# ZPP-Robotics/OSQP-Solver

Measured on AMD Instinct MI355X. Metric: QPs/sec on a 1024-QP batch of box-QPs (n=512, m=1024), OSQP defaults; ADMM iters/sec alongside, higher is better.
Workload: dtype f64

## Files before the change

### include/mi_osqp.h

```cpp
#ifndef MI_OSQP_H
#define MI_OSQP_H

#include <stdint.h>

#ifdef __cplusplus
extern "C" {
#endif

typedef enum {
  MI_OSQP_OK = 0,
  MI_OSQP_ERR_INVALID_DATA = 1,
  MI_OSQP_ERR_INVALID_SETTINGS = 2,
  MI_OSQP_ERR_PATTERN_CHANGED = 3,
  MI_OSQP_ERR_NONCONVEX = 4,
  MI_OSQP_ERR_DEVICE = 5,
  MI_OSQP_ERR_NULL = 6,
  MI_OSQP_ERR_ALLOC = 7
} mi_osqp_error;

typedef enum {
  MI_OSQP_EXIT_OPTIMAL = 0,
  MI_OSQP_EXIT_PRIMAL_INFEASIBLE = 1,
  MI_OSQP_EXIT_DUAL_INFEASIBLE = 2,
  MI_OSQP_EXIT_OPTIMAL_INACCURATE = 3,
  MI_OSQP_EXIT_PRIMAL_INFEASIBLE_INACCURATE = 4,
  MI_OSQP_EXIT_DUAL_INFEASIBLE_INACCURATE = 5,
  MI_OSQP_EXIT_MAX_ITERATIONS = 6,
  MI_OSQP_EXIT_INTERRUPTED = 7,
  MI_OSQP_EXIT_TIME_LIMIT_REACHED = 8,
  MI_OSQP_EXIT_NON_CONVEX = 9,
  MI_OSQP_EXIT_UNKNOWN = 10
} mi_osqp_exit_code;

typedef struct {
  double  rho;
  double  sigma;
  int64_t scaling;
  int64_t adaptive_rho;
  int64_t adaptive_rho_interval;
  double  adaptive_rho_tolerance;
  int64_t max_iter;
  double  eps_abs;
  double  eps_rel;
  double  eps_prim_inf;
  double  eps_dual_inf;
  double  alpha;
  int64_t scaled_termination;
  int64_t check_termination;
  int64_t warm_start;
  int64_t verbose;
  int64_t polish;
  int64_t polish_refine_iter;
  double  delta;
} mi_osqp_settings;

typedef struct {
  int64_t iter;
  int64_t status_val;
  int64_t exit_code;
  double  obj_val;
  double  pri_res;
  double  dua_res;
  int64_t rho_updates;
  double  rho_estimate;
  double  rho;
  int64_t status_polish;
} mi_osqp_info;

typedef struct {
  int64_t n, m, N, batch, tile, n_tiles;
  int64_t nnz_P_triu, nnz_A, nnz_KKT, nnz_L;
  int64_t n_supernodes, n_blocks;
  int64_t fwd_levels, bwd_levels, fwd_slots, bwd_slots, chk_slots;
  int64_t lds_bytes, threads_per_block;
  int64_t dense_tail_rows, dense_tail_slots;
  double  setup_seconds_host, setup_seconds_factor, setup_seconds_upload;
  int64_t nnz_L_before_tail;
  int64_t solve_groups, solve_group_threads;
  int64_t resident_state, lds_bytes_iterate;
  int64_t pipelined_refactors;
  int64_t resident_factor_steps, lds_bytes_factor;
  int64_t dense_tail_tasks, dense_tail_waves_used, dense_tail_wave_tasks_max;
  int64_t refactor_lanes;
  int64_t iterate_launches_deep_ring, iterate_launches_long_head;
} mi_osqp_stats;

typedef struct mi_osqp_solver mi_osqp_solver;
typedef struct mi_osqp_batch  mi_osqp_batch;

void        mi_osqp_default_settings(mi_osqp_settings *s);
const char *mi_osqp_exit_code_name(int64_t exit_code);
const char *mi_osqp_error_name(int64_t err);
const char *mi_osqp_version(void);
const char *mi_osqp_last_error(void);

int mi_osqp_setup(mi_osqp_solver **out, int64_t n, int64_t m,
                  const int64_t *P_colptr, const int64_t *P_rowidx, const double *P_val,
                  const double *q,
                  const int64_t *A_colptr, const int64_t *A_rowidx, const double *A_val,
                  const double *l, const double *u, const mi_osqp_settings *settings);
int mi_osqp_update_A(mi_osqp_solver *h, const int64_t *A_colptr, const int64_t *A_rowidx,
                     const double *A_val);
int mi_osqp_update_bounds(mi_osqp_solver *h, const double *l, const double *u);
int mi_osqp_update_A_bounds(mi_osqp_solver *h, const int64_t *A_colptr, const int64_t *A_rowidx, const double *A_val,
                            const double *l, const double *u);
int mi_osqp_warm_start_x(mi_osqp_solver *h, const double *x);
int mi_osqp_update_q(mi_osqp_solver *h, const double *q);
int mi_osqp_update_P(mi_osqp_solver *h, const int64_t *P_colptr, const int64_t *P_rowidx, const double *P_val);
int mi_osqp_update_P_A(mi_osqp_solver *h, const int64_t *P_colptr, const int64_t *P_rowidx, const double *P_val,
                       const int64_t *A_colptr, const int64_t *A_rowidx, const double *A_val);
int mi_osqp_warm_start_y(mi_osqp_solver *h, const double *y);
int mi_osqp_solve(mi_osqp_solver *h, mi_osqp_info *info);
int mi_osqp_get_primal(mi_osqp_solver *h, double *x_out);
int mi_osqp_get_dual(mi_osqp_solver *h, double *y_out);
int mi_osqp_get_prim_inf_cert(mi_osqp_solver *h, double *dy_out );
int mi_osqp_get_dual_inf_cert(mi_osqp_solver *h, double *dx_out );
int mi_osqp_adjoint(mi_osqp_solver *h, const double *dx, const double *dy, double *dq, double *dP, double *dA, double *dl, double *du,
                    int32_t *status);
int mi_osqp_get_stats(mi_osqp_solver *h, mi_osqp_stats *st);
int mi_osqp_get_settings(mi_osqp_solver *h, mi_osqp_settings *out);
int mi_osqp_update_settings(mi_osqp_solver *h, const mi_osqp_settings *s);
void mi_osqp_free(mi_osqp_solver *h);

int mi_osqp_batch_setup(mi_osqp_batch **out, int64_t B, int64_t n, int64_t m,
                        const int64_t *P_colptr, const int64_t *P_rowidx, const double *P_val,
                        const double *q,
                        const int64_t *A_colptr, const int64_t *A_rowidx, const double *A_val,
                        const double *l, const double *u, const mi_osqp_settings *settings,
                        int64_t device);
int mi_osqp_batch_update_A(mi_osqp_batch *h, const int64_t *A_colptr, const int64_t *A_rowidx,
                           const double *A_val);
int mi_osqp_batch_update_bounds(mi_osqp_batch *h, const double *l, const double *u);
int mi_osqp_batch_update_A_bounds(mi_osqp_batch *h, const int64_t *A_colptr, const int64_t *A_rowidx, const double *A_val,
                                  const double *l, const double *u);
int mi_osqp_batch_warm_start_x(mi_osqp_batch *h, const double *x);
int mi_osqp_batch_update_q(mi_osqp_batch *h, const double *q);
int mi_osqp_batch_update_P(mi_osqp_batch *h, const int64_t *P_colptr, const int64_t *P_rowidx, const double *P_val);
int mi_osqp_batch_update_P_A(mi_osqp_batch *h, const int64_t *P_colptr, const int64_t *P_rowidx, const double *P_val,
                             const int64_t *A_colptr, const int64_t *A_rowidx, const double *A_val);
int mi_osqp_batch_warm_start_y(mi_osqp_batch *h, const double *y);
int mi_osqp_batch_get_P_upper_pattern(mi_osqp_batch *h, int64_t *colptr, int64_t *rowidx, int64_t *nnz_out);
int mi_osqp_batch_solve(mi_osqp_batch *h);
int mi_osqp_batch_get_primal(mi_osqp_batch *h, double *x_out );
int mi_osqp_batch_get_dual(mi_osqp_batch *h, double *y_out );
int mi_osqp_batch_get_info(mi_osqp_batch *h, mi_osqp_info *info );
int mi_osqp_batch_get_prim_inf_cert(mi_osqp_batch *h, double *dy_out );
int mi_osqp_batch_get_dual_inf_cert(mi_osqp_batch *h, double *dx_out );
int mi_osqp_batch_get_stats(mi_osqp_batch *h, mi_osqp_stats *st);
int mi_osqp_batch_get_ordering(mi_osqp_batch *h, int64_t *kkt_perm);
void mi_osqp_batch_free(mi_osqp_batch *h);
int mi_osqp_prefetch_analysis(int64_t B, int64_t n, int64_t m, const int64_t *Pp, const int64_t *Pi,
                              const int64_t *Ap, const int64_t *Ai, int64_t device);
void mi_osqp_release_device_cache(void);

int mi_osqp_batch_update_bounds_device(mi_osqp_batch *h, const double *d_l, const double *d_u, void *stream);
int mi_osqp_batch_update_A_bounds_device(mi_osqp_batch *h, const double *d_Av, const double *d_l, const double *d_u, void *stream);
int mi_osqp_batch_update_q_device(mi_osqp_batch *h, const double *d_q, void *stream);
int mi_osqp_batch_update_P_device(mi_osqp_batch *h, const double *d_Pv, void *stream);
int mi_osqp_batch_update_P_A_bounds_device(mi_osqp_batch *h, const double *d_Pv, const double *d_Av, const double *d_l, const double *d_u,
                                           void *stream);
int mi_osqp_batch_solve_device(mi_osqp_batch *h, double *d_x_out, int32_t *d_status, int32_t *d_iters, void *stream);
int mi_osqp_batch_reset(mi_osqp_batch *h);
int mi_osqp_batch_last_solve_stats(mi_osqp_batch *h, int64_t *total_iters, int64_t *kernel_launches,
                                   double *device_seconds, double *refactor_seconds, int64_t *refactor_count,
                                   double *compact_seconds);
int mi_osqp_batch_last_polish_stats(mi_osqp_batch *h, int64_t *polished, int64_t *accepted, double *seconds);
int mi_osqp_batch_get_polish_active(mi_osqp_batch *h, int8_t *act);
// ... 45 lines not shown
int mi_gomp_scene_create(mi_gomp_scene **out, mi_osqp_batch *h, int64_t dims, int64_t waypoints,
                         int64_t n_balls, const mi_gomp_ball *balls, int64_t n_lines, const mi_gomp_line *lines,
                         const double *con_lo, const double *con_hi);
typedef struct { int32_t n_joints; int32_t reserved; double a[8], d[8], alpha[8], theta0[8]; } mi_gomp_chain;
int mi_gomp_scene_create_chain(mi_gomp_scene **out, mi_osqp_batch *h, int64_t dims, int64_t waypoints,
                               const mi_gomp_chain *chain, int64_t n_balls, const mi_gomp_ball *balls,
                               int64_t n_lines, const mi_gomp_line *lines, const double *con_lo, const double *con_hi);
typedef struct { double a[3], b[3]; double radius; double margin; } mi_gomp_capsule;
int mi_gomp_scene_create_world(mi_gomp_scene **out, mi_osqp_batch *h, int64_t dims, int64_t waypoints,
                               const mi_gomp_chain *chain, int64_t n_balls, const mi_gomp_ball *balls,
                               int64_t n_lines, const mi_gomp_line *lines, int64_t n_capsules, const mi_gomp_capsule *capsules,
                               const double *con_lo, const double *con_hi);
void mi_gomp_scene_free(mi_gomp_scene *sc);
int mi_gomp_scene_set_rows(mi_gomp_scene *sc, int64_t n_ids, const int64_t *ids, const double *A_val, const double *l, const double *u);
int mi_gomp_scene_get_rows(mi_gomp_scene *sc, int64_t id, double *A_val, double *l, double *u);
int mi_gomp_assemble_some(mi_gomp_scene *sc, int64_t n_ids, const int64_t *ids, const double *x, int32_t *ok_out);
int mi_gomp_relinearise_some(mi_gomp_scene *sc, int64_t n_ids, const int64_t *ids, const double *x, int32_t *ok_out);

typedef struct mi_osqp_multi mi_osqp_multi;
int mi_osqp_multi_batch_setup(mi_osqp_multi **out, int64_t n_devices, const int64_t *devices,
                              int64_t B, int64_t n, int64_t m,
                              const int64_t *P_colptr, const int64_t *P_rowidx, const double *P_val,
                              const double *q,
                              const int64_t *A_colptr, const int64_t *A_rowidx, const double *A_val,
                              const double *l, const double *u, const mi_osqp_settings *settings);
int mi_osqp_multi_batch_update_A(mi_osqp_multi *h, const int64_t *A_colptr, const int64_t *A_rowidx, const double *A_val);
int mi_osqp_multi_batch_update_bounds(mi_osqp_multi *h, const double *l, const double *u);
int mi_osqp_multi_batch_update_A_bounds(mi_osqp_multi *h, const int64_t *A_colptr, const int64_t *A_rowidx, const double *A_val,
                                        const double *l, const double *u);
int mi_osqp_multi_batch_warm_start_x(mi_osqp_multi *h, const double *x);
int mi_osqp_multi_batch_update_q(mi_osqp_multi *h, const double *q);
int mi_osqp_multi_batch_update_P(mi_osqp_multi *h, const int64_t *P_colptr, const int64_t *P_rowidx, const double *P_val);
int mi_osqp_multi_batch_update_P_A(mi_osqp_multi *h, const int64_t *P_colptr, const int64_t *P_rowidx, const double *P_val,
                                   const int64_t *A_colptr, const int64_t *A_rowidx, const double *A_val);
int mi_osqp_multi_batch_warm_start_y(mi_osqp_multi *h, const double *y);
int mi_osqp_multi_batch_get_settings(mi_osqp_multi *h, mi_osqp_settings *out);
int mi_osqp_multi_batch_update_settings(mi_osqp_multi *h, const mi_osqp_settings *s);
int mi_osqp_multi_batch_update_rho_each(mi_osqp_multi *h, const double *rho );
int mi_osqp_multi_batch_solve(mi_osqp_multi *h);
int mi_osqp_multi_batch_solve_async(mi_osqp_multi *h);
int mi_osqp_multi_batch_wait(mi_osqp_multi *h);
int mi_osqp_multi_batch_get_primal(mi_osqp_multi *h, double *x_out );
int mi_osqp_multi_batch_get_dual(mi_osqp_multi *h, double *y_out );
int mi_osqp_multi_batch_get_info(mi_osqp_multi *h, mi_osqp_info *info );
int mi_osqp_multi_batch_get_prim_inf_cert(mi_osqp_multi *h, double *dy_out );
int mi_osqp_multi_batch_get_dual_inf_cert(mi_osqp_multi *h, double *dx_out );
int64_t mi_osqp_multi_batch_shards(mi_osqp_multi *h);
int mi_osqp_multi_batch_shard(mi_osqp_multi *h, int64_t k, int64_t *device, int64_t *begin, int64_t *end, mi_osqp_batch **handle);
void mi_osqp_multi_batch_free(mi_osqp_multi *h);

int mi_osqp_batch_spmv(mi_osqp_batch *h, const double *d_x, const double *d_y,
                       double *d_Px, double *d_Aty, double *d_Ax, void *stream);
int mi_osqp_batch_kkt_solve(mi_osqp_batch *h, const double *d_rhs, double *d_sol, void *stream);
int mi_osqp_batch_refactor_device(mi_osqp_batch *h);
int mi_osqp_batch_kernel_time(mi_osqp_batch *h, double *avg_ms, int64_t *launches);
int mi_osqp_batch_refactor_time(mi_osqp_batch *h, double *factor_ms, double *tail_ms, int64_t *launches, int64_t *qps);
int mi_osqp_batch_refactor_peak(mi_osqp_batch *h, int64_t *qps, double *factor_ms, double *tail_ms);

int mi_osqp_batch_get_scaling(mi_osqp_batch *h, double *D , double *E , double *c );

int mi_osqp_debug_host_kkt_solve(int64_t n, int64_t m,
                                 const int64_t *P_colptr, const int64_t *P_rowidx, const double *P_val,
                                 const int64_t *A_colptr, const int64_t *A_rowidx, const double *A_val,
                                 const double *l, const double *u, const mi_osqp_settings *settings,
                                 int64_t tile, const double *rhs ,
                                 double *sol_schedule , double *sol_direct ,
                                 mi_osqp_stats *st);

int mi_osqp_debug_host_block_factor(int64_t n, int64_t m,
                                    const int64_t *P_colptr, const int64_t *P_rowidx, const double *P_val,
                                    const int64_t *A_colptr, const int64_t *A_rowidx, const double *A_val,
                                    const double *l, const double *u, const mi_osqp_settings *settings,
                                    double *max_rel_diff_L, double *max_rel_diff_Dinv, int64_t *counts);

int mi_osqp_debug_refactor_chunks(int64_t n_flagged, const int64_t *flagged, int64_t n_active, const int64_t *active, int64_t tile,
                                  int64_t chunk_qps, int64_t max_chunks, int64_t *n_chunks, int64_t *work_begin, int64_t *tiles,
                                  int64_t *tile_begin);

int mi_osqp_debug_refactor_lanes(int64_t n_flagged, const int64_t *flagged, int64_t n_active, const int64_t *active, int64_t tile,
                                 int64_t chunk_qps, int64_t max_chunks, int64_t kbt, int64_t lanes, int64_t chunk0_first,
                                 int64_t scratch_slots, int64_t *n_lanes, int64_t *lane_of, int64_t *order, int64_t *order_begin,
                                 int64_t *scratch_begin, int64_t *n_waits, int64_t *wait_chunk, int64_t *wait_for);

int mi_osqp_debug_iterate_form(int64_t tiles, int64_t has_head, int64_t forced_form, int64_t long_min, int64_t *form);

int mi_osqp_debug_trace_kkt_solve(mi_osqp_batch *h, int32_t which, const double *d_rhs, double *d_sol,
                                  uint32_t *out, int64_t out_capacity_words, int64_t *dims);

#ifdef __cplusplus
}
#endif
#endif
```

### osqp-solver_amd/__init__.py

```python
import ctypes as C
import os

import numpy as np

try:
    import torch
except ImportError:
    torch = None

from . import build as _build

_HERE = os.path.dirname(os.path.abspath(__file__))
_LIB = None

EXIT_NAMES = ["kOptimal", "kPrimalInfeasible", "kDualInfeasible", "kOptimalInaccurate",
              "kPrimalInfeasibleInaccurate", "kDualInfeasibleInaccurate", "kMaxIterations",
              "kInterrupted", "kTimeLimitReached", "kNonConvex", "kUnknown"]
K_OPTIMAL = 0


class Settings(C.Structure):
    _fields_ = [("rho", C.c_double), ("sigma", C.c_double), ("scaling", C.c_int64),
                ("adaptive_rho", C.c_int64), ("adaptive_rho_interval", C.c_int64),
                ("adaptive_rho_tolerance", C.c_double), ("max_iter", C.c_int64),
                ("eps_abs", C.c_double), ("eps_rel", C.c_double), ("eps_prim_inf", C.c_double),
                ("eps_dual_inf", C.c_double), ("alpha", C.c_double), ("scaled_termination", C.c_int64),
                ("check_termination", C.c_int64), ("warm_start", C.c_int64), ("verbose", C.c_int64),
                ("polish", C.c_int64), ("polish_refine_iter", C.c_int64), ("delta", C.c_double)]


class Info(C.Structure):
    _fields_ = [("iter", C.c_int64), ("status_val", C.c_int64), ("exit_code", C.c_int64),
                ("obj_val", C.c_double), ("pri_res", C.c_double), ("dua_res", C.c_double),
                ("rho_updates", C.c_int64), ("rho_estimate", C.c_double), ("rho", C.c_double),
                ("status_polish", C.c_int64)]

    def as_dict(self):
        return {k: getattr(self, k) for k, _ in self._fields_}


class Stats(C.Structure):
    _fields_ = [(k, C.c_int64) for k in
                ("n", "m", "N", "batch", "tile", "n_tiles", "nnz_P_triu", "nnz_A", "nnz_KKT", "nnz_L",
                 "n_supernodes", "n_blocks", "fwd_levels", "bwd_levels", "fwd_slots", "bwd_slots",
                 "chk_slots", "lds_bytes", "threads_per_block", "dense_tail_rows", "dense_tail_slots")] + \
               [(k, C.c_double) for k in ("setup_seconds_host", "setup_seconds_factor", "setup_seconds_upload")] + \
               [("nnz_L_before_tail", C.c_int64), ("solve_groups", C.c_int64), ("solve_group_threads", C.c_int64),
                ("resident_state", C.c_int64), ("lds_bytes_iterate", C.c_int64), ("pipelined_refactors", C.c_int64),
                ("resident_factor_steps", C.c_int64), ("lds_bytes_factor", C.c_int64),
                ("dense_tail_tasks", C.c_int64), ("dense_tail_waves_used", C.c_int64), ("dense_tail_wave_tasks_max", C.c_int64),
                ("refactor_lanes", C.c_int64),
                ("iterate_launches_deep_ring", C.c_int64), ("iterate_launches_long_head", C.c_int64)]

    def as_dict(self):
        return {k: getattr(self, k) for k, _ in self._fields_}


class MiOsqpError(RuntimeError):
    def __init__(self, code, where):
        self.code = int(code)
        L = lib()
        msg = L.mi_osqp_error_name(int(code)).decode()
        extra = L.mi_osqp_last_error().decode()
        super().__init__(f"{where}: error {int(code)} ({msg}) {extra}")


def lib():
    global _LIB
    if _LIB is None:
        path = os.path.join(_HERE, "libmi_osqp.so")
        if os.environ.get("MI_OSQP_LIBRARY"):
            path = os.environ["MI_OSQP_LIBRARY"]
        else:
            try:
                path = _build.build()
            except Exception as e:
                if not os.path.exists(path):
                    raise ImportError(f"libmi_osqp.so missing and could not be built: {e}") from e
        L = C.CDLL(path)
        ip, dp, vp = C.POINTER(C.c_int64), C.POINTER(C.c_double), C.c_void_p
        L.mi_osqp_default_settings.argtypes = [C.POINTER(Settings)]
        for f in ("mi_osqp_exit_code_name", "mi_osqp_error_name"):
            getattr(L, f).restype = C.c_char_p; getattr(L, f).argtypes = [C.c_int64]
        L.mi_osqp_version.restype = C.c_char_p
        L.mi_osqp_last_error.restype = C.c_char_p
        L.mi_osqp_batch_setup.argtypes = [C.POINTER(vp), C.c_int64, C.c_int64, C.c_int64, ip, ip, dp, dp, ip, ip, dp,
                                          dp, dp, C.POINTER(Settings), C.c_int64]
        L.mi_osqp_batch_update_A.argtypes = [vp, ip, ip, dp]
        L.mi_osqp_batch_update_A_bounds.argtypes = [vp, ip, ip, dp, dp, dp]
        L.mi_osqp_batch_update_bounds.argtypes = [vp, dp, dp]
        L.mi_osqp_batch_warm_start_x.argtypes = [vp, dp]
        L.mi_osqp_batch_update_q.argtypes = [vp, dp]
        L.mi_osqp_batch_update_q_device.argtypes = [vp, vp, vp]
        L.mi_osqp_batch_update_P.argtypes = [vp, ip, ip, dp]
        L.mi_osqp_batch_update_P_A.argtypes = [vp, ip, ip, dp, ip, ip, dp]
        L.mi_osqp_batch_warm_start_y.argtypes = [vp, dp]
        L.mi_osqp_batch_get_P_upper_pattern.argtypes = [vp, ip, ip, ip]
        L.mi_osqp_batch_update_P_device.argtypes = [vp, vp, vp]
        L.mi_osqp_batch_update_P_A_bounds_device.argtypes = [vp, vp, vp, vp, vp, vp]
        L.mi_osqp_batch_update_P_some.argtypes = [vp, C.c_int64, ip, dp]
        L.mi_osqp_batch_update_P_A_bounds_some.argtypes = [vp, C.c_int64, ip, dp, dp, dp, dp]
        L.mi_osqp_batch_update_q_some.argtypes = [vp, C.c_int64, ip, dp]
        L.mi_osqp_batch_warm_start_y_some.argtypes = [vp, C.c_int64, ip, dp]
        L.mi_osqp_settings_update_check.argtypes = [C.POINTER(Settings), C.POINTER(Settings)]
        L.mi_osqp_batch_get_settings.argtypes = [vp, C.POINTER(Settings)]
        L.mi_osqp_batch_update_settings.argtypes = [vp, C.POINTER(Settings)]
        L.mi_osqp_batch_update_rho_each.argtypes = [vp, dp]
        L.mi_osqp_batch_update_rho_some.argtypes = [vp, C.c_int64, ip, dp]
        L.mi_osqp_get_settings.argtypes = [vp, C.POINTER(Settings)]
        L.mi_osqp_update_settings.argtypes = [vp, C.POINTER(Settings)]
        L.mi_osqp_multi_batch_get_settings.argtypes = [vp, C.POINTER(Settings)]
        L.mi_osqp_multi_batch_update_settings.argtypes = [vp, C.POINTER(Settings)]
        L.mi_osqp_multi_batch_update_rho_each.argtypes = [vp, dp]
        L.mi_osqp_batch_solve.argtypes = [vp]
        L.mi_osqp_batch_get_primal.argtypes = [vp, dp]
        L.mi_osqp_batch_get_dual.argtypes = [vp, dp]
        L.mi_osqp_batch_get_info.argtypes = [vp, C.POINTER(Info)]
        for f in ("mi_osqp_get_prim_inf_cert", "mi_osqp_get_dual_inf_cert", "mi_osqp_batch_get_prim_inf_cert",
                  "mi_osqp_batch_get_dual_inf_cert", "mi_osqp_multi_batch_get_prim_inf_cert", "mi_osqp_multi_batch_get_dual_inf_cert"):
            getattr(L, f).argtypes = [vp, dp]
        L.mi_osqp_batch_get_prim_inf_cert_some.argtypes = [vp, C.c_int64, ip, dp]
        L.mi_osqp_batch_get_dual_inf_cert_some.argtypes = [vp, C.c_int64, ip, dp]
        L.mi_osqp_batch_get_stats.argtypes = [vp, C.POINTER(Stats)]
        L.mi_osqp_batch_get_ordering.argtypes = [vp, ip]
        L.mi_osqp_batch_free.argtypes = [vp]; L.mi_osqp_batch_free.restype = None
        L.mi_osqp_batch_update_bounds_device.argtypes = [vp, vp, vp, vp]
        L.mi_osqp_batch_update_A_bounds_device.argtypes = [vp, vp, vp, vp, vp]
        L.mi_osqp_batch_solve_device.argtypes = [vp, vp, vp, vp, vp]
        L.mi_osqp_batch_reset.argtypes = [vp]
        L.mi_osqp_batch_refactor_device.argtypes = [vp]
        L.mi_osqp_batch_last_solve_stats.argtypes = [vp, ip, ip, dp, dp, ip, dp]
        L.mi_osqp_batch_last_polish_stats.argtypes = [vp, ip, ip, dp]
        L.mi_osqp_batch_get_polish_active.argtypes = [vp, C.POINTER(C.c_int8)]
        L.mi_osqp_batch_adjoint.argtypes = [vp, dp, dp, dp, dp, dp, dp, dp, C.POINTER(C.c_int32)]
        L.mi_osqp_adjoint.argtypes = [vp, dp, dp, dp, dp, dp, dp, dp, C.POINTER(C.c_int32)]
        L.mi_osqp_batch_adjoint_device.argtypes = [vp] * 10
        L.mi_osqp_batch_get_scaling.argtypes = [vp, dp, dp, dp]
        L.mi_osqp_batch_spmv.argtypes = [vp, vp, vp, vp, vp, vp, vp]
        L.mi_osqp_batch_kkt_solve.argtypes = [vp, vp, vp, vp]
        L.mi_osqp_batch_kernel_time.argtypes = [vp, dp, ip]
        L.mi_osqp_batch_refactor_time.argtypes = [vp, dp, dp, ip, ip]
        L.mi_osqp_batch_refactor_peak.argtypes = [vp, ip, dp, dp]
        L.mi_osqp_batch_reinit_some.argtypes = [vp, C.c_int64, ip, dp, dp, dp]
        L.mi_osqp_batch_update_A_bounds_some.argtypes = [vp, C.c_int64, ip, dp, dp, dp]
        L.mi_osqp_batch_warm_start_x_some.argtypes = [vp, C.c_int64, ip, dp]
        L.mi_osqp_batch_solve_begin_some.argtypes = [vp, C.c_int64, ip]
        L.mi_osqp_batch_polish_some.argtypes = [vp, C.c_int64, ip]
        L.mi_osqp_batch_advance.argtypes = [vp, C.c_int64]
        L.mi_osqp_batch_poll.argtypes = [vp, C.c_int64, ip, ip, C.c_int64]
        L.mi_osqp_batch_get_primal_some.argtypes = [vp, C.c_int64, ip, dp]
        L.mi_osqp_batch_get_dual_some.argtypes = [vp, C.c_int64, ip, dp]
        L.mi_osqp_batch_get_info_some.argtypes = [vp, C.c_int64, ip, C.POINTER(Info)]
        L.mi_osqp_batch_running.argtypes = [vp]; L.mi_osqp_batch_running.restype = C.c_int64
        L.mi_osqp_batch_ring_wraps.argtypes = [vp]; L.mi_osqp_batch_ring_wraps.restype = C.c_int64
        L.mi_osqp_release_device_cache.argtypes = []; L.mi_osqp_release_device_cache.restype = None
        L.mi_osqp_setup.argtypes = [C.POINTER(vp), C.c_int64, C.c_int64, ip, ip, dp, dp, ip, ip, dp, dp, dp, C.POINTER(Settings)]
        L.mi_osqp_update_A.argtypes = [vp, ip, ip, dp]
        L.mi_osqp_update_bounds.argtypes = [vp, dp, dp]
        L.mi_osqp_warm_start_x.argtypes = [vp, dp]
        L.mi_osqp_update_q.argtypes = [vp, dp]
        L.mi_osqp_update_P.argtypes = [vp, ip, ip, dp]
        L.mi_osqp_update_P_A.argtypes = [vp, ip, ip, dp, ip, ip, dp]
        L.mi_osqp_warm_start_y.argtypes = [vp, dp]
        L.mi_osqp_solve.argtypes = [vp, C.POINTER(Info)]
        L.mi_osqp_get_primal.argtypes = [vp, dp]
        L.mi_osqp_get_dual.argtypes = [vp, dp]
        L.mi_osqp_get_stats.argtypes = [vp, C.POINTER(Stats)]
        L.mi_osqp_free.argtypes = [vp]; L.mi_osqp_free.restype = None
        L.mi_osqp_multi_batch_setup.argtypes = [C.POINTER(vp), C.c_int64, ip, C.c_int64, C.c_int64, C.c_int64, ip, ip, dp, dp,
                                                ip, ip, dp, dp, dp, C.POINTER(Settings)]
        L.mi_osqp_multi_batch_update_A.argtypes = [vp, ip, ip, dp]
        L.mi_osqp_multi_batch_update_bounds.argtypes = [vp, dp, dp]
        L.mi_osqp_multi_batch_update_A_bounds.argtypes = [vp, ip, ip, dp, dp, dp]
        L.mi_osqp_multi_batch_warm_start_x.argtypes = [vp, dp]
        L.mi_osqp_multi_batch_update_q.argtypes = [vp, dp]
        L.mi_osqp_multi_batch_update_P.argtypes = [vp, ip, ip, dp]
        L.mi_osqp_multi_batch_update_P_A.argtypes = [vp, ip, ip, dp, ip, ip, dp]
        L.mi_osqp_multi_batch_warm_start_y.argtypes = [vp, dp]
        L.mi_osqp_multi_batch_solve.argtypes = [vp]
        L.mi_osqp_multi_batch_solve_async.argtypes = [vp]
        L.mi_osqp_multi_batch_wait.argtypes = [vp]
        L.mi_osqp_multi_batch_get_primal.argtypes = [vp, dp]
        L.mi_osqp_multi_batch_get_dual.argtypes = [vp, dp]
        L.mi_osqp_multi_batch_get_info.argtypes = [vp, C.POINTER(Info)]
        L.mi_osqp_multi_batch_shards.argtypes = [vp]; L.mi_osqp_multi_batch_shards.restype = C.c_int64
        L.mi_osqp_multi_batch_shard.argtypes = [vp, C.c_int64, ip, ip, ip, C.POINTER(vp)]
        L.mi_osqp_multi_batch_free.argtypes = [vp]; L.mi_osqp_multi_batch_free.restype = None
        L.mi_osqp_debug_host_kkt_solve.argtypes = [C.c_int64, C.c_int64, ip, ip, dp, ip, ip, dp, dp, dp,
                                                   C.POINTER(Settings), C.c_int64, dp, dp, dp, C.POINTER(Stats)]
        L.mi_osqp_debug_refactor_chunks.argtypes = [C.c_int64, ip, C.c_int64, ip, C.c_int64, C.c_int64, C.c_int64, ip, ip, ip, ip]
        L.mi_osqp_debug_refactor_lanes.argtypes = [C.c_int64, ip, C.c_int64, ip] + [C.c_int64] * 7 + [ip] * 8
        L.mi_osqp_debug_iterate_form.argtypes = [C.c_int64] * 4 + [ip]
        L.mi_osqp_prefetch_analysis.argtypes = [C.c_int64, C.c_int64, C.c_int64, ip, ip, ip, ip, C.c_int64]
        L.mi_osqp_debug_host_block_factor.argtypes = [C.c_int64, C.c_int64, ip, ip, dp, ip, ip, dp, dp, dp,
                                                      C.POINTER(Settings), dp, dp, ip]
        _LIB = L
    return _LIB


def host_cores():
    try:
        n = len(os.sched_getaffinity(0))
    except Exception:
        n = os.cpu_count() or 1
    for path in ("/sys/fs/cgroup/cpu.max",):
        try:
            quota, period = open(path).read().split()[:2]
            if quota != "max":
                n = min(n, max(1, int(round(int(quota) / int(period)))))
        except Exception:
            pass
    try:
        q = int(open("/sys/fs/cgroup/cpu/cpu.cfs_quota_us").read())
        p = int(open("/sys/fs/cgroup/cpu/cpu.cfs_period_us").read())
        if q > 0:
            n = min(n, max(1, int(round(q / p))))
    except Exception:
        pass
    return n


def default_settings(**kw):
    s = Settings()
    lib().mi_osqp_default_settings(C.byref(s))
    for k, v in kw.items():
        if not hasattr(s, k):
            raise KeyError(k)
        setattr(s, k, v)
    return s


class HandleSettings(Settings):

    def bind(self, getter):
        self._getter = getter
        return self

    def __call__(self):
        out = Settings()
        self._getter(out)
        C.memmove(C.byref(self), C.byref(out), C.sizeof(Settings))
        return out


def settings_update_check(in_force, wanted):
    return int(lib().mi_osqp_settings_update_check(C.byref(in_force), C.byref(wanted)))


def _handle_settings(kw, get_name, owner):
    import weakref
    hs = HandleSettings()
    C.memmove(C.byref(hs), C.byref(default_settings(**kw)), C.sizeof(Settings))
    ref = weakref.ref(owner)

    def getter(out):
        _chk(getattr(lib(), get_name)(ref()._h, C.byref(out)), get_name)
    return hs.bind(getter)


def _update_settings(self, fn_name, fields):
    s = self.settings()
    for k, v in fields.items():
        if not hasattr(s, k):
            raise KeyError(k)
        setattr(s, k, v)
    _chk(getattr(lib(), fn_name)(self._h, C.byref(s)), fn_name)
    return self.settings()


def _i64(a):
    return np.ascontiguousarray(a, dtype=np.int64)


def _f64(a):
# ... 498 lines not shown
        return self._b.update_settings(**fields)

    def solve(self):
        info = self._b.solve()[0]
        return int(info.exit_code), self._b.primal()[0]

    def info(self):
        return self._b.info()[0]

    def dual(self):
        return self._b.dual()[0]

    def prim_inf_cert(self):
        return self._b.prim_inf_cert()[0]

    def dual_inf_cert(self):
        return self._b.dual_inf_cert()[0]

    def adjoint(self, dx, dy=None):
        out = self._b.adjoint(dx, dy)
        return {k: (int(v[0]) if k == "status" else v[0]) for k, v in out.items()}

    def stats(self):
        return self._b.stats()


def debug_host_kkt_solve(P, A, l, u, rhs, tri_waves=0, **settings):
    L = lib()
    P, A = _csc(P), _csc(A)
    n, m = A.shape[1], A.shape[0]
    s = default_settings(**settings)
    rhs = _f64(rhs)
    sol_s, sol_d = np.empty(n + m), np.empty(n + m)
    st = Stats()
    Pp, Pi, Px = _i64(P.indptr), _i64(P.indices), _f64(P.data)
    Ap, Ai, Ax = _i64(A.indptr), _i64(A.indices), _f64(A.data)
    l, u = _f64(l), _f64(u)
    rc = L.mi_osqp_debug_host_kkt_solve(n, m, _ip(Pp), _ip(Pi), _dp(Px), _ip(Ap), _ip(Ai), _dp(Ax), _dp(l), _dp(u),
                                        C.byref(s), 1 + int(tri_waves), _dp(rhs), _dp(sol_s), _dp(sol_d), C.byref(st))
    _chk(rc, "debug_host_kkt_solve")
    return sol_s, sol_d, st.as_dict()


def prefetch_analysis(P, A, B=1, device=-1, check=True):
    L = lib()
    P, A = _csc(P), _csc(A)
    n, m = A.shape[1], A.shape[0]
    Pp, Pi, Ap, Ai = _i64(P.indptr), _i64(P.indices), _i64(A.indptr), _i64(A.indices)
    rc = L.mi_osqp_prefetch_analysis(B, n, m, _ip(Pp), _ip(Pi), _ip(Ap), _ip(Ai), device)
    if check:
        _chk(rc, "prefetch_analysis")
    return rc


def debug_refactor_chunks(flagged, active, tile, chunk_qps, max_chunks=8):
    f, a = _i64(flagged), _i64(active)
    nch = C.c_int64()
    wb = np.zeros(max_chunks + 2, dtype=np.int64); tb = np.zeros(max_chunks + 2, dtype=np.int64)
    tl = np.zeros(max(1, len(a)), dtype=np.int64)
    _chk(lib().mi_osqp_debug_refactor_chunks(len(f), _ip(f), len(a), _ip(a), tile, chunk_qps, max_chunks, C.byref(nch), _ip(wb), _ip(tl),
                                             _ip(tb)), "debug_refactor_chunks")
    k = int(nch.value)
    return ([f[wb[c]:wb[c + 1]].tolist() for c in range(k)], [tl[tb[c]:tb[c + 1]].tolist() for c in range(k)])


def debug_refactor_lanes(flagged, active, tile, chunk_qps, lanes, kbt=None, chunk0_first=False, scratch_slots=None, max_chunks=8):
    f, a = _i64(flagged), _i64(active)
    kbt = tile if kbt is None else kbt
    work, _ = debug_refactor_chunks(flagged, active, tile, chunk_qps, max_chunks)
    k = len(work)
    nl, nw = C.c_int64(), C.c_int64()
    lane_of = np.zeros(max_chunks + 2, dtype=np.int64); order = np.zeros(max_chunks + 2, dtype=np.int64)
    ob = np.zeros(4, dtype=np.int64); sb = np.zeros(max_chunks + 2, dtype=np.int64)
    wc = np.zeros((max_chunks + 1) ** 2, dtype=np.int64); wf = np.zeros((max_chunks + 1) ** 2, dtype=np.int64)
    _chk(lib().mi_osqp_debug_refactor_lanes(len(f), _ip(f), len(a), _ip(a), tile, chunk_qps, max_chunks, kbt, lanes, int(bool(chunk0_first)),
                                            2 ** 31 - 1 if scratch_slots is None else scratch_slots, C.byref(nl), _ip(lane_of), _ip(order),
                                            _ip(ob), _ip(sb), C.byref(nw), _ip(wc), _ip(wf)), "debug_refactor_lanes")
    L = int(nl.value)
    return dict(n_lanes=L, lane_of=lane_of[:k].tolist(), order=[order[ob[l]:ob[l + 1]].tolist() for l in range(L)],
                scratch=[(int(sb[c]), (len(work[c]) + kbt - 1) // kbt * kbt) for c in range(k)],
                waits=list(zip(wc[:nw.value].tolist(), wf[:nw.value].tolist())))


def debug_iterate_form(tiles, has_head=True, forced_form=0, long_min=-1):
    form = C.c_int64()
    _chk(lib().mi_osqp_debug_iterate_form(tiles, int(bool(has_head)), forced_form, long_min, C.byref(form)), "debug_iterate_form")
    return int(form.value)


def debug_host_block_factor(P, A, l, u, **settings):
    L = lib()
    P, A = _csc(P), _csc(A)
    n, m = A.shape[1], A.shape[0]
    s = default_settings(**settings)
    Pp, Pi, Px = _i64(P.indptr), _i64(P.indices), _f64(P.data)
    Ap, Ai, Ax = _i64(A.indptr), _i64(A.indices), _f64(A.data)
    l, u = _f64(l), _f64(u)
    dL, dD = C.c_double(), C.c_double()
    cnt = (C.c_int64 * 4)()
    rc = L.mi_osqp_debug_host_block_factor(n, m, _ip(Pp), _ip(Pi), _dp(Px), _ip(Ap), _ip(Ai), _dp(Ax), _dp(l), _dp(u),
                                           C.byref(s), C.byref(dL), C.byref(dD), cnt)
    _chk(rc, "debug_host_block_factor")
    return dL.value, dD.value, dict(blocks=cnt[0], triples=cnt[1], storage=cnt[2], levels=cnt[3])
```

### osqp-solver_amd/csrc/device_types.h

```cpp
#pragma once
#include <hip/hip_runtime.h>
#include <stdint.h>

namespace miosqp {

#define MI_CHUNK 16

struct SchedDev {
  const uint32_t *step, *idxw;
  const uint64_t *idxw64;
  const uint32_t *lvl_pos, *tail_bar;
  int n_phases, nw, n_levels;
  uint32_t n_steps, n_slots;
};

struct DenseTailDev {
  int s, k, n_phases;
  uint32_t n_steps;
  const uint32_t *task;
  const uint32_t *wave_task, *wave_step, *tail_bar;
};

enum { DS_C = 0, DS_CINV, DS_RHO, DS_RHO_EST, DS_PRI_RES, DS_DUA_RES, DS_OBJ, DS_COUNT };
enum { IS_STATUS = 0, IS_ITER, IS_RHO_UPDATES, IS_DONE, IS_NEED_REFACTOR, IS_CUR, IS_PENDING, IS_EPOCH, IS_COUNT };

enum { RF_FORM_NONE = 0, RF_FORM_DEEP_RING = 1, RF_FORM_LONG_HEAD = 2 };

struct KernelArgs {
  int n, m, N, B;
  SchedDev fwd, bwd, chk;
  const uint32_t *pinv;
  const uint32_t *xloc;
  const double *fwd_val, *bwd_val, *chk_val, *dinv;
  DenseTailDev dt;
  const double *dt_val;
  const double *fwd_val0, *bwd_val0, *dt_val0;
  const int *use_work;
  double *x, *z, *y;
  const double *q, *l, *u, *rho_vec, *rho_inv, *Dsc, *Dsc_inv, *Esc, *Esc_inv;
  double *dx, *dy, *out1, *out2, *dscal;
  int *iscal;
  double *x_out, *y_out;
  double *cert_out;
  int cert_stride;
  double *xs_global;
  int xs_len;
  int rs_off;
  int rf_off;
  int rf_form;
  int wide;
  double sigma, alpha, eps_abs, eps_rel, eps_prim_inf, eps_dual_inf, rho_tolerance;
  int check_termination, rho_interval, max_iter, scaled_termination, scaling, adaptive_rho;
  int iter_begin, iter_end;
  int op_out_lds;
  int info_at_end;
  int mw_groups;
  unsigned *mw_bar;
  double *mw_scratch;
  int df;
  unsigned df_shadow;
  const unsigned char *rflag;
  const int *sel;
  const int *tiles;
};

struct FactorArgs {
  int n, m, N, B, nnzP, nnzK, pa_len, n_levels, force_all;
  int debug_skip;
  uint32_t storage;
  SchedDev fwd, bwd;
  const uint32_t *blk, *lvl, *utask, *tri4, *dtask, *ttask, *asm_dst, *asm_src;
  const uint32_t *ubig;
  int *use_work;
  const int32_t *fwd_srcblk, *bwd_srcblk;
  const double *pa_val, *l, *u, *dscal;
  double *rho_vec, *rho_inv, *Lblk, *Dl, *dinv_scratch, *fwd_val, *bwd_val, *dinv;
  int *iscal, *npos;
  int home_bt;
  const int *work;
  int wg_base;
  double sigma;
  int dt_k;
  int mw_groups;
  unsigned *mw_bar;
  const signed char *pmask;
  const int32_t *arow;
  int *pstat;
  double pdelta;
};

struct TailArgs {
  int n, N, s, k, kbt, home_bt;
  uint32_t storage, n_slots;
  int n_lt, n_ltcol;
  uint32_t n_quads;
  int nh;
  uint32_t cs_doubles;
  const int *work;
  int wg_base;
  const uint32_t *lt_pos, *ltcol_col, *tile_tab, *wave_tiles, *diag_tile;
  const uint64_t *asm_q64;
  const int32_t *src_tile;
  const uint32_t *dt_task, *dt_task_step;
  uint32_t n_tasks;
  const double *Lblk, *Dl;
  double *Sd, *dt_val, *dinv;
  int *npos, *iscal;
  unsigned long long *trace;
  int *pstat;
};
hipError_t launch_tail(const TailArgs &a, int nwork, size_t lds_asm, size_t lds, hipStream_t st);

struct PolishArgs {
  int *stat;
  signed char *act;
  double *sol;
  int refine_iter;
  int inner;
  double delta;
};
hipError_t launch_polish_active(const KernelArgs &a, const PolishArgs &p, int BT, hipStream_t st);
hipError_t launch_polish_active_list(const KernelArgs &a, const PolishArgs &p, const int *slots, int nslots, int BT, hipStream_t st);
hipError_t launch_polish_publish(const KernelArgs &a, const PolishArgs &p, const int *slots, int nslots, int *host_stat, int BT, hipStream_t st);
hipError_t launch_polish(const KernelArgs &a, const PolishArgs &p, int BT, int tiles, int threads, size_t lds, int n_cus, hipStream_t st);
struct AdjointArgs {
  const double *gx, *gy;
  double *dq, *dP, *dA, *dl, *du;
  const int32_t *prow, *pcol, *arow, *acol;
  int nnzP, nnzA;
};
hipError_t launch_adjoint(const KernelArgs &a, const PolishArgs &p, const AdjointArgs &g, int BT, int tiles, int threads, size_t lds, int n_cus, hipStream_t st);
hipError_t launch_adjoint_finish(const int *stat, const AdjointArgs &g, int32_t *status, int B, int n, int m, hipStream_t st);
hipError_t launch_factor(const FactorArgs &a, int BT, int tiles, int threads, hipStream_t st);
size_t factor_lds_bytes(int BT, int threads);
bool factor_fits_lds(const FactorArgs &a, int threads);

int max_coresident_groups(int threads, size_t lds, int n_cus);
int max_coresident_factor_groups(int threads, int n_cus);
hipError_t launch_iterate(const KernelArgs &a, int BT, int tiles, int threads, size_t lds, hipStream_t st);
int rf_head_steps(int form);
int rf_lds_steps();
hipError_t launch_check(const KernelArgs &a, int BT, int tiles, int threads, size_t lds, hipStream_t st);
hipError_t launch_advance(const KernelArgs &a, int BT, int tiles, int threads, size_t lds, hipStream_t st, int max_segments, int seg_len,
                          int *host_is, double *host_ds, unsigned *stop, unsigned seq, unsigned *counter, unsigned *host_done);
hipError_t launch_spmv(const KernelArgs &a, int BT, int tiles, int threads, size_t lds, hipStream_t st,
                       const double *x, const double *y, double *Px, double *Aty, double *Ax);
struct SpmvFused {
  const uint32_t *ptr, *ent;
  const double *pa_val;
  int pa_len;
  const uint32_t *ell, *rowid;
  int n_pass;
  uint32_t ell_off[4], ell_k[4];
};
hipError_t launch_spmv_fused(const KernelArgs &a, const SpmvFused &t, int BT, int tiles, int n_cus, hipStream_t st,
                             const double *x, const double *y, double *Px, double *Aty, double *Ax);
size_t spmv_fused_lds_bytes(int n, int m, int pa_len, int BT);
hipError_t launch_kkt_solve(const KernelArgs &a, int BT, int tiles, int threads, size_t lds, hipStream_t st,
                            const double *rhs, double *sol);
hipError_t launch_kkt_trace(const KernelArgs &a, int BT, int tiles, int threads, size_t lds, hipStream_t st,
                            const double *rhs, double *sol, uint32_t *trace, uint32_t words);
hipError_t launch_warm_start(const KernelArgs &a, int BT, int tiles, int threads, size_t lds, hipStream_t st,
                             const double *x0);
hipError_t launch_interleave(const double *src, double *dst, const int *ids, int nq, int len, int BT, hipStream_t st);
hipError_t launch_scatter(const double *src, double *dst, const int *map, const int *ids, int nq, int srclen,
                          const SchedDev &sd, int BT, hipStream_t st);
hipError_t launch_deinterleave(const double *src, double *dst, int nq, int len, int BT, hipStream_t st);
struct RuizArgs {
  int n, m, nnzP, nnzA, B, BT, iters;
  const int *ids;
  int raw_by_qp;
  int fresh;
  const double *rawP, *rawq;
  const int32_t *Prow, *Pcol, *Arow, *Acol;
  const double *rawPnew;
  const double *rawA;
  const double *rawl, *rawu;
  double *pa_val, *q, *Dsc, *Dsc_inv, *Esc, *Esc_inv, *l, *u, *dscal;
  double *dn, *en;
  double *pa_out;
};
hipError_t launch_ruiz(const RuizArgs &a, hipStream_t st);
hipError_t launch_lin_cost(const double *gq, const int *ids, double *q, double *rawq, const double *Dsc, const double *dscal,
                           int nq, int n, int BT, int scaling, hipStream_t st);
hipError_t launch_warm_start_y(const KernelArgs &a, int nslots, int BT, hipStream_t st, const double *y0);
hipError_t launch_start_slots(const KernelArgs &a, const int *slots, const int *clear, int nslots, int BT, int cold, hipStream_t st);
hipError_t launch_fresh_slots(const KernelArgs &a, const int *slots, int nslots, int BT, double rho0, hipStream_t st);
hipError_t launch_set_rho_slots(const KernelArgs &a, const int *slots, const double *rho, double rho_all, int nslots, int BT, hipStream_t st);
hipError_t launch_worklist(const int *iscal, int *work, int nslots, int BT, hipStream_t st);
hipError_t launch_resume_flagged(const KernelArgs &a, int nslots, int BT, hipStream_t st);
hipError_t launch_copy_slot_streams(double *dst, const double *src, const int *slots, int nslots, size_t per, hipStream_t st);
hipError_t launch_keep_rows(double *dst, const double *src, const int *ids, int n_ids, int len, hipStream_t st);
hipError_t launch_copy_flagged_streams(double *dst, const double *src, const int *flags, int want, int nslots, size_t per, hipStream_t st);
hipError_t launch_copy_slot_rows(double *dst, const double *src, const int *slots, int nslots, int len, int BT, hipStream_t st);
enum { MI_GM_UR5E_FLANGE = 1, MI_GM_UR5E_WRIST3 = 2, MI_GM_UR5E_ELBOW = 3, MI_GM_YAW_2LINK = 4, MI_GM_TABLE = 5, MI_GM_DH_CHAIN = 6 };
#define MI_GOMP_MAXD 8
struct GompChainDev { int n_joints, pad; double a[MI_GOMP_MAXD], d[MI_GOMP_MAXD], ca[MI_GOMP_MAXD], sa[MI_GOMP_MAXD], theta0[MI_GOMP_MAXD]; };
struct GompBallDev { int model, is_gripper; double radius; double param[12]; };
struct GompLineDev { double D[3], A[3]; int below, pad; };
struct GompCapsuleDev { double a[3], e[3], ee, R, margin; };
struct GompArgs {
  int dims, W, n_balls, n_lines, n, m, nnzA, n_ids, row0, write_rows;
  int n_caps, pad;
  const int *ids;
  const GompBallDev *balls;
  const GompLineDev *lines;
  const GompCapsuleDev *caps;
  double con_lo[3], con_hi[3];
  const int *aidx;
  const double *traj;
  double *A, *l, *u;
  int *ok;
  GompChainDev chain;
};
hipError_t launch_gomp_relinearise(const GompArgs &g, hipStream_t st);
hipError_t launch_gather_status(const int *iscal, int32_t *status, int32_t *iters, int B, int BT, hipStream_t st);
hipError_t launch_fail_slots(const KernelArgs &a, const int *slots, int nfail, int BT, int iter, hipStream_t st);
hipError_t launch_fail_flagged(const KernelArgs &a, const int *slots, int nslots, int BT, int iter, hipStream_t st);
hipError_t launch_bounds(const double *gl, const double *gu, double *l, double *u, const double *Esc,
                         const double *rho_vec, const double *dscal, int *changed, int B, int m, int BT,
                         int scaling, hipStream_t st);

}
```

### osqp-solver_amd/csrc/host_core.cpp

```cpp
#include "host_core.hpp"
#include "sched_format.h"

#include <algorithm>
#include <cmath>
#include <cstdio>
#include <cstdlib>
#include <cstring>
#include <numeric>
#include <set>
#include <chrono>
#include <thread>

#include "../../include/mi_osqp.h"

namespace miosqp {

int validate_settings(const Settings &s) {
  if (s.scaling < 0 || s.max_iter <= 0 || s.check_termination < 0) return 1;
  if (s.adaptive_rho != 0 && s.adaptive_rho != 1) return 1;
  if (s.adaptive_rho_interval < 0 || s.adaptive_rho_tolerance < 1.0) return 1;
  if (!(s.rho > 0.0) || !(s.sigma > 0.0)) return 1;
  if (s.eps_abs < 0.0 || s.eps_rel < 0.0 || (s.eps_abs == 0.0 && s.eps_rel == 0.0)) return 1;
  if (!(s.eps_prim_inf > 0.0) || !(s.eps_dual_inf > 0.0)) return 1;
  if (!(s.alpha > 0.0) || !(s.alpha < 2.0)) return 1;
  if ((s.scaled_termination | 1) != 1 || (s.warm_start | 1) != 1) return 1;
  if ((s.polish | 1) != 1 || s.polish_refine_iter < 0 || !(s.delta > 0.0)) return 1;
  return 0;
}


static void min_degree(int N, const std::vector<int> &Kp, const std::vector<int> &Ki,
                       std::vector<int> &perm) {
  std::vector<std::vector<int>> adj(N);
  for (int j = 0; j < N; j++)
    for (int k = Kp[j]; k < Kp[j + 1]; k++) {
      int i = Ki[k];
      if (i != j) { adj[i].push_back(j); adj[j].push_back(i); }
    }
  for (auto &a : adj) { std::sort(a.begin(), a.end()); a.erase(std::unique(a.begin(), a.end()), a.end()); }
  std::vector<char> dead(N, 0);
  std::set<std::pair<int, int>> pq;
  std::vector<int> deg(N);
  for (int v = 0; v < N; v++) { deg[v] = (int)adj[v].size(); pq.insert({deg[v], v}); }
  perm.assign(N, 0);
  std::vector<int> tmp;
  int alive = N;
  for (int step = 0; step < N && !pq.empty();) {
    const int v = pq.begin()->second;
    pq.erase(pq.begin());
    if ((int)adj[v].size() == alive - 1) {
      perm[step++] = v; dead[v] = 1;
      for (int u = 0; u < N; u++) if (!dead[u]) { perm[step++] = u; dead[u] = 1; }
      break;
    }
    perm[step++] = v; dead[v] = 1; alive--;
    const std::vector<int> S = adj[v];
    for (int u : S) {
      tmp.clear();
      std::set_union(adj[u].begin(), adj[u].end(), S.begin(), S.end(), std::back_inserter(tmp));
      tmp.erase(std::remove_if(tmp.begin(), tmp.end(), [&](int x) { return x == u || x == v; }), tmp.end());
      adj[u].swap(tmp);
      pq.erase({deg[u], u});
      deg[u] = (int)adj[u].size();
      pq.insert({deg[u], u});
    }
    std::vector<int>().swap(adj[v]);
  }
}

namespace {
struct NDCtx {
  const std::vector<std::vector<int>> &adj;
  std::vector<int> stamp, level;
  int cur = 0;
  std::vector<int> out;
  int leaf;
};

void nd_leaf(NDCtx &c, const std::vector<int> &nodes) {
  int k = (int)nodes.size();
  if (k <= 2) { for (int v : nodes) c.out.push_back(v); return; }
  int st = ++c.cur;
  std::vector<int> loc(k);
  for (int i = 0; i < k; i++) { c.stamp[nodes[i]] = st; c.level[nodes[i]] = i; }
  std::vector<int> Kp(k + 1, 0), Ki;
  for (int j = 0; j < k; j++) {
    for (int u : c.adj[nodes[j]]) if (c.stamp[u] == st && c.level[u] < j) Ki.push_back(c.level[u]);
    Ki.push_back(j);
    Kp[j + 1] = (int)Ki.size();
  }
// ... 777 lines not shown
    }
    dt.n_lt = (int)dt.lt_pos.size(); dt.n_ltcol = (int)dt.ltcol_col.size();
    const uint16_t zero_slot = (uint16_t)dt.n_lt;
    for (auto &fr : frag) for (auto &f : fr) for (uint16_t &v : f.second) if (v == 0xFFFFu) v = zero_slot;
    struct TileRec { int I, J; std::vector<std::pair<int, int>> src; };
    std::vector<TileRec> tiles;
    for (int I = 0; I < nt; I++)
      for (int J = 0; J <= I; J++) {
        TileRec t{I, J, {}};
        size_t a = 0, b = 0;
        while (a < frag[I].size() && b < frag[J].size()) {
          if (frag[I][a].first < frag[J][b].first) a++;
          else if (frag[I][a].first > frag[J][b].first) b++;
          else { t.src.push_back({(int)a, (int)b}); a++; b++; }
        }
        tiles.push_back(std::move(t));
      }
    const int nw = 16;
    std::vector<int> order(tiles.size());
    std::iota(order.begin(), order.end(), 0);
    std::stable_sort(order.begin(), order.end(), [&](int x, int y) { return tiles[x].src.size() > tiles[y].src.size(); });
    std::vector<std::vector<int>> mine(nw);
    for (size_t d = 0; d < order.size(); d++) { const size_t round = d / nw, pos = d % nw; mine[(round & 1) ? nw - 1 - pos : pos].push_back(order[d]); }
    dt.tile_tab.clear(); dt.wave_tiles.assign(nw + 1, 0u); dt.asm_q.clear(); dt.asm_qcol.clear();
    for (int w = 0; w < nw; w++) {
      dt.wave_tiles[w] = (uint32_t)(dt.tile_tab.size() / 4);
      for (int ti : mine[w]) {
        const TileRec &t = tiles[ti];
        const uint32_t q0 = (uint32_t)(dt.asm_q.size() / 64);
        const size_t padded = (t.src.size() + 31) / 32 * 32;
        for (size_t s0 = 0; s0 < padded; s0 += 4) {
          for (int g = 0; g < 4; g++) {
            const bool real = s0 + g < t.src.size();
            const auto *fa = real ? &frag[t.I][t.src[s0 + g].first] : nullptr;
            const auto *fb = real ? &frag[t.J][t.src[s0 + g].second] : nullptr;
            dt.asm_qcol.push_back(real ? (uint16_t)fa->first : (uint16_t)0);
            for (int e = 0; e < 16; e++) dt.asm_q.push_back(real ? ((uint32_t)fa->second[e] | ((uint32_t)fb->second[e] << 16)) : ((uint32_t)zero_slot | ((uint32_t)zero_slot << 16)));
          }
        }
        const uint32_t blk_id = find_blk(ct0 + t.I, ct0 + t.J);
        dt.tile_tab.insert(dt.tile_tab.end(), {((uint32_t)t.I << 16) | (uint32_t)t.J, bf.blk[4 * blk_id], q0, (uint32_t)(dt.asm_q.size() / 64)});
      }
    }
    dt.wave_tiles[nw] = (uint32_t)(dt.tile_tab.size() / 4);
    dt.asm_q64.resize(dt.asm_q.size());
    for (size_t e = 0; e < dt.asm_q.size(); e++) {
      const uint64_t w = dt.asm_q[e], ci = dt.asm_qcol[e / 16];
      dt.asm_q64[e] = ((w & 0xFFFFu) * 8u) | ((((w >> 16) * 8u) | ((ci * 8u) << 17)) << 32);
    }
    dt.src_tile.resize(dt.src.size());
    for (size_t e = 0; e < dt.src.size(); e++) {
      const int32_t sc = dt.src[e];
      dt.src_tile[e] = sc < 0 ? sc : (int32_t)dt_tile_offset(sc % k, sc / k);
    }
    dt.diag_tile.resize(k);
    for (int i = 0; i < k; i++) dt.diag_tile[i] = dt_tile_offset(i, i);
    dt.task_step.clear();
    { uint32_t pos = 0; for (size_t t = 0; t < dt.task.size() / 4; t++) { dt.task_step.push_back(pos); pos += dt.task[4 * t + 3]; } }
  }
}


Tuning tuning_from_env() {
  Tuning t;
  if (const char *e = getenv("MI_OSQP_TILE")) { const int v = atoi(e); if (v == 1 || v == 2 || v == 4) t.tile = v; }
  if (const char *e = getenv("MI_OSQP_THREADS")) t.threads = std::max(64, std::min(1024, atoi(e) / 64 * 64));
  t.global_xs = getenv("MI_OSQP_GLOBAL_XS") != nullptr;
  if (const char *e = getenv("MI_OSQP_GROUPS")) t.groups = std::max(0, std::min(256, atoi(e)));
  if (const char *e = getenv("MI_OSQP_GROUP_THREADS")) t.group_threads = std::max(64, std::min(512, atoi(e) / 64 * 64));
  if (const char *e = getenv("MI_OSQP_ASSUME_CUS")) t.assume_cus = std::max(0, atoi(e));
  if (const char *e = getenv("MI_OSQP_FACTOR_THREADS")) t.factor_threads = std::max(64, std::min(1024, atoi(e) / 64 * 64));
  if (const char *e = getenv("MI_OSQP_FACTOR_GROUPS")) t.factor_groups = std::max(1, std::min(256, atoi(e)));
  t.ruiz = getenv("MI_OSQP_HOST_RUIZ") ? 1 : getenv("MI_OSQP_DEVICE_RUIZ") ? -1 : 0;
  if (const char *e = getenv("MI_OSQP_CONT_RING_KB")) t.cont_ring_kb = std::max(0L, atol(e));
  if (const char *e = getenv("MI_OSQP_ANALYSIS_CACHE")) t.analysis_cache = atoi(e) != 0;
  t.stream_state = getenv("MI_OSQP_STREAM_STATE") != nullptr;
  t.stream_factor = getenv("MI_OSQP_STREAM_FACTOR") != nullptr;
  if (const char *e = getenv("MI_OSQP_REFACTOR_PIPELINE")) t.refactor_pipeline = atoi(e) != 0;
  if (const char *e = getenv("MI_OSQP_REFACTOR_PIPELINE_MIN")) t.pipeline_min = std::max(0, atoi(e));
  if (const char *e = getenv("MI_OSQP_REFACTOR_CHUNKS")) t.pipeline_chunks = std::max(0, std::min(8, atoi(e)));
  if (const char *e = getenv("MI_OSQP_REFACTOR_CHUNK_QPS")) t.pipeline_chunk_qps = std::max(0, atoi(e));
  if (const char *e = getenv("MI_OSQP_REFACTOR_LANES")) t.refactor_lanes = std::max(1, std::min(3, atoi(e)));
  if (const char *e = getenv("MI_OSQP_REFACTOR_CHUNK0")) t.lanes_chunk0 = atoi(e) != 0;
  if (const char *e = getenv("MI_OSQP_RF_FORM")) { const int v = atoi(e); if (v == kIterDeepRing || v == kIterLongHead) t.rf_form = v; }
  if (const char *e = getenv("MI_OSQP_RF_LONG_MIN")) t.rf_long_min = std::max(0, atoi(e));
  AnalysisTuning &a = t.analysis;
  if (const char *e = getenv("MI_OSQP_DENSE_TAIL")) a.dense_tail = atoi(e);
  if (const char *e = getenv("MI_OSQP_ORDERING")) a.ordering = e[0];
  if (const char *e = getenv("MI_OSQP_ND_LEAF")) a.nd_leaf = atoi(e);
  if (const char *e = getenv("MI_OSQP_RELAX")) a.relax = atoi(e);
  a.serial = getenv("MI_OSQP_SERIAL_ANALYSIS") != nullptr;
  return t;
}

RefactorChunks refactor_chunks(const std::vector<int> &flagged, const std::vector<int> &active, int bt, int chunk_qps, int max_chunks) {
  RefactorChunks rc;
  const int nq = (int)flagged.size();
  max_chunks = std::max(1, max_chunks);
  chunk_qps = std::max(1, chunk_qps);
  if ((nq + chunk_qps - 1) / chunk_qps > max_chunks) chunk_qps = (nq + max_chunks - 1) / max_chunks;
  const int n_ref = (nq + chunk_qps - 1) / chunk_qps;
  rc.n_chunks = 1 + n_ref;
  rc.work_begin.assign(1, 0);
  for (int c = 0; c <= n_ref; c++) rc.work_begin.push_back(std::min(nq, c * chunk_qps));
  std::vector<std::pair<int, int>> tc;
  size_t f = 0;
  for (size_t i = 0; i < active.size(); i++) {
    const int tile = active[i] / bt;
    if (i && active[i - 1] / bt == tile) continue;
    int chunk = 0;
    while (f < flagged.size() && flagged[f] / bt < tile) f++;
    for (size_t g = f; g < flagged.size() && flagged[g] / bt == tile; g++) chunk = 1 + (int)g / chunk_qps;
    tc.emplace_back(chunk, tile);
  }
  std::stable_sort(tc.begin(), tc.end(), [](const std::pair<int, int> &x, const std::pair<int, int> &y) { return x.first < y.first; });
  rc.tile_begin.assign((size_t)rc.n_chunks + 1, 0);
  for (const auto &p : tc) { rc.tiles.push_back(p.second); rc.tile_begin[(size_t)p.first + 1]++; }
  for (int c = 0; c < rc.n_chunks; c++) rc.tile_begin[(size_t)c + 1] += rc.tile_begin[c];
  return rc;
}

RefactorLanes refactor_lanes(const RefactorChunks &ch, const std::vector<int> &flagged, int bt, int kbt, int lanes, bool chunk0_first, int scratch_slots) {
  RefactorLanes rl;
  const int nc = ch.n_chunks, n_ref = nc - 1;
  bt = std::max(1, bt); kbt = std::max(1, kbt);
  int L = std::max(1, std::min(std::min(3, lanes), std::max(1, n_ref)));
  std::vector<int> padded((size_t)nc + 1, 0);
  for (int c = 1; c < nc; c++) padded[(size_t)c + 1] = padded[c] + (ch.work_begin[(size_t)c + 1] - ch.work_begin[c] + kbt - 1) / kbt * kbt;
  if (padded[nc] > scratch_slots) L = 1;
  rl.n_lanes = L;
  rl.lane_of.assign(nc, 0);
  rl.order.assign(L, std::vector<int>());
  rl.scratch_begin.assign((size_t)nc + 1, 0);
  if (L == 1) {
    for (int c = 0; c < nc; c++) rl.order[0].push_back(c);
    return rl;
  }
  rl.scratch_begin = padded;
  for (int c = 1; c < nc; c++) { rl.lane_of[c] = (c - 1) % L; rl.order[(c - 1) % L].push_back(c); }
  if (chunk0_first) { rl.lane_of[0] = L - 1; rl.order[L - 1].insert(rl.order[L - 1].begin(), 0); }
  else {
    int at = L - 1;
    for (int a = L - 1; a >= 0; a--) if (rl.order[a].size() < rl.order[at].size()) at = a;
    rl.lane_of[0] = at; rl.order[at].push_back(0);
  }
  for (int c = 1; c < nc; c++) {
    std::vector<char> need(nc, 0);
    for (int t = ch.tile_begin[c]; t < ch.tile_begin[(size_t)c + 1]; t++) {
      const int tile = ch.tiles[t];
      size_t g = std::lower_bound(flagged.begin(), flagged.end(), tile * bt) - flagged.begin();
      for (; g < flagged.size() && flagged[g] / bt == tile; g++) {
        const int d = (int)(std::upper_bound(ch.work_begin.begin() + 1, ch.work_begin.end(), (int)g) - ch.work_begin.begin()) - 1;
        if (d >= 1 && d < c && rl.lane_of[d] != rl.lane_of[c]) need[d] = 1;
      }
    }
    for (int d = 1; d < c; d++) if (need[d]) { rl.wait_chunk.push_back(c); rl.wait_for.push_back(d); }
  }
  return rl;
}

int iterate_form(int tiles, bool has_head, const Tuning &t) {
  if (!has_head) return kIterStreamed;
  if (t.rf_form == kIterDeepRing || t.rf_form == kIterLongHead) return t.rf_form;
  const int long_min = t.rf_long_min >= 0 ? t.rf_long_min : kRfLongMinDefault;
  return tiles > 0 && tiles >= long_min ? kIterLongHead : kIterDeepRing;
}


int analyze(int64_t n64, int64_t m64, const int64_t *Pp, const int64_t *Pi, const int64_t *Ap,
            const int64_t *Ai, const AnalysisTuning &tune, Analysis &an, int nwaves, int bt, int max_extra_rows, int dense_tail_max, int tri_waves, int n_tiles) {
  if (nwaves < 1 || nwaves > 16 || (bt != 1 && bt != 2 && bt != 4) || tri_waves < 0 || tri_waves > 2048) return MI_OSQP_ERR_INVALID_SETTINGS;
  if (n64 <= 0 || m64 < 0 || !Pp || !Ap || n64 + m64 > (int64_t)1 << 30) return MI_OSQP_ERR_INVALID_DATA;
  int n = (int)n64, m = (int)m64, N = n + m;
  an = Analysis();
  an.n = n; an.m = m; an.N = N;
  if (Pp[0] != 0 || Ap[0] != 0) return MI_OSQP_ERR_INVALID_DATA;
  for (int j = 0; j < n; j++) {
    if (Pp[j + 1] < Pp[j] || Ap[j + 1] < Ap[j]) return MI_OSQP_ERR_INVALID_DATA;
    for (int64_t k = Pp[j]; k < Pp[j + 1]; k++) if (Pi[k] < 0 || Pi[k] >= n) return MI_OSQP_ERR_INVALID_DATA;
    for (int64_t k = Ap[j]; k < Ap[j + 1]; k++) if (Ai[k] < 0 || Ai[k] >= m) return MI_OSQP_ERR_INVALID_DATA;
  }
  if (Pp[n] > (int64_t)1 << 30 || Ap[n] > (int64_t)1 << 30) return MI_OSQP_ERR_INVALID_DATA;
  an.Pp.assign(n + 1, 0);
  for (int j = 0; j < n; j++) {
    an.Pp[j] = (int)an.Pi.size();
    for (int64_t k = Pp[j]; k < Pp[j + 1]; k++)
      if (Pi[k] <= j) { an.Pi.push_back((int)Pi[k]); an.Psrc.push_back((int)k); }
  }
  an.Pp[n] = (int)an.Pi.size();
  an.Ap.assign(Ap, Ap + n + 1);
  an.Ai.assign(Ai, Ai + Ap[n]);
  int nnzP = an.Pp[n], nnzA = an.Ap[n];
  std::vector<int> cnt(N, 0);
  an.PisDiag.assign(nnzP, 0);
  std::vector<char> hasDiag(n, 0);
  for (int j = 0; j < n; j++)
    for (int k = an.Pp[j]; k < an.Pp[j + 1]; k++) { cnt[j]++; if (an.Pi[k] == j) { hasDiag[j] = 1; an.PisDiag[k] = 1; } }
  for (int j = 0; j < n; j++) if (!hasDiag[j]) cnt[j]++;
  for (int k = 0; k < nnzA; k++) cnt[n + an.Ai[k]]++;
  for (int r = 0; r < m; r++) cnt[n + r]++;
  an.Kp.assign(N + 1, 0);
  for (int j = 0; j < N; j++) an.Kp[j + 1] = an.Kp[j] + cnt[j];
  an.Ki.assign(an.Kp[N], 0);
  an.PtoK.assign(nnzP, 0); an.AtoK.assign(nnzA, 0); an.rhotoK.assign(m, 0);
  std::vector<int> nxt(an.Kp.begin(), an.Kp.end() - 1);
  for (int j = 0; j < n; j++) {
    for (int k = an.Pp[j]; k < an.Pp[j + 1]; k++) { int pos = nxt[j]++; an.Ki[pos] = an.Pi[k]; an.PtoK[k] = pos; }
    if (!hasDiag[j]) { int pos = nxt[j]++; an.Ki[pos] = j; an.sigmaOnlyK.push_back(pos); }
  }
  for (int j = 0; j < n; j++)
    for (int k = an.Ap[j]; k < an.Ap[j + 1]; k++) { int pos = nxt[n + an.Ai[k]]++; an.Ki[pos] = j; an.AtoK[k] = pos; }
  for (int r = 0; r < m; r++) { int pos = nxt[n + r]++; an.Ki[pos] = n + r; an.rhotoK[r] = pos; }
  an.tri_waves = tri_waves;
  an.wide = N >= 65535 || 2 * n + m >= 65535 || tri_waves > 0;
  if (max_extra_rows < 0) max_extra_rows = 1 << 30;
  if (!an.wide && max_extra_rows > 65534 - N) max_extra_rows = 65534 - N;
  auto finalize = [&](Analysis &an, const std::vector<int> &perm0, double &cost, int relax_zeros = 0, int *phases_out = nullptr, double *stream_out = nullptr) {
    an.perm = perm0;
    an.pinv.assign(N, 0);
    for (int k = 0; k < N; k++) an.pinv[an.perm[k]] = k;
    build_permuted_lower(an);
    std::vector<std::vector<int>> cols;
    std::vector<int> parent, post;
    symbolic(an, cols, parent);
    postorder(parent, post);
    {
      std::vector<int> p2(N);
      for (int k = 0; k < N; k++) p2[k] = an.perm[post[k]];
      an.perm.swap(p2);
      for (int k = 0; k < N; k++) an.pinv[an.perm[k]] = k;
    }
    build_permuted_lower(an);
    symbolic(an, cols, parent);
    an.etree = parent;
    if (relax_zeros > 0) {
      auto close = [&](int s0, int e) {
        for (int c = s0; c < e; c++) {
          std::vector<int> ns;
          ns.reserve((size_t)(e - c) + cols[e].size());
          for (int r = c + 1; r <= e; r++) ns.push_back(r);
          ns.insert(ns.end(), cols[e].begin(), cols[e].end());
// ... 719 lines not shown
```

### osqp-solver_amd/csrc/host_core.hpp

```cpp
#pragma once

#include <cstdint>
#include <string>
#include <vector>

namespace miosqp {

constexpr double kInfty = 1e30;
constexpr double kRhoMin = 1e-6, kRhoMax = 1e6, kRhoEqOverIneq = 1e3, kRhoTol = 1e-4;
constexpr double kMinScaling = 1e-4, kMaxScaling = 1e4;
constexpr double kDivisionTol = 1.0 / kInfty;
constexpr int kChunk = 16;
constexpr uint32_t kNoRow = 0xFFFFFFFFu;

struct Settings {
  double rho = 0.1, sigma = 1e-6;
  int64_t scaling = 10, adaptive_rho = 1, adaptive_rho_interval = 0;
  double adaptive_rho_tolerance = 5.0;
  int64_t max_iter = 4000;
  double eps_abs = 1e-3, eps_rel = 1e-3, eps_prim_inf = 1e-4, eps_dual_inf = 1e-4, alpha = 1.6;
  int64_t scaled_termination = 0, check_termination = 25, warm_start = 1, verbose = 0;
  int64_t polish = 0, polish_refine_iter = 3;
  double delta = 1e-6;
};
int validate_settings(const Settings &s);

struct AnalysisTuning {
  int dense_tail = -1;
  char ordering = 0;
  int nd_leaf = 0;
  int relax = -1;
  bool serial = false;
  bool operator==(const AnalysisTuning &o) const {
    return dense_tail == o.dense_tail && ordering == o.ordering && nd_leaf == o.nd_leaf && relax == o.relax && serial == o.serial;
  }
};
struct Tuning {
  int tile = 0;
  int threads = 0;
  bool global_xs = false;
  int groups = -1;
  int group_threads = 0;
  int assume_cus = 0;
  int factor_threads = 1024;
  int factor_groups = 0;
  int ruiz = 0;
  long cont_ring_kb = -1;
  bool analysis_cache = true;
  bool stream_state = false;
  bool stream_factor = false;
  bool refactor_pipeline = true;
  int pipeline_min = 0;
  int pipeline_chunks = 0;
  int pipeline_chunk_qps = 0;
  int refactor_lanes = 0;
  int lanes_chunk0 = -1;
  int rf_form = 0;
  int rf_long_min = -1;
  AnalysisTuning analysis;
};
Tuning tuning_from_env();

enum IterateForm { kIterStreamed = 0, kIterDeepRing = 1, kIterLongHead = 2 };
constexpr int kRfLongMinDefault = 0;
int iterate_form(int tiles, bool has_head, const Tuning &t);

struct RefactorChunks {
  int n_chunks = 1;
  std::vector<int> work_begin;
  std::vector<int> tiles;
  std::vector<int> tile_begin;
};
RefactorChunks refactor_chunks(const std::vector<int> &flagged, const std::vector<int> &active, int bt, int chunk_qps, int max_chunks);

struct RefactorLanes {
  int n_lanes = 1;
  std::vector<int> lane_of;
  std::vector<std::vector<int>> order;
  std::vector<int> scratch_begin;
  std::vector<int> wait_chunk, wait_for;
};
RefactorLanes refactor_lanes(const RefactorChunks &ch, const std::vector<int> &flagged, int bt, int kbt, int lanes, bool chunk0_first, int scratch_slots);

struct Schedule {
  int n_phases = 0, nw = 0, bt = 1;
  bool barriers = true;
  std::vector<uint32_t> phase;
  std::vector<int> level_first_phase;
  std::vector<uint32_t> step;
  std::vector<uint32_t> step_ob;
  std::vector<uint32_t> outA;
  std::vector<uint32_t> idx;
  std::vector<uint32_t> idxw;
  std::vector<uint64_t> idxw64;
  std::vector<int32_t> src;
  uint32_t n_slots = 0;
  uint32_t n_steps = 0;
  std::vector<uint32_t> wave_range;
  std::vector<uint32_t> lvl_pos;
  std::vector<uint32_t> tail_bar;
  bool dataflow = false;
  uint32_t shadow = 0, pad = 0;
  uint32_t phys_steps() const { return n_steps; }
  size_t phase_stride() const { return 4 * (size_t)nw + 1; }
  int n_levels = 0;
};

struct BlockFactor {
  uint32_t storage = 0;
  std::vector<uint32_t> blk;
  std::vector<uint32_t> lvl;
  std::vector<uint32_t> utask;
  std::vector<uint32_t> tri;
  std::vector<uint32_t> tri4;
  std::vector<uint32_t> utask4;
  bool overflow = false;
  std::vector<uint32_t> ubig;
  std::vector<uint32_t> dtask4;
  std::vector<uint32_t> ttask4;
  std::vector<uint32_t> dtask;
  std::vector<uint32_t> ttask;
  std::vector<uint32_t> asm_dst;
  std::vector<uint32_t> asm_src;
  std::vector<int32_t> lpos;
  int n_levels = 0;
  size_t n_blocks() const { return blk.size() / 4; }
};
enum { ASM_P = 0, ASM_P_SIGMA = 1, ASM_SIGMA = 2, ASM_A = 3, ASM_NEG_RHOINV = 4 };

struct DenseTail {
  int s = 0, k = 0, nb = 0;
  int nw = 0, n_phases = 0;
  uint32_t n_steps = 0;
  std::vector<uint32_t> task;
  std::vector<uint32_t> wave_task;
  std::vector<uint32_t> wave_step;
  std::vector<uint32_t> tail_bar;
  std::vector<int32_t> src;
  std::vector<uint32_t> sblk;
  int n_lt = 0, n_ltcol = 0;
  std::vector<uint32_t> lt_pos;
  std::vector<uint32_t> ltcol_col;
  std::vector<uint32_t> tile_tab;
  std::vector<uint32_t> wave_tiles;
  std::vector<uint32_t> asm_q;
  std::vector<uint16_t> asm_qcol;
  std::vector<uint64_t> asm_q64;
  std::vector<int32_t> src_tile;
  std::vector<uint32_t> diag_tile;
  std::vector<uint32_t> task_step;
  size_t asm_lds_bytes() const { return ((size_t)n_lt + 1 + (size_t)n_ltcol) * sizeof(double); }
};
inline uint32_t dt_tile_offset(int i, int j) {
  const int I = i / 16, J = j / 16, r = i % 16, c = j % 16;
  return (uint32_t)((I * (I + 1) / 2 + J) * 256 + ((r % 4) * 16 + c) * 4 + r / 4);
}
enum { DT_DIAG = 1, DT_SWAP = 2 };

struct Analysis {
  int n = 0, m = 0, N = 0;
  bool wide = false;
  std::vector<int> Pp, Pi, Psrc;
  std::vector<int> Ap, Ai;
  std::vector<int> Kp, Ki, PtoK, AtoK, rhotoK, sigmaOnlyK;
  std::vector<char> PisDiag;
// ... 65 lines not shown
```

### osqp-solver_amd/csrc/kernels.hip

```cpp
#include <hip/hip_runtime.h>
#include <stdint.h>
#include <stdlib.h>
#include <string.h>

#include <algorithm>
#include <map>
#include <mutex>

#include "device_types.h"
#include "sched_format.h"

namespace miosqp {

static hipError_t ensure_dynamic_lds(const void *kern, size_t lds);

#define MI_INFTY 1e30
#define MI_MIN_SCALING 1e-4
#define MI_DIV_TOL 1e-30
#define MI_RHO_EST_DIV 1e-10
#define MI_RHO_MIN 1e-6
#define MI_RHO_MAX 1e6
#define MI_NOROW 0xFFFFFFFFu
#ifdef MI_OSQP_DEBUG_BUILD
#define MI_DBG_SKIP(a) ((a).debug_skip)
// ... 881 lines not shown
      run_tri<BT, MI_PFV_NT(NT, GX), GX, 0, WIDE>(a.bwd, p.vbwd, xs, wave, lane);
    } else {
      kkt_solve_lds<BT, MI_PFV_NT(NT, GX), GX, WIDE>(a, p, xs, tid, nthr, wave, nw, lane, mw);
    }
    constexpr int U = GX ? 4 : 1;
    int tid_i = tid;
    if constexpr (RF != 0) asm volatile("" : "+v"(tid_i));
    uint32_t fl[U], xl[U];
    for (int e0 = tid_i; e0 < n * BT; e0 += nthr * U) {
      size_t pos[U]; double xt[U], xp[U], qv[U];
#pragma unroll
      for (int u = 0; u < U; u++) { const int e = e0 + u * nthr < n * BT ? e0 + u * nthr : e0; pos[u] = (size_t)a.pinv[e / BT] * BT + b; }
      if (df) {
#pragma unroll
        for (int u = 0; u < U; u++) { fl[u] = a.rflag[pos[u]]; xl[u] = a.xloc[pos[u]]; }
      }
#pragma unroll
      for (int u = 0; u < U; u++) {
        const int e = e0 + u * nthr < n * BT ? e0 + u * nthr : e0;
        xt[u] = df ? ld_sc1(xs + df_bloc((uint32_t)pos[u], fl[u], sh)) : xs[pos[u]]; xp[u] = X[e]; qv[u] = Q[e];
      }
#pragma unroll
      for (int u = 0; u < U; u++) {
        const int e = e0 + u * nthr;
        if (e < n * BT) {
          double xn = alpha * xt[u] + (1.0 - alpha) * xp[u];
          if (!done) {
            X[e] = xn;
            if constexpr (RS) { if (last) p.x[e] = xn; }
            if (do_info) p.dx[e] = xn - xp[u];
          } else xn = xp[u];
          if (df) { st_sc1(xs + pos[u], sigma * xn - qv[u]); df_arm_fwd(xs, (uint32_t)pos[u], fl[u], xl[u], sh); }
          else xs[pos[u]] = sigma * xn - qv[u];
        }
      }
    }
    for (int e0 = tid_i; e0 < m * BT; e0 += nthr * U) {
      size_t pos[U]; double nu[U], zp[U], yv[U], ri[U], rv[U], lo[U], up[U];
#pragma unroll
      for (int u = 0; u < U; u++) { const int e = e0 + u * nthr < m * BT ? e0 + u * nthr : e0; pos[u] = (size_t)a.pinv[n + e / BT] * BT + b; }
      if (df) {
#pragma unroll
        for (int u = 0; u < U; u++) { fl[u] = a.rflag[pos[u]]; xl[u] = a.xloc[pos[u]]; }
      }
#pragma unroll
      for (int u = 0; u < U; u++) {
        const int e = e0 + u * nthr < m * BT ? e0 + u * nthr : e0;
        nu[u] = df ? ld_sc1(xs + df_bloc((uint32_t)pos[u], fl[u], sh)) : xs[pos[u]]; zp[u] = Z[e]; yv[u] = Y[e]; ri[u] = RI[e]; rv[u] = RV[e]; lo[u] = LO[e]; up[u] = UP[e];
      }
#pragma unroll
      for (int u = 0; u < U; u++) {
        const int e = e0 + u * nthr;
        if (e < m * BT) {
          double zt = zp[u] - ri[u] * yv[u];
          zt += ri[u] * nu[u];
          const double zr = alpha * zt + (1.0 - alpha) * zp[u];
          double zn = fmin(fmax(zr + ri[u] * yv[u], lo[u]), up[u]);
          const double dyv = rv[u] * (zr - zn);
          double yn = yv[u] + dyv;
          if (!done) {
            Z[e] = zn; Y[e] = yn;
            if constexpr (RS) { if (last) { p.z[e] = zn; p.y[e] = yn; } }
            if (do_info) p.dy[e] = dyv;
          } else { zn = zp[u]; yn = yv[u]; }
          if (df) { st_sc1(xs + pos[u], zn - ri[u] * yn); df_arm_fwd(xs, (uint32_t)pos[u], fl[u], xl[u], sh); }
          else xs[pos[u]] = zn - ri[u] * yn;
        }
      }
    }
    if constexpr (GX) wg_or_grid_barrier(mw); else __syncthreads();
  }
}
template <int BT, int NT, bool GX, bool WIDE = false, bool RS = false, int RF = 0>
__global__ __launch_bounds__(NT) void iterate_kernel(KernelArgs a) {
  extern __shared__ double smem[];
  iterate_body<BT, NT, GX, WIDE, RS, RF>(a, smem, a.iter_end - a.iter_begin);
}

template <int BT, int NT, bool GX, bool WIDE = false>
__device__ __forceinline__ int check_body(const KernelArgs &a, double *smem, int n_iter) {
  bool dfm = false;
  if constexpr (GX && BT == 1 && WIDE) dfm = a.df != 0 && a.mw_groups > 1;
  const Mw mw{a.mw_bar, dfm ? (unsigned)a.mw_groups : 1u};
  const int tile = dfm ? 0 : blockIdx.x;
  const int ltid = threadIdx.x, lwave = __builtin_amdgcn_readfirstlane(ltid >> 6), lnw = blockDim.x >> 6;
  const int tid = dfm ? blockIdx.x * blockDim.x + threadIdx.x : threadIdx.x, nthr = dfm ? blockDim.x * mw.G : blockDim.x;
  const int lane = tid & 63, wave = __builtin_amdgcn_readfirstlane(tid >> 6), nw = nthr >> 6;
  const int b = tid % BT;
  auto sync = [&]() { if constexpr (GX && BT == 1 && WIDE) wg_or_grid_barrier(mw); else __syncthreads(); };
  auto gscratch = [&](int slot) { return a.mw_scratch + (size_t)slot * 256 * 16; };
  const int n = a.n, m = a.m;
  double *red;
  double *xs = solve_vector<BT, GX>(a, smem, tile, red);
  const TilePtrs<BT> p = tile_ptrs<BT>(a, tile, true);
  int done = p.iscal[IS_DONE * BT + b];
  if (__syncthreads_and(done)) return 0;
  const int iter = p.iscal[IS_CUR * BT + b] + n_iter;
  int status = p.iscal[IS_STATUS * BT + b];
  int rho_updates = p.iscal[IS_RHO_UPDATES * BT + b];
  double rho = p.dscal[DS_RHO * BT + b];
  const double c = p.dscal[DS_C * BT + b], cinv = p.dscal[DS_CINV * BT + b];
  const bool unscale = a.scaling && !a.scaled_termination;
  const bool is_last = iter >= a.max_iter;
  const bool is_check = a.check_termination && (iter % a.check_termination == 0);
  const bool is_rho = a.adaptive_rho && a.rho_interval && (iter % a.rho_interval == 0);
  bool any_check = is_check || is_last, any_last = is_last;
  if constexpr (BT > 1) { any_check = __syncthreads_or(any_check); any_last = __syncthreads_or(any_last); }
  int need_refactor = 0;
  for (int e = tid; e < n * BT; e += nthr) xs[e] = p.x[e];
  for (int e = tid; e < m * BT; e += nthr) xs[(size_t)n * BT + e] = p.y[e];
  sync();
  run_spmv<BT, MI_PFV, WIDE>(a.chk, p.vchk, xs, p.out1, wave, lane, 0, 3, nw);
  sync();
  double mx[14];
#pragma unroll
  for (int k = 0; k < 14; k++) mx[k] = 0.0;
  double sm[1] = {0.0};
  for (int e = tid; e < n * BT; e += nthr) {
    const double px = p.out1[e], aty = p.out1[(size_t)n * BT + e], qv = p.q[e], xv = p.x[e];
    const double di = p.Dsc_inv[e];
    double dres = qv + px;
    dres += aty;
    mx[0] = fmax(mx[0], fabs(dres));      mx[1] = fmax(mx[1], fabs(di * dres));
    mx[2] = fmax(mx[2], fabs(qv));        mx[3] = fmax(mx[3], fabs(aty));   mx[4] = fmax(mx[4], fabs(px));
    mx[5] = fmax(mx[5], fabs(di * qv));   mx[6] = fmax(mx[6], fabs(di * aty)); mx[7] = fmax(mx[7], fabs(di * px));
    sm[0] += 0.5 * xv * px + qv * xv;
  }
  for (int e = tid; e < m * BT; e += nthr) {
    const double ax = p.out1[(size_t)2 * n * BT + e], zv = p.z[e], ei = p.Esc_inv[e];
    const double pres = ax - zv;
    mx[8] = fmax(mx[8], fabs(pres));      mx[9] = fmax(mx[9], fabs(ei * pres));
    mx[10] = fmax(mx[10], fabs(zv));      mx[11] = fmax(mx[11], fabs(ax));
    mx[12] = fmax(mx[12], fabs(ei * zv)); mx[13] = fmax(mx[13], fabs(ei * ax));
  }
  block_reduce<BT, 14, true>(mx, red, ltid, lwave, lnw, lane);
  block_reduce<BT, 1, false>(sm, red, ltid, lwave, lnw, lane);
  if constexpr (GX && BT == 1 && WIDE) {
    grid_reduce<14, true>(mx, red, mw, gscratch(0), ltid, lwave, lnw, lane);
    grid_reduce<1, false>(sm, red, mw, gscratch(1), ltid, lwave, lnw, lane);
  }
  const double pri_res = (m == 0) ? 0.0 : (unscale ? mx[9] : mx[8]);
  const double dua_res = unscale ? cinv * mx[1] : mx[0];
  double obj = sm[0];
  if (a.scaling) obj *= cinv;
  const double pri_nrm = unscale ? fmax(mx[12], mx[13]) : fmax(mx[10], mx[11]);
  const double dua_nrm = unscale ? cinv * fmax(fmax(mx[5], mx[6]), mx[7]) : fmax(fmax(mx[2], mx[3]), mx[4]);

  double mi[4] = {0.0, 0.0, 0.0, 0.0};
  double si[2] = {0.0, 0.0};
  for (int e = tid; e < n * BT; e += nthr) {
    const double d = p.dx[e];
    xs[e] = d;
    mi[1] = fmax(mi[1], unscale ? fabs(p.Dsc[e] * d) : fabs(d));
    si[1] += p.q[e] * d;
  }
  for (int e = tid; e < m * BT; e += nthr) {
    double d = p.dy[e];
    const double lo = p.l[e], up = p.u[e];
    if (up > MI_INFTY * MI_MIN_SCALING) {
      if (lo < -MI_INFTY * MI_MIN_SCALING) d = 0.0; else d = fmin(d, 0.0);
    } else if (lo < -MI_INFTY * MI_MIN_SCALING) d = fmax(d, 0.0);
    xs[(size_t)n * BT + e] = d;
    mi[0] = fmax(mi[0], unscale ? fabs(p.Esc[e] * d) : fabs(d));
    si[0] += up * fmax(d, 0.0) + lo * fmin(d, 0.0);
  }
  sync();
  run_spmv<BT, MI_PFV, WIDE>(a.chk, p.vchk, xs, p.out2, wave, lane, 0, 3, nw);
// ... 41 lines not shown
             mi[3] < cost_scaling * eps_dinf * norm_dx) dual_inf = viol[0] == 0.0;
    if (prim_ok && dual_ok) return approx ? 2 : 1;
    if (prim_inf) return approx ? 3 : -3;
    if (dual_inf) return approx ? 4 : -4;
    return 0;
  };

  int new_status = 0;
  if (any_check) { const int s0 = decide(false); if (is_check || is_last) new_status = s0; }
  double rho_est = p.dscal[DS_RHO_EST * BT + b];
  auto rho_estimate = [&]() -> double {
    const double pr = mx[8] / (fmax(mx[10], mx[11]) + MI_RHO_EST_DIV);
    const double du = mx[0] / (fmax(fmax(mx[2], mx[3]), mx[4]) + MI_RHO_EST_DIV);
    double e = rho * sqrt(pr / du);
    return fmin(fmax(e, MI_RHO_MIN), MI_RHO_MAX);
  };
  if (!done && is_rho && (new_status == 0 || (is_last && !is_check))) {
    const double rn = rho_estimate();
    rho_est = rn;
    if (rn > rho * a.rho_tolerance || rn < rho / a.rho_tolerance) {
      need_refactor = 1;
      rho = fmin(fmax(rn, MI_RHO_MIN), MI_RHO_MAX);
      rho_updates++;
    }
  }
  if (any_last) {
    const int s1 = decide(true);
    if (!done && new_status == 0 && is_last) new_status = s1 ? s1 : -2;
  }
  if (!done && new_status != 0) {
    done = 1; status = new_status;
    rho_est = rho_estimate();

    if (tid < BT) {
      p.dscal[DS_PRI_RES * BT + b] = pri_res; p.dscal[DS_DUA_RES * BT + b] = dua_res;
      p.dscal[DS_OBJ * BT + b] = (status == -3 || status == 3) ? MI_INFTY
                                 : (status == -4 || status == 4) ? -MI_INFTY
                                 : (status == -7) ? __builtin_nan("") : obj;
      p.iscal[IS_ITER * BT + b] = iter;
    }
  }
  if (tid < BT) p.dscal[DS_RHO_EST * BT + b] = rho_est;
  const int just_done = done && (p.iscal[IS_DONE * BT + b] == 0);
  sync();
  const int slot = tile * BT + b, qp = slot < a.B ? slot : -1;
  if (just_done && qp >= 0) {
    const bool has_sol = !(status == -3 || status == 3 || status == -4 || status == 4 || status == -7);
    const double nanv = __builtin_nan("");
    for (int e = tid; e < n * BT; e += nthr) {
      const int i = e / BT;
      a.x_out[(size_t)qp * n + i] = has_sol ? (a.scaling ? p.Dsc[e] * p.x[e] : p.x[e]) : nanv;
      if (!has_sol) p.x[e] = 0.0;
    }
    for (int e = tid; e < m * BT; e += nthr) {
      const int j = e / BT;
      a.y_out[(size_t)qp * m + j] = has_sol ? (a.scaling ? p.Esc[e] * p.y[e] * cinv : p.y[e]) : nanv;
      if (!has_sol) { p.y[e] = 0.0; p.z[e] = 0.0; }
    }
    if (status == -3 || status == 3) {
      double *cert = a.cert_out + (size_t)qp * a.cert_stride;
      for (int e = tid; e < m * BT; e += nthr) {
        double d = p.dy[e];
        const double lo = p.l[e], up = p.u[e];
        if (up > MI_INFTY * MI_MIN_SCALING) {
          if (lo < -MI_INFTY * MI_MIN_SCALING) d = 0.0; else d = fmin(d, 0.0);
        } else if (lo < -MI_INFTY * MI_MIN_SCALING) d = fmax(d, 0.0);
        cert[e / BT] = (unscale ? p.Esc[e] * d : d) / norm_dy;
      }
    } else if (status == -4 || status == 4) {
      double *cert = a.cert_out + (size_t)qp * a.cert_stride;
      for (int e = tid; e < n * BT; e += nthr) {
        const double d = p.dx[e];
        cert[e / BT] = (unscale ? p.Dsc[e] * d : d) / norm_dx;
      }
    }
  }
  sync();
  const bool was_done = done && !just_done;
  if (tid < BT) {
    p.iscal[IS_DONE * BT + b] = done; p.iscal[IS_STATUS * BT + b] = status;
    p.iscal[IS_RHO_UPDATES * BT + b] = rho_updates;
    if (!was_done) { p.iscal[IS_NEED_REFACTOR * BT + b] = need_refactor; p.iscal[IS_CUR * BT + b] = iter; }
    p.dscal[DS_RHO * BT + b] = rho;
  }
  int ev = (just_done ? 1 : 0) | (need_refactor ? 2 : 0);
  if constexpr (BT > 1) ev = (__syncthreads_or(ev & 1) ? 1 : 0) | (__syncthreads_or(ev & 2) ? 2 : 0);
  return ev;
}
template <int BT, int NT, bool GX, bool WIDE = false>
__global__ __launch_bounds__(NT) void check_kernel(KernelArgs a) {
  extern __shared__ double smem[];
  (void)check_body<BT, NT, GX, WIDE>(a, smem, a.iter_end - a.iter_begin);
}

struct AdvanceArgs {
  int max_segments, seg_len;
  int *host_is;
  double *host_ds;
  unsigned *stop;
  unsigned seq;
  unsigned *counter;
  unsigned *host_done;
};
template <int BT, int NT, bool RS = false>
__global__ __launch_bounds__(NT) void advance_kernel(KernelArgs a, AdvanceArgs v) {
  extern __shared__ double smem[];
  const int tile = blockIdx.x, tid = threadIdx.x;
  int *is = a.iscal + (size_t)tile * IS_COUNT * BT;
  if (tid < BT && __hip_atomic_load(&is[IS_PENDING * BT + tid], __ATOMIC_ACQUIRE, __HIP_MEMORY_SCOPE_AGENT) == 1) {
    is[IS_PENDING * BT + tid] = 0; is[IS_DONE * BT + tid] = 0;
  }
  __syncthreads();
  bool iterated = false;
  for (int sgm = 0; sgm < v.max_segments; sgm++) {
    const int done = tid < BT ? is[IS_DONE * BT + tid] : 1;
    if (__syncthreads_and(done)) break;
    iterated = true;
    iterate_body<BT, NT, false, false, RS>(a, smem, v.seg_len);
    const int ev = check_body<BT, NT, false>(a, smem, v.seg_len);
    if ((ev & 1) && v.stop && tid == 0) __hip_atomic_store(v.stop, v.seq, __ATOMIC_RELAXED, __HIP_MEMORY_SCOPE_AGENT);
    if (ev & 2) {
      __syncthreads();
      if (tid < BT && is[IS_NEED_REFACTOR * BT + tid] == 1 && !is[IS_DONE * BT + tid]) { is[IS_DONE * BT + tid] = 1; is[IS_PENDING * BT + tid] = 2; }
    }
    if (v.stop && sgm + 1 < v.max_segments) {
      const unsigned sw = __hip_atomic_load(v.stop, __ATOMIC_RELAXED, __HIP_MEMORY_SCOPE_AGENT);
      if (__syncthreads_or(sw == v.seq)) break;
    }
    __syncthreads();
  }
  if (!v.host_is) return;
  __syncthreads();
  if (tid < IS_COUNT * BT) v.host_is[(size_t)tile * IS_COUNT * BT + tid] = is[tid];
  if (v.host_ds && tid < DS_COUNT * BT) v.host_ds[(size_t)tile * DS_COUNT * BT + tid] = a.dscal[(size_t)tile * DS_COUNT * BT + tid];
  __threadfence_system();
  __syncthreads();
  if (tid == 0 && v.counter) {
    if (iterated) __hip_atomic_fetch_add(v.counter + 1, 1u, __ATOMIC_RELAXED, __HIP_MEMORY_SCOPE_AGENT);
    const unsigned left = __hip_atomic_fetch_add(v.counter, 1u, __ATOMIC_ACQ_REL, __HIP_MEMORY_SCOPE_AGENT) + 1u;
    if (left == gridDim.x) {
      const unsigned active = __hip_atomic_load(v.counter + 1, __ATOMIC_RELAXED, __HIP_MEMORY_SCOPE_AGENT);
      __hip_atomic_store(v.counter, 0u, __ATOMIC_RELAXED, __HIP_MEMORY_SCOPE_AGENT);
      __hip_atomic_store(v.counter + 1, 0u, __ATOMIC_RELAXED, __HIP_MEMORY_SCOPE_AGENT);
      v.host_done[1] = active;
      __threadfence_system();
      __hip_atomic_store(v.host_done, v.seq, __ATOMIC_RELEASE, __HIP_MEMORY_SCOPE_SYSTEM);
    }
  }
}


template <int BT, int NT, bool GX, bool WIDE = false>
__global__ __launch_bounds__(NT) void spmv_kernel(KernelArgs a, const double *__restrict__ gx,
                                                    const double *__restrict__ gy, double *gPx,
                                                    double *gAty, double *gAx) {
  extern __shared__ double smem[];
  const int tile = blockIdx.x, tid = threadIdx.x, nthr = blockDim.x;
  const int lane = tid & 63, wave = __builtin_amdgcn_readfirstlane(tid >> 6);
  const int n = a.n, m = a.m;
  double *lds_rest;
  double *xs = solve_vector<BT, GX>(a, smem, tile, lds_rest);
  const TilePtrs<BT> p = tile_ptrs<BT>(a, tile);
  double *res = a.op_out_lds ? smem + (size_t)(n + m) * BT : p.out1;
  for (int bb = 0; bb < BT; bb++) {
    const int q = tile * BT + bb;
    const bool ok = q < a.B;
// ... 1437 lines not shown
    return hipGetLastError();
  };
  const int slots = (a.k / 16 - 4 + MI_TAIL_NW - 1) / MI_TAIL_NW;
  if (slots <= 1) return go(&tail_kernel<1, 4>);
  if (slots == 2) return go(&tail_kernel<2, 4>);
  if (slots == 3) return go(&tail_kernel<3, 4>);
  return go(&tail_kernel<4, 4>);
}


__global__ void interleave_kernel(const double *__restrict__ src, double *dst, const int *ids, int nq,
                                  int len, int BT) {
  const size_t g = (size_t)blockIdx.x * blockDim.x + threadIdx.x;
  if (g >= (size_t)nq * len) return;
  const int j = (int)(g / len), i = (int)(g % len);
  const int q = ids ? ids[j] : j;
  dst[((size_t)(q / BT) * len + i) * BT + (q % BT)] = src[g];
}
__global__ void scatter_kernel(const double *__restrict__ src, double *dst, const int *__restrict__ map,
                               const int *ids, int nq, int srclen, SchedDev sd, int BT) {
  const size_t g = (size_t)blockIdx.x * blockDim.x + threadIdx.x;
  const uint32_t slots = sd.n_slots;
  if (g >= (size_t)nq * slots) return;
  const int j = (int)(g / slots);
  const uint32_t s = (uint32_t)(g % slots);
  const int q = ids ? ids[j] : j;
  dst[(size_t)q * slots + s] = slot_value(map[s], src + (size_t)j * srclen, 1, 0);
  (void)BT;
}
__global__ void deinterleave_kernel(const double *__restrict__ src, double *dst, int nq, int len, int BT) {
  const size_t g = (size_t)blockIdx.x * blockDim.x + threadIdx.x;
  if (g >= (size_t)nq * len) return;
  const int q = (int)(g / len), i = (int)(g % len);
  dst[g] = src[((size_t)(q / BT) * len + i) * BT + (q % BT)];
}
__global__ void gather_status_kernel(const int *__restrict__ iscal, int32_t *status, int32_t *iters, int B, int BT) {
  const int q = blockIdx.x * blockDim.x + threadIdx.x;
  if (q >= B) return;
  const int *t = iscal + (size_t)(q / BT) * IS_COUNT * BT;
  if (status) status[q] = t[IS_STATUS * BT + q % BT];
  if (iters) iters[q] = t[IS_ITER * BT + q % BT];
}
__global__ void fail_slots_kernel(KernelArgs a, const int *__restrict__ slots, int BT, int iter) {
  const int slot = slots[blockIdx.x], tid = threadIdx.x, nthr = blockDim.x;
  if (slot < 0) return;
  const size_t tile = (size_t)slot / BT, b = (size_t)slot % BT;
  const int qp = slot < a.B ? slot : -1;
  const double nanv = __builtin_nan("");
  for (int i = tid; i < a.n; i += nthr) {
    a.x[(tile * a.n + i) * BT + b] = 0.0;
    if (qp >= 0) a.x_out[(size_t)qp * a.n + i] = nanv;
  }
  for (int j = tid; j < a.m; j += nthr) {
    a.z[(tile * a.m + j) * BT + b] = 0.0; a.y[(tile * a.m + j) * BT + b] = 0.0;
    if (qp >= 0) a.y_out[(size_t)qp * a.m + j] = nanv;
  }
  if (tid == 0) {
    int *is = a.iscal + tile * IS_COUNT * BT;
    is[IS_DONE * BT + b] = 1; is[IS_STATUS * BT + b] = -7; is[IS_NEED_REFACTOR * BT + b] = 0; is[IS_ITER * BT + b] = iter;
    double *ds = a.dscal + tile * DS_COUNT * BT;
    ds[DS_OBJ * BT + b] = nanv; ds[DS_PRI_RES * BT + b] = nanv; ds[DS_DUA_RES * BT + b] = nanv;
  }
}
hipError_t launch_fail_slots(const KernelArgs &a, const int *slots, int nfail, int BT, int iter, hipStream_t st) {
  if (!nfail) return hipSuccess;
  hipLaunchKernelGGL(fail_slots_kernel, dim3(nfail), dim3(256), 0, st, a, slots, BT, iter);
  return hipGetLastError();
}
__device__ __forceinline__ void fail_one_slot(const KernelArgs &a, int slot, int BT, int iter, int tid, int nthr) {
  const size_t tile = (size_t)slot / BT, b = (size_t)slot % BT;
  const double nanv = __builtin_nan("");
  for (int i = tid; i < a.n; i += nthr) { a.x[(tile * a.n + i) * BT + b] = 0.0; if (slot < a.B) a.x_out[(size_t)slot * a.n + i] = nanv; }
  for (int j = tid; j < a.m; j += nthr) {
    a.z[(tile * a.m + j) * BT + b] = 0.0; a.y[(tile * a.m + j) * BT + b] = 0.0;
    if (slot < a.B) a.y_out[(size_t)slot * a.m + j] = nanv;
  }
  if (tid == 0) {
    int *is = a.iscal + tile * IS_COUNT * BT;
    is[IS_DONE * BT + b] = 1; is[IS_STATUS * BT + b] = -7; is[IS_ITER * BT + b] = iter;
    double *ds = a.dscal + tile * DS_COUNT * BT;
    ds[DS_OBJ * BT + b] = nanv; ds[DS_PRI_RES * BT + b] = nanv; ds[DS_DUA_RES * BT + b] = nanv;
  }
}
__global__ void fail_flagged_kernel(KernelArgs a, const int *__restrict__ slots, int BT, int iter) {
  const int slot = slots[blockIdx.x];
  if (slot < 0) return;
  int *flag = a.iscal + ((size_t)slot / BT) * IS_COUNT * BT + IS_NEED_REFACTOR * BT + (size_t)slot % BT;
  if (*flag >= 0) return;
  fail_one_slot(a, slot, BT, iter, threadIdx.x, blockDim.x);
  __syncthreads();
  if (threadIdx.x == 0) *flag = 0;
}
hipError_t launch_fail_flagged(const KernelArgs &a, const int *slots, int nslots, int BT, int iter, hipStream_t st) {
  if (nslots <= 0) return hipSuccess;
  hipLaunchKernelGGL(fail_flagged_kernel, dim3(nslots), dim3(256), 0, st, a, slots, BT, iter);
  return hipGetLastError();
}
__global__ void start_slots_kernel(KernelArgs a, const int *__restrict__ slots, const int *__restrict__ clear, int BT, int cold) {
  const int slot = slots[blockIdx.x], tid = threadIdx.x, nthr = blockDim.x;
  if (slot < 0) return;
  const size_t tile = (size_t)slot / BT, b = (size_t)slot % BT;
  int *is = a.iscal + tile * IS_COUNT * BT;
  if (is[IS_NEED_REFACTOR * BT + b] < 0) {
    fail_one_slot(a, slot, BT, 0, tid, nthr);
    __syncthreads();
    if (tid == 0) { is[IS_PENDING * BT + b] = 0; __threadfence_system(); is[IS_EPOCH * BT + b] += 1; }
    return;
  }
  if (cold) {
    for (int i = tid; i < a.n; i += nthr) a.x[(tile * a.n + i) * BT + b] = 0.0;
    for (int j = tid; j < a.m; j += nthr) { a.z[(tile * a.m + j) * BT + b] = 0.0; a.y[(tile * a.m + j) * BT + b] = 0.0; }
  }
  __syncthreads();
  if (tid == 0) {
    is[IS_STATUS * BT + b] = -10; is[IS_ITER * BT + b] = 0; is[IS_NEED_REFACTOR * BT + b] = 0;
    is[IS_CUR * BT + b] = 0;
    if (clear[blockIdx.x]) is[IS_RHO_UPDATES * BT + b] = 0;
    __threadfence();
    __hip_atomic_store(&is[IS_PENDING * BT + b], 1, __ATOMIC_RELEASE, __HIP_MEMORY_SCOPE_AGENT);
    __threadfence();
    is[IS_EPOCH * BT + b] += 1;
  }
}
hipError_t launch_start_slots(const KernelArgs &a, const int *slots, const int *clear, int nslots, int BT, int cold, hipStream_t st) {
  if (!nslots) return hipSuccess;
  hipLaunchKernelGGL(start_slots_kernel, dim3(nslots), dim3(256), 0, st, a, slots, clear, BT, cold);
  return hipGetLastError();
}
__global__ void fresh_slots_kernel(KernelArgs a, const int *__restrict__ slots, int BT, double rho0) {
  const int slot = slots[blockIdx.x], tid = threadIdx.x, nthr = blockDim.x;
  if (slot < 0) return;
  const size_t tile = (size_t)slot / BT, b = (size_t)slot % BT;
  for (int i = tid; i < a.n; i += nthr) { a.x[(tile * a.n + i) * BT + b] = 0.0; a.dx[(tile * a.n + i) * BT + b] = 0.0; }
  for (int j = tid; j < a.m; j += nthr) { a.z[(tile * a.m + j) * BT + b] = 0.0; a.y[(tile * a.m + j) * BT + b] = 0.0; a.dy[(tile * a.m + j) * BT + b] = 0.0; }
  if (tid == 0) {
    int *is = a.iscal + tile * IS_COUNT * BT;
    is[IS_STATUS * BT + b] = -10; is[IS_ITER * BT + b] = 0; is[IS_RHO_UPDATES * BT + b] = 0; is[IS_DONE * BT + b] = 1;
    is[IS_NEED_REFACTOR * BT + b] = 0; is[IS_CUR * BT + b] = 0; is[IS_PENDING * BT + b] = 0;
    double *ds = a.dscal + tile * DS_COUNT * BT;
    ds[DS_RHO * BT + b] = rho0; ds[DS_RHO_EST * BT + b] = rho0; ds[DS_PRI_RES * BT + b] = 0.0; ds[DS_DUA_RES * BT + b] = 0.0; ds[DS_OBJ * BT + b] = 0.0;
  }
}
hipError_t launch_fresh_slots(const KernelArgs &a, const int *slots, int nslots, int BT, double rho0, hipStream_t st) {
  if (!nslots) return hipSuccess;
  hipLaunchKernelGGL(fresh_slots_kernel, dim3(nslots), dim3(256), 0, st, a, slots, BT, rho0);
  return hipGetLastError();
}
__global__ void set_rho_slots_kernel(KernelArgs a, const int *__restrict__ slots, const double *__restrict__ rho, double rho_all, int nslots, int BT) {
  const int j = (int)(blockIdx.x * blockDim.x + threadIdx.x);
  if (j >= nslots) return;
  const int slot = slots ? slots[j] : j;
  if (slot < 0) return;
  const size_t tile = (size_t)slot / BT, b = (size_t)slot % BT;
  a.dscal[(tile * DS_COUNT + DS_RHO) * BT + b] = rho ? rho[j] : rho_all;
}
hipError_t launch_set_rho_slots(const KernelArgs &a, const int *slots, const double *rho, double rho_all, int nslots, int BT, hipStream_t st) {
  if (nslots <= 0) return hipSuccess;
  hipLaunchKernelGGL(set_rho_slots_kernel, dim3((nslots + 255) / 256), dim3(256), 0, st, a, slots, rho, rho_all, nslots, BT);
  return hipGetLastError();
}
__global__ __launch_bounds__(1024) void worklist_kernel(const int *__restrict__ iscal, int *work, int nslots, int BT) {
  __shared__ int s_cnt;
  if (threadIdx.x == 0) s_cnt = 0;
  for (int s = threadIdx.x; s < nslots; s += blockDim.x) work[s] = -1;
  __syncthreads();
  for (int s = threadIdx.x; s < nslots; s += blockDim.x)
    if (iscal[(size_t)(s / BT) * IS_COUNT * BT + IS_NEED_REFACTOR * BT + s % BT] == 1) work[atomicAdd(&s_cnt, 1)] = s;
}
hipError_t launch_worklist(const int *iscal, int *work, int nslots, int BT, hipStream_t st) {
  hipLaunchKernelGGL(worklist_kernel, dim3(1), dim3(1024), 0, st, iscal, work, nslots, BT);
  return hipGetLastError();
}
__global__ void resume_flagged_kernel(KernelArgs a, int BT) {
  const int slot = blockIdx.x, tid = threadIdx.x, nthr = blockDim.x;
  const size_t tile = (size_t)slot / BT, b = (size_t)slot % BT;
  int *is = a.iscal + tile * IS_COUNT * BT;
  if (is[IS_PENDING * BT + b] != 2) return;
  const int flag = is[IS_NEED_REFACTOR * BT + b];
  if (flag == 1) return;
  if (flag < 0) fail_one_slot(a, slot, BT, is[IS_CUR * BT + b], tid, nthr);
  __syncthreads();
  __threadfence();
  if (tid == 0) __hip_atomic_store(&is[IS_PENDING * BT + b], flag < 0 ? 0 : 1, __ATOMIC_RELEASE, __HIP_MEMORY_SCOPE_AGENT);
}
hipError_t launch_resume_flagged(const KernelArgs &a, int nslots, int BT, hipStream_t st) {
  if (!nslots) return hipSuccess;
  hipLaunchKernelGGL(resume_flagged_kernel, dim3(nslots), dim3(64), 0, st, a, BT);
  return hipGetLastError();
}
__global__ void copy_slot_streams_kernel(double *dst, const double *__restrict__ src, const int *__restrict__ slots, size_t per) {
  const int slot = slots[blockIdx.y];
  if (slot < 0) return;
  const size_t off = (size_t)slot * per;
  for (size_t e = (size_t)blockIdx.x * blockDim.x + threadIdx.x; e < per; e += (size_t)gridDim.x * blockDim.x) dst[off + e] = src[off + e];
}
__global__ void copy_flagged_streams_kernel(double *dst, const double *__restrict__ src, const int *__restrict__ flags, int want, size_t per) {
  const int slot = blockIdx.y;
  if (flags && (flags[slot] != 0) != (want != 0)) return;
  const size_t off = (size_t)slot * per;
  for (size_t e = (size_t)blockIdx.x * blockDim.x + threadIdx.x; e < per; e += (size_t)gridDim.x * blockDim.x) dst[off + e] = src[off + e];
}
hipError_t launch_copy_flagged_streams(double *dst, const double *src, const int *flags, int want, int nslots, size_t per, hipStream_t st) {
  if (!nslots || !per) return hipSuccess;
  const unsigned gx = (unsigned)std::min<size_t>(64, (per + 1023) / 1024);
  hipLaunchKernelGGL(copy_flagged_streams_kernel, dim3(gx, nslots), dim3(256), 0, st, dst, src, flags, want, per);
  return hipGetLastError();
}
hipError_t launch_copy_slot_streams(double *dst, const double *src, const int *slots, int nslots, size_t per, hipStream_t st) {
  if (!nslots || !per) return hipSuccess;
  const unsigned gx = (unsigned)std::min<size_t>(64, (per + 255) / 256);
  hipLaunchKernelGGL(copy_slot_streams_kernel, dim3(gx, nslots), dim3(256), 0, st, dst, src, slots, per);
  return hipGetLastError();
}
__global__ void copy_slot_rows_kernel(double *dst, const double *__restrict__ src, const int *__restrict__ slots, int len, int BT) {
  const int slot = slots[blockIdx.y];
  if (slot < 0) return;
  const size_t base = (size_t)(slot / BT) * len * BT + slot % BT;
  for (int i = blockIdx.x * blockDim.x + threadIdx.x; i < len; i += gridDim.x * blockDim.x) dst[base + (size_t)i * BT] = src[base + (size_t)i * BT];
}
hipError_t launch_copy_slot_rows(double *dst, const double *src, const int *slots, int nslots, int len, int BT, hipStream_t st) {
  if (!nslots || !len) return hipSuccess;
  const unsigned gx = (unsigned)std::min(16, (len + 255) / 256);
  hipLaunchKernelGGL(copy_slot_rows_kernel, dim3(gx, nslots), dim3(256), 0, st, dst, src, slots, len, BT);
  return hipGetLastError();
}
__global__ void keep_rows_kernel(double *__restrict__ dst, const double *__restrict__ src, const int *__restrict__ ids, int len) {
  const int j = blockIdx.y;
  const size_t to = (size_t)ids[j] * len, from = (size_t)j * len;
  for (int i = blockIdx.x * blockDim.x + threadIdx.x; i < len; i += gridDim.x * blockDim.x) dst[to + i] = src[from + i];
}
hipError_t launch_keep_rows(double *dst, const double *src, const int *ids, int n_ids, int len, hipStream_t st) {
  if (!n_ids || !len) return hipSuccess;
  const unsigned gx = (unsigned)std::min(16, (len + 255) / 256);
  hipLaunchKernelGGL(keep_rows_kernel, dim3(gx, n_ids), dim3(256), 0, st, dst, src, ids, len);
  return hipGetLastError();
}
__global__ void bounds_kernel(const double *__restrict__ gl, const double *__restrict__ gu, double *l, double *u,
                              const double *__restrict__ Esc, const double *__restrict__ rho_vec,
                              const double *__restrict__ dscal, int *changed, int B, int m, int BT, int scaling) {
  const size_t g = (size_t)blockIdx.x * blockDim.x + threadIdx.x;
  if (g >= (size_t)B * m) return;
  const int q = (int)(g / m), i = (int)(g % m);
  const size_t e = ((size_t)(q / BT) * m + i) * BT + (q % BT);
  double lo = fmax(gl[g], -MI_INFTY), up = fmin(gu[g], MI_INFTY);
  if (lo > up) { atomicOr(changed, 2); return; }
  if (scaling) { lo *= Esc[e]; up *= Esc[e]; }
  l[e] = lo; u[e] = up;
  const double rho = dscal[((size_t)(q / BT) * DS_COUNT + DS_RHO) * BT + (q % BT)];
  double want;
  if (lo < -MI_INFTY * MI_MIN_SCALING && up > MI_INFTY * MI_MIN_SCALING) want = MI_RHO_MIN;
  else if (up - lo < 1e-4) want = 1e3 * rho;
  else want = rho;
  if (want != rho_vec[e]) atomicOr(changed, 1);
// ... 718 lines not shown
```

### osqp-solver_amd/csrc/solver.hip

```cpp
#include <hip/hip_runtime.h>
#include <time.h>

#include <algorithm>
#include <atomic>
#include <chrono>
#include <cmath>
#include <condition_variable>
#include <functional>
#include <limits>
#include <cstdio>
#include <cstdlib>
#include <cstring>
#include <string>
#include <thread>
#include <map>
#include <memory>
#include <mutex>
#include <vector>

#include "../../include/mi_osqp.h"
#include "device_types.h"
#include "host_core.hpp"

using namespace miosqp;
// ... 202 lines not shown
    return 0;
  }
  void free() { if (p && !devpool::give(dev, p, cap)) (void)hipFree(p); p = nullptr; n = 0; cap = 0; }
  ~DevBuf() { free(); }
};

struct SchedBufs {
  DevBuf<uint32_t> step, idxw, lvl_pos, tail_bar;
  DevBuf<uint64_t> idxw64;
  DevBuf<int32_t> src;
  int upload(const Schedule &s) {
    int rc;
    if ((rc = step.upload(s.step)) || (rc = idxw.upload(s.idxw)) || (rc = idxw64.upload(s.idxw64)) || (rc = src.upload(s.src)) ||
        (rc = lvl_pos.upload(s.lvl_pos)) || (rc = tail_bar.upload(s.tail_bar))) return rc;
    return 0;
  }
  SchedDev view(const Schedule &s) const {
    SchedDev d; d.step = step.p; d.idxw = idxw.p; d.idxw64 = idxw64.p; d.lvl_pos = lvl_pos.p; d.tail_bar = tail_bar.p;
    d.n_phases = s.n_phases; d.nw = s.nw; d.n_levels = s.n_levels;
    d.n_steps = s.n_steps; d.n_slots = s.n_slots;
    return d;
  }
};

struct mi_osqp_batch {
  Settings st;
  bool rho_interval_auto = false;
  Tuning tune;
  std::shared_ptr<const Analysis> anp;
  int B = 0, BT = 1, ntiles = 0, threads = 512, device = 0, n_cus = 256;
  size_t lds = 0;
  size_t lds_iter = 0;
  int rs_off = 0;
  size_t lds_factor = 0;
  int rf_off = 0, rf_steps = 0;
  int64_t rf_launches[3] = {0, 0, 0};
  std::vector<QPNumeric> qp;
  bool host_bounds_stale = false;
  hipStream_t stream = nullptr;
  SchedBufs fwd, bwd, chk;
  DevBuf<uint32_t> pinv, xloc;
  DevBuf<double> fwd_val, bwd_val, chk_val, dinv, x, z, y, q, l, u, rho_vec, rho_inv, Dsc, Dsc_inv, Esc, Esc_inv;
  DevBuf<double> dx, dy, out1, out2, dscal, x_out, y_out, xs_global;
  DevBuf<double> cert_out;
  bool global_xs = false;
  int mw_groups = 0, mw_threads = 0;
  DevBuf<uint32_t> mw_bar;
  DevBuf<unsigned char> rflag;
  DevBuf<double> mw_scratch;
  DevBuf<double> fwd_val0, bwd_val0, dinv0, rho_vec0, rho_inv0, dscal0;
  DevBuf<int> use_work;
  DevBuf<int> iscal, flag, npos;
  DevBuf<uint32_t> bf_blk, bf_lvl, bf_utask, bf_tri, bf_dtask, bf_ttask, bf_asm_dst, bf_asm_src, bf_ubig;
  DevBuf<int32_t> fwd_srcblk, bwd_srcblk;
  DevBuf<double> pa_val, Lblk, Dl, dinv_scratch;
  DevBuf<uint32_t> dt_task, dt_wave_task, dt_wave_step, dt_tail_bar;
  DevBuf<uint32_t> dt_lt_pos, dt_ltcol_col, dt_tile_tab, dt_wave_tiles, dt_diag_tile, dt_task_step;
  DevBuf<uint64_t> dt_asm_q64;
  DevBuf<int32_t> dt_src_tile;
  int dt_nh = 0; uint32_t dt_cs_doubles = 0; size_t dt_lds = 0, dt_lds_asm = 0;
  DevBuf<int32_t> dt_src;
  DevBuf<double> dt_val, dt_val0, dt_Sd;
  DevBuf<uint32_t> sp_ptr, sp_ent;
  DevBuf<uint32_t> sp_ell, sp_rowid;
  int sp_npass = 0;
  uint32_t sp_ell_off[4] = {0, 0, 0, 0}, sp_ell_k[4] = {0, 0, 0, 0};
  bool host_rho_stale = false;
  bool host_scaling_stale = false;
  DevBuf<int32_t> rz_prow, rz_pcol, rz_arow, rz_acol;
  bool clear_rho_updates = true;
  int *h_npos = nullptr;
  DevBuf<double> stage; DevBuf<int> ids, work;
  int *h_iscal = nullptr;
  double *h_dscal = nullptr;
  size_t h_iscal_cap = 0, h_dscal_cap = 0, h_npos_cap = 0, pin_cap = 0;
  double *pin = nullptr;
  size_t pin_n = 0;
  hipEvent_t ev0 = nullptr, ev1 = nullptr, evf0 = nullptr, evf1 = nullptr, evf2 = nullptr;
  hipStream_t pipe_r = nullptr, pipe_i = nullptr, pipe_x = nullptr;
  hipEvent_t pipe_ev[streampool::kPipeEvents] = {};
  DevBuf<int> tile_list;
  int64_t pipelined_refactors = 0;
  int64_t refactor_lanes = 0;
  double factor_ms_sum = 0.0, dense_ms_sum = 0.0;
  int64_t refactor_launches = 0, refactor_qps = 0, peak_qps = 0;
  double peak_factor_ms = 0.0, peak_tail_ms = 0.0;
  mi_osqp_stats stats{};
  int64_t last_total_iters = 0, last_launches = 0, last_refactors = 0;
  double last_device_s = 0.0, last_refactor_s = 0.0, kernel_ms_sum = 0.0;
  int64_t kernel_launches = 0, kernel_qp_iters = 0;
  bool solved_once = false;
  std::vector<char> failed;
  DevBuf<int> fail_list;
  DevBuf<double> rawP, rawq;
  DevBuf<double> pol_fwd, pol_bwd, pol_dinv, pol_dt, pol_sol;
  DevBuf<signed char> pol_act;
  DevBuf<int> pol_stat;
  std::vector<int> pol_status;
  int64_t pol_count = 0, pol_accepted = 0;
  double pol_seconds = 0.0;
  hipEvent_t evp0 = nullptr, evp1 = nullptr;
  DevBuf<int> adj_stat;
  struct Cont {
    bool on = false;
    int L = 25;
    unsigned launch_seq = 0;
    DevBuf<unsigned> stop;
    int64_t adv_seq = 0, polled_seq = 0;
    std::vector<char> running, clear_rho;
    std::vector<mi_osqp_info> info;
    int n_running = 0;
    int *h_is[2] = {nullptr, nullptr}; double *h_ds[2] = {nullptr, nullptr}; size_t h_is_cap[2] = {0, 0}, h_ds_cap[2] = {0, 0};
    hipEvent_t ev[2] = {nullptr, nullptr}; int64_t seq_of[2] = {0, 0};
    double *xh = nullptr, *yh = nullptr; size_t xh_cap = 0, yh_cap = 0;
    double *ch = nullptr; size_t ch_cap = 0;
    std::vector<int> cert_status;
    char *ring_h = nullptr; size_t ring_cap = 0, ring_h_cap = 0, ring_head = 0;
    int64_t ring_wraps = 0;
    DevBuf<char> ring_d;
    DevBuf<int> work;
    hipEvent_t ev_adv = nullptr;
    std::vector<int> epoch;
    DevBuf<double> rz_scratch;
    double *keepA = nullptr, *keepl = nullptr, *keepu = nullptr;
    DevBuf<unsigned> counter;
    unsigned *h_done = nullptr; size_t h_done_cap = 0;
    std::vector<char> polishable, polishing;
    std::vector<int> pol_status;
    int *h_pstat = nullptr; size_t h_pstat_cap = 0;
  } cont;
  ~mi_osqp_batch() {
    DevGuard guard(device);
    if (stream) (void)hipStreamSynchronize(stream);
    for (int k = 0; k < 2; k++) { hostpool::give(cont.h_is[k], cont.h_is_cap[k]); hostpool::give(cont.h_ds[k], cont.h_ds_cap[k]); if (cont.ev[k]) (void)hipEventDestroy(cont.ev[k]); }
    hostpool::give(cont.xh, cont.xh_cap); hostpool::give(cont.yh, cont.yh_cap); hostpool::give(cont.ch, cont.ch_cap); hostpool::give(cont.ring_h, cont.ring_h_cap);
    if (cont.ev_adv) (void)hipEventDestroy(cont.ev_adv);
    if (evp0) (void)hipEventDestroy(evp0);
    if (evp1) (void)hipEventDestroy(evp1);
    hostpool::give(cont.h_done, cont.h_done_cap); hostpool::give(cont.h_pstat, cont.h_pstat_cap);
    hostpool::give(h_iscal, h_iscal_cap); hostpool::give(h_dscal, h_dscal_cap); hostpool::give(pin, pin_cap); hostpool::give(h_npos, h_npos_cap);
    if (pipe_r) (void)hipStreamSynchronize(pipe_r);
    if (pipe_i) (void)hipStreamSynchronize(pipe_i);
    if (pipe_x) (void)hipStreamSynchronize(pipe_x);
    streampool::Bundle sb{device, stream, {ev0, ev1, evf0, evf1, evf2}, pipe_r, pipe_i, pipe_x, {}};
    for (int k = 0; k < streampool::kPipeEvents; k++) sb.pipe_ev[k] = pipe_ev[k];
    if (stream && ev0 && ev1 && evf0 && evf1 && evf2) streampool::give(sb);
    else streampool::destroy(sb);
  }
};

struct mi_osqp_solver { mi_osqp_batch *b = nullptr; };


static Settings to_settings(const mi_osqp_settings *s) {
  Settings t;
  if (!s) return t;
  t.rho = s->rho; t.sigma = s->sigma; t.scaling = s->scaling; t.adaptive_rho = s->adaptive_rho;
  t.adaptive_rho_interval = s->adaptive_rho_interval; t.adaptive_rho_tolerance = s->adaptive_rho_tolerance;
  t.max_iter = s->max_iter; t.eps_abs = s->eps_abs; t.eps_rel = s->eps_rel; t.eps_prim_inf = s->eps_prim_inf;
  t.eps_dual_inf = s->eps_dual_inf; t.alpha = s->alpha; t.scaled_termination = s->scaled_termination;
  t.check_termination = s->check_termination; t.warm_start = s->warm_start; t.verbose = s->verbose;
  t.polish = s->polish; t.polish_refine_iter = s->polish_refine_iter; t.delta = s->delta;
  return t;
}

static void dense_tail_deal_stats(const DenseTail &dt, mi_osqp_stats &s) {
  s.dense_tail_tasks = s.dense_tail_waves_used = s.dense_tail_wave_tasks_max = 0;
  if (!dt.k) return;
  s.dense_tail_tasks = (int64_t)dt.task.size() / 4;
  for (int w = 0; w < dt.nw; w++) {
    const int64_t c = (int64_t)dt.wave_task[w + 1] - (int64_t)dt.wave_task[w];
    s.dense_tail_waves_used += c > 0; s.dense_tail_wave_tasks_max = std::max(s.dense_tail_wave_tasks_max, c);
  }
}

static size_t lds_bytes(int N, int BT, int threads) {
  int nw = threads / 64;
  return ((size_t)N * BT + (size_t)nw * 14 * BT + 14 * BT) * sizeof(double);
}

static KernelArgs make_args(mi_osqp_batch *h) {
  KernelArgs a{};
  a.n = (*h->anp).n; a.m = (*h->anp).m; a.N = (*h->anp).N; a.B = h->B;
  a.fwd = h->fwd.view((*h->anp).fwd); a.bwd = h->bwd.view((*h->anp).bwd); a.chk = h->chk.view((*h->anp).chk);
  a.pinv = h->pinv.p; a.xloc = h->xloc.p;
  a.fwd_val = h->fwd_val.p; a.bwd_val = h->bwd_val.p; a.chk_val = h->chk_val.p; a.dinv = h->dinv.p;
  a.fwd_val0 = h->fwd_val0.p; a.bwd_val0 = h->bwd_val0.p; a.dt_val0 = h->dt_val0.p;
  a.use_work = (h->fwd_val0.p && h->bwd_val0.p && (!(*h->anp).dt.k || h->dt_val0.p)) ? h->use_work.p : nullptr;
  a.x = h->x.p; a.z = h->z.p; a.y = h->y.p; a.q = h->q.p; a.l = h->l.p; a.u = h->u.p;
  a.rho_vec = h->rho_vec.p; a.rho_inv = h->rho_inv.p; a.Dsc = h->Dsc.p; a.Dsc_inv = h->Dsc_inv.p;
  a.Esc = h->Esc.p; a.Esc_inv = h->Esc_inv.p; a.dx = h->dx.p; a.dy = h->dy.p; a.out1 = h->out1.p; a.out2 = h->out2.p;
  a.dscal = h->dscal.p; a.iscal = h->iscal.p;
  a.x_out = h->x_out.p; a.y_out = h->y_out.p;
  a.cert_out = h->cert_out.p; a.cert_stride = (int)std::max<int64_t>(std::max<int64_t>(a.n, a.m), 1);
  a.xs_global = h->global_xs ? h->xs_global.p : nullptr; a.xs_len = (*h->anp).xs_total; a.wide = (*h->anp).wide ? 1 : 0;
  a.rs_off = h->rs_off; a.rf_off = h->rf_off;
  a.rf_form = iterate_form(h->ntiles, h->rf_off != 0, h->tune);
  a.mw_groups = h->mw_groups; a.mw_bar = h->mw_bar.p; a.mw_scratch = h->mw_scratch.p;
  a.df = (*h->anp).df ? 1 : 0; a.df_shadow = (unsigned)(*h->anp).Next; a.rflag = h->rflag.p;
  {
    const DenseTail &dt = (*h->anp).dt;
    a.dt.s = dt.s; a.dt.k = dt.k; a.dt.n_phases = dt.n_phases; a.dt.n_steps = dt.n_steps;
    a.dt.task = h->dt_task.p; a.dt.wave_task = h->dt_wave_task.p; a.dt.wave_step = h->dt_wave_step.p; a.dt.tail_bar = h->dt_tail_bar.p;
    a.dt_val = h->dt_val.p;
  }
  const Settings &s = h->st;
  a.sigma = s.sigma; a.alpha = s.alpha; a.eps_abs = s.eps_abs; a.eps_rel = s.eps_rel;
  a.eps_prim_inf = s.eps_prim_inf; a.eps_dual_inf = s.eps_dual_inf; a.rho_tolerance = s.adaptive_rho_tolerance;
  a.check_termination = (int)s.check_termination; a.rho_interval = (int)s.adaptive_rho_interval;
  a.max_iter = (int)s.max_iter; a.scaled_termination = (int)s.scaled_termination; a.scaling = s.scaling ? 1 : 0;
  a.adaptive_rho = (int)s.adaptive_rho; a.iter_begin = 0; a.iter_end = 0; a.info_at_end = 1;
  return a;
}

static FactorArgs make_factor_args(mi_osqp_batch *h, int force_all) {
  FactorArgs a{};
  const Analysis &an = (*h->anp);
  a.n = an.n; a.m = an.m; a.N = an.N; a.B = h->B; a.nnzP = an.Pp[an.n]; a.nnzK = an.nnzK();
  a.pa_len = an.Pp[an.n] + an.Ap[an.n]; a.n_levels = an.bf.n_levels; a.force_all = force_all;
  a.storage = an.bf.storage; a.fwd = h->fwd.view(an.fwd); a.bwd = h->bwd.view(an.bwd);
  a.blk = h->bf_blk.p; a.lvl = h->bf_lvl.p; a.utask = h->bf_utask.p; a.tri4 = h->bf_tri.p; a.dtask = h->bf_dtask.p; a.ubig = h->bf_ubig.p;
  a.ttask = h->bf_ttask.p; a.asm_dst = h->bf_asm_dst.p; a.asm_src = h->bf_asm_src.p;
  a.fwd_srcblk = h->fwd_srcblk.p; a.bwd_srcblk = h->bwd_srcblk.p;
// ... 746 lines not shown
  if (!h->evp1) HIPCHK(hipEventCreate(&h->evp1));
  return MI_OSQP_OK;
}

static constexpr int kPolishInner = 4;

static int polish_impl(mi_osqp_batch *h, const KernelArgs &a) {
  const int BT = h->BT, ntl = h->ntiles;
  int rc;
  h->pol_count = h->pol_accepted = 0; h->pol_seconds = 0.0;
  h->pol_status.assign((size_t)h->B, 0);
  if ((rc = ensure_polish_buffers(h))) return rc;
  std::vector<int> work = koptimal_slots(h);
  PolishArgs pa{h->pol_stat.p, h->pol_act.p, h->pol_sol.p, (int)h->st.polish_refine_iter, kPolishInner, h->st.delta};
  HIPCHK(hipEventRecord(h->evp0, h->stream));
  HIPCHK(launch_polish_active(a, pa, BT, h->stream));
  const int n_pol = (int)work.size();
  if (n_pol) {
    if ((rc = device_refactor_slots(h, std::move(work), nullptr, &pa))) return rc;
    if ((rc = run_spinning(h, h->stream, [&]() -> int {
          HIPCHK(launch_polish(polish_stream_args(h, a), pa, BT, ntl, h->mw_groups > 0 ? h->mw_threads : h->threads, h->lds, h->n_cus, h->stream));
          HIPCHK(hipEventRecord(h->evp1, h->stream));
          return MI_OSQP_OK;
        }))) return rc;
  } else {
    HIPCHK(hipEventRecord(h->evp1, h->stream));
  }
  HIPCHK(hipMemcpyAsync(h->pol_status.data(), h->pol_stat.p, (size_t)h->B * sizeof(int), hipMemcpyDeviceToHost, h->stream));
  HIPCHK(hipStreamSynchronize(h->stream));
  float ms = 0.f;
  HIPCHK(hipEventElapsedTime(&ms, h->evp0, h->evp1));
  h->pol_seconds = ms * 1e-3;
  h->pol_count = n_pol;
  for (int v : h->pol_status) h->pol_accepted += v == 1;
  return MI_OSQP_OK;
}

static int adjoint_impl(mi_osqp_batch *h, const AdjointArgs &ga, int32_t *d_status, hipStream_t user_stream) {
  hipStream_t keep = h->stream;
  struct Restore { mi_osqp_batch *h; hipStream_t s; ~Restore() { h->stream = s; } } restore{h, keep};
  if (user_stream) h->stream = user_stream;
  const Analysis &an = (*h->anp);
  const int BT = h->BT, ntl = h->ntiles;
  int rc;
  if ((rc = ensure_polish_buffers(h))) return rc;
  if (!h->adj_stat.p && ((rc = h->adj_stat.alloc((size_t)ntl * BT)))) return rc;
  if ((rc = h->adj_stat.zero(h->stream))) return rc;
  std::vector<int> work;
  if (h->solved_once) {
    HIPCHK(hipMemcpyAsync(h->h_iscal, h->iscal.p, (size_t)ntl * IS_COUNT * BT * sizeof(int), hipMemcpyDeviceToHost, h->stream));
    HIPCHK(hipStreamSynchronize(h->stream));
    work = koptimal_slots(h);
  }
  if (!work.empty()) {
    const KernelArgs a = make_args(h);
    PolishArgs pa{h->adj_stat.p, h->pol_act.p, h->pol_sol.p, (int)h->st.polish_refine_iter};
    HIPCHK(launch_polish_active(a, pa, BT, h->stream));
    if ((rc = device_refactor_slots(h, std::move(work), nullptr, &pa))) return rc;
    if ((rc = run_spinning(h, h->stream, [&]() -> int {
          HIPCHK(launch_adjoint(polish_stream_args(h, a), pa, ga, BT, ntl, h->mw_groups > 0 ? h->mw_threads : h->threads, h->lds, h->n_cus, h->stream));
          return MI_OSQP_OK;
        }))) return rc;
  }
  HIPCHK(launch_adjoint_finish(h->adj_stat.p, ga, d_status, h->B, an.n, an.m, h->stream));
  HIPCHK(hipStreamSynchronize(h->stream));
  return MI_OSQP_OK;
}

struct PipeRegion {
  bool open = false;
  int iter = 0, n_chunks = 0, n_lanes = 1;
  bool tail = false;
  double host_s = 0.0;
  std::vector<int> work, wl, tiles;
  std::vector<int> lane_last;
};
constexpr int kDefaultLanes = 2;
constexpr bool kDefaultChunk0First = false;
static bool pipeline_applies(const mi_osqp_batch *h, int n_ref) {
  const int longer_than = h->tune.pipeline_min > 0 ? h->tune.pipeline_min : h->n_cus;
  return h->tune.refactor_pipeline && n_ref > longer_than && h->mw_groups <= 0 && !h->global_xs && !(*h->anp).wide && !(*h->anp).df;
}

static int pipelined_refactor_iterate(mi_osqp_batch *h, const KernelArgs &a, const std::vector<int> &work, const std::vector<int> &active, PipeRegion *pr) {
  using streampool::kPipeChunks; using streampool::kPipeEvents; using streampool::kPipeLanes;
  const double t_begin = now_s();
  const int BT = h->BT, nq = (int)work.size();
  int rc;
  if (!h->pipe_r) HIPCHK(hipStreamCreateWithFlags(&h->pipe_r, hipStreamNonBlocking));
  if (!h->pipe_i) HIPCHK(hipStreamCreateWithFlags(&h->pipe_i, hipStreamNonBlocking));
  for (int k = 0; k < kPipeEvents; k++) if (!h->pipe_ev[k]) HIPCHK(hipEventCreate(&h->pipe_ev[k]));
  hipEvent_t ev_fork = h->pipe_ev[0], ev_i0 = h->pipe_ev[1], ev_join = h->pipe_ev[2];
  auto ev_chunk = [&](int c, int k) { return h->pipe_ev[3 + 3 * (c - 1) + k]; };
  auto ev_lane = [&](int l) { return h->pipe_ev[3 + 3 * kPipeChunks + l]; };
  int n_even = h->tune.pipeline_chunks > 0 ? h->tune.pipeline_chunks : (nq + h->n_cus - 1) / h->n_cus;
  int chunk_qps = (nq + n_even - 1) / n_even;
  if (h->tune.pipeline_chunks <= 0 && h->tune.pipeline_chunk_qps > 0) chunk_qps = h->tune.pipeline_chunk_qps;
  const RefactorChunks ch = refactor_chunks(work, active, BT, chunk_qps, kPipeChunks);
  const int kbt = nq <= h->n_cus ? 1 : BT;
  const int lanes_asked = h->tune.refactor_lanes > 0 ? h->tune.refactor_lanes : kDefaultLanes;
  const RefactorLanes rl = refactor_lanes(ch, work, BT, kbt, std::min(lanes_asked, kPipeLanes), h->tune.lanes_chunk0 < 0 ? kDefaultChunk0First : h->tune.lanes_chunk0 != 0,
                                          h->ntiles * BT + 4);
  const int L = rl.n_lanes;
  if (L > 2 && !h->pipe_x) HIPCHK(hipStreamCreateWithFlags(&h->pipe_x, hipStreamNonBlocking));
  std::vector<int> &wl = pr->wl;
  std::vector<int> wl_begin(1, 0);
  wl.clear();
  for (int c = 1; c < ch.n_chunks; c++) {
    wl.insert(wl.end(), work.begin() + ch.work_begin[c], work.begin() + ch.work_begin[c + 1]);
    wl.resize((wl.size() + kbt - 1) / kbt * kbt, -1);
    wl_begin.push_back((int)wl.size());
  }
  pr->tiles = ch.tiles; pr->work = work;
  if (h->work.n < wl.size() && (rc = h->work.alloc((size_t)h->ntiles * BT + 4 + (size_t)BT * kPipeChunks))) return rc;
  if (h->tile_list.n < ch.tiles.size() && (rc = h->tile_list.alloc((size_t)h->ntiles))) return rc;
  HIPCHK(hipMemcpyAsync(h->work.p, wl.data(), wl.size() * sizeof(int), hipMemcpyHostToDevice, h->stream));
  HIPCHK(hipMemcpyAsync(h->tile_list.p, pr->tiles.data(), pr->tiles.size() * sizeof(int), hipMemcpyHostToDevice, h->stream));
  pr->host_s = now_s() - t_begin;
  HIPCHK(hipEventRecord(ev_fork, h->stream));
  FactorArgs fa = make_factor_args(h, 0);
  const bool tail = (*h->anp).dt.k != 0;
  auto enqueue_refactor = [&](int c, int base, hipStream_t st) -> int {
    const int *wc = h->work.p + wl_begin[c - 1];
    const int slots = wl_begin[c] - wl_begin[c - 1];
    fa.work = wc; fa.wg_base = base / kbt;
    HIPCHK(hipEventRecord(ev_chunk(c, 0), st));
    HIPCHK(launch_factor(fa, kbt, slots / kbt, h->tune.factor_threads, st));
    HIPCHK(hipEventRecord(ev_chunk(c, 1), st));
    if (tail) {
      TailArgs da = make_tail_args(h, kbt, wc);
      da.wg_base = base;
      HIPCHK(launch_tail(da, slots, h->dt_lds_asm, h->dt_lds, st));
    }
    HIPCHK(hipEventRecord(ev_chunk(c, 2), st));
    return 0;
  };
  KernelArgs ai = a;
  auto enqueue_iterate = [&](int c, hipStream_t st) -> int {
    const int nt = ch.tile_begin[c + 1] - ch.tile_begin[c];
    if (!nt) return 0;
    ai.tiles = h->tile_list.p + ch.tile_begin[c];
    ai.rf_form = iterate_form(nt, h->rf_off != 0, h->tune);
    h->rf_launches[ai.rf_form]++;
    HIPCHK(launch_iterate(ai, BT, nt, h->threads, h->lds_iter + h->lds_factor, st));
    return 0;
  };
  pr->lane_last.assign(L, 0);
  if (L == 1) {
    HIPCHK(hipStreamWaitEvent(h->pipe_r, ev_fork, 0));
    HIPCHK(hipStreamWaitEvent(h->pipe_i, ev_fork, 0));
    for (int c = 1; c < ch.n_chunks; c++) if ((rc = enqueue_refactor(c, 0, h->pipe_r))) return rc;
    pr->lane_last[0] = ch.n_chunks - 1;
    HIPCHK(hipEventRecord(ev_i0, h->pipe_i));
    for (int c = 0; c < ch.n_chunks; c++) {
      if (c) HIPCHK(hipStreamWaitEvent(h->pipe_i, ev_chunk(c, 2), 0));
      if ((rc = enqueue_iterate(c, h->pipe_i))) return rc;
    }
    HIPCHK(hipEventRecord(ev_lane(0), h->pipe_i));
    HIPCHK(hipStreamWaitEvent(h->stream, ev_lane(0), 0));
  } else {
    hipStream_t lane[kPipeLanes] = {h->pipe_r, h->pipe_i, h->pipe_x};
    for (int l = 0; l < L; l++) HIPCHK(hipStreamWaitEvent(lane[l], ev_fork, 0));
    const bool chunk0_first = rl.order[rl.lane_of[0]].front() == 0;
    if (chunk0_first && (rc = enqueue_iterate(0, lane[rl.lane_of[0]]))) return rc;
    size_t w = 0;
    for (int c = 1; c < ch.n_chunks; c++) {
      const int l = rl.lane_of[c];
      if ((rc = enqueue_refactor(c, rl.scratch_begin[c], lane[l]))) return rc;
      pr->lane_last[l] = c;
      for (; w < rl.wait_chunk.size() && rl.wait_chunk[w] == c; w++) HIPCHK(hipStreamWaitEvent(lane[l], ev_chunk(rl.wait_for[w], 2), 0));
      if ((rc = enqueue_iterate(c, lane[l]))) return rc;
    }
    if (!chunk0_first && (rc = enqueue_iterate(0, lane[rl.lane_of[0]]))) return rc;
    for (int l = 0; l < L; l++) { HIPCHK(hipEventRecord(ev_lane(l), lane[l])); HIPCHK(hipStreamWaitEvent(h->stream, ev_lane(l), 0)); }
  }
  HIPCHK(hipEventRecord(ev_join, h->stream));
  HIPCHK(launch_fail_flagged(a, h->work.p, (int)wl.size(), BT, a.iter_begin, h->stream));
  pr->open = true; pr->iter = a.iter_begin; pr->n_chunks = ch.n_chunks; pr->n_lanes = L; pr->tail = tail;
  h->refactor_lanes = std::max<int64_t>(h->refactor_lanes, L);
  return 0;
}

static int pipelined_region_finish(mi_osqp_batch *h, PipeRegion *pr) {
  using streampool::kPipeChunks;
  if (!pr->open) return 0;
  pr->open = false;
  const int BT = h->BT, nq = (int)pr->work.size();
  hipEvent_t ev_fork = h->pipe_ev[0], ev_i0 = h->pipe_ev[1], ev_join = h->pipe_ev[2];
  auto ev_chunk = [&](int c, int k) { return h->pipe_ev[3 + 3 * (c - 1) + k]; };
  float f_ms = 0.f, d_ms = 0.f, r_ms = 0.f, i_ms = 0.f, w_ms = 0.f;
  for (int c = 1; c < pr->n_chunks; c++) {
    float f = 0.f, d = 0.f;
    HIPCHK(hipEventElapsedTime(&f, ev_chunk(c, 0), ev_chunk(c, 1))); HIPCHK(hipEventElapsedTime(&d, ev_chunk(c, 1), ev_chunk(c, 2)));
    f_ms += f; d_ms += pr->tail ? d : 0.f;
  }
  for (int c : pr->lane_last) {
    float r = 0.f;
    if (c) HIPCHK(hipEventElapsedTime(&r, ev_fork, ev_chunk(c, 2)));
    r_ms = std::max(r_ms, r);
  }
  HIPCHK(hipEventElapsedTime(&w_ms, ev_fork, ev_join));
  if (pr->n_lanes == 1) HIPCHK(hipEventElapsedTime(&i_ms, ev_i0, h->pipe_ev[3 + 3 * kPipeChunks])); else i_ms = w_ms;
  const double wall = pr->host_s + 1e-3 * std::max(w_ms, r_ms), ref_s = pr->host_s + 1e-3 * r_ms;
  h->last_refactor_s += ref_s; h->last_device_s += wall - ref_s;
  h->kernel_ms_sum += i_ms; h->kernel_launches++; h->last_launches++;
  h->factor_ms_sum += f_ms; h->dense_ms_sum += d_ms; h->refactor_launches++; h->refactor_qps += nq;
  if (nq >= h->peak_qps) { h->peak_qps = nq; h->peak_factor_ms = f_ms; h->peak_tail_ms = d_ms; }
  h->pipelined_refactors++;
  for (int s : pr->work)
    if (s >= 0 && s < h->B && h->h_iscal[(size_t)(s / BT) * IS_COUNT * BT + IS_STATUS * BT + s % BT] == -7) h->failed[s] = 1;
  return 0;
}

static int solve_impl(mi_osqp_batch *h, double *d_x_out, hipStream_t user_stream) {
  hipStream_t keep = h->stream;
  struct Restore { mi_osqp_batch *h; hipStream_t s; ~Restore() { h->stream = s; } } restore{h, keep};
  if (user_stream) h->stream = user_stream;
  int rc;
  if ((rc = reset_solve_state(h, !h->st.warm_start))) return rc;
  KernelArgs a = make_args(h);
  if (d_x_out) a.x_out = d_x_out;
  h->last_total_iters = h->last_launches = h->last_refactors = 0;
  h->last_device_s = h->last_refactor_s = 0.0;
  const int BT = h->BT, ntl = h->ntiles, nslots = ntl * BT;
  const Settings &S = h->st;
  int iterating = ntl;
  {
    std::vector<int> bad;
    for (int q = 0; q < h->B; q++) if (h->failed[q]) bad.push_back(q);
    if ((rc = fail_slots(h, a, bad, 0))) return rc;
  }
  auto segment_end = [&](int iter) {
    int seg_end = (int)S.max_iter;
    if (S.check_termination > 0) seg_end = std::min<int64_t>(seg_end, (iter / S.check_termination + 1) * S.check_termination);
    if (S.adaptive_rho && S.adaptive_rho_interval > 0)
      seg_end = std::min<int64_t>(seg_end, (iter / S.adaptive_rho_interval + 1) * S.adaptive_rho_interval);
    return seg_end;
  };
  auto loop = [&]() -> int {
    int iter = 0;
    bool iterated = false;
    PipeRegion region;
    while (true) {
      const int seg_end = segment_end(iter);
      a.iter_begin = iter; a.iter_end = seg_end; a.info_at_end = 1;
      {
        std::unique_lock<std::mutex> spin_lock(spin_mutex(h->device), std::defer_lock);
        if (h->mw_groups > 0) spin_lock.lock();
        if (!iterated) {
          HIPCHK(hipEventRecord(h->ev0, h->stream));
          if (h->mw_groups > 0) HIPCHK(hipMemsetAsync(h->mw_bar.p, 0, 4 * sizeof(uint32_t), h->stream));
          a.rf_form = iterate_form(iterating, h->rf_off != 0, h->tune);
          h->rf_launches[a.rf_form]++;
          HIPCHK(launch_iterate(a, BT, ntl, h->mw_groups > 0 ? h->mw_threads : h->threads, h->lds_iter + h->lds_factor, h->stream));
          HIPCHK(hipEventRecord(h->ev1, h->stream));
        }
        {
          int chk_threads = h->mw_groups > 0 ? h->mw_threads : h->threads;
          if (h->mw_groups <= 0 && h->threads == 1024 && ntl > 2 * h->n_cus) chk_threads = 512;
          HIPCHK(launch_check(a, BT, ntl, chk_threads, h->lds, h->stream));
        }
        HIPCHK(hipMemcpyAsync(h->h_iscal, h->iscal.p, (size_t)ntl * IS_COUNT * BT * sizeof(int), hipMemcpyDeviceToHost, h->stream));
        HIPCHK(hipStreamSynchronize(h->stream));
      }
      if ((rc = mw_barrier_ok(h))) {
        const std::string why = g_last_error;
        (void)restore_snapshot(h);
        g_last_error = why + " (the handle is back in the state of its last setup / update, cold-started)";
        return rc;
      }
      if (!iterated) {
        float ms = 0.f;
        HIPCHK(hipEventElapsedTime(&ms, h->ev0, h->ev1));
        h->last_device_s += ms * 1e-3; h->kernel_ms_sum += ms; h->kernel_launches++; h->last_launches++;
      } else if ((rc = pipelined_region_finish(h, &region))) return rc;
      iterated = false;
      iter = seg_end;
      std::vector<int> active, work;
      for (int s = 0; s < h->B; s++) {
        const int *t = h->h_iscal + (size_t)(s / BT) * IS_COUNT * BT;
        if (!t[IS_DONE * BT + s % BT]) active.push_back(s);
        if (t[IS_NEED_REFACTOR * BT + s % BT]) work.push_back(s);
      }
      const int n_ref = (int)work.size();
      if (active.empty() && !n_ref) break;
      if (n_ref) {
        double tr = now_s();
        std::vector<int> bad;
        int rc2;
        if (!active.empty() && pipeline_applies(h, n_ref)) {
          KernelArgs nx = a;
          nx.iter_begin = iter; nx.iter_end = segment_end(iter); nx.info_at_end = 1;
          if ((rc2 = pipelined_refactor_iterate(h, nx, work, active, &region))) return rc2;
          iterated = true;
          tr = now_s();
        } else if ((rc2 = device_refactor_slots(h, std::move(work), &bad))) return rc2;
        if ((rc2 = fail_slots(h, a, bad, iter))) return rc2;
        h->host_rho_stale = true;
        h->last_refactors += n_ref;
        h->last_refactor_s += now_s() - tr;
        if (!bad.empty()) {
          std::vector<char> isbad(nslots, 0);
          for (int q : bad) isbad[q] = 1;
          active.erase(std::remove_if(active.begin(), active.end(), [&](int q) { return isbad[q] != 0; }), active.end());
        }
      }
      if (active.empty()) break;
      iterating = 0;
      for (size_t i = 0; i < active.size(); i++) iterating += !i || active[i] / BT != active[i - 1] / BT;
    }
    return MI_OSQP_OK;
  };
  rc = loop();
  if (rc) {
    if (h->pipe_r) (void)hipStreamSynchronize(h->pipe_r);
    if (h->pipe_i) (void)hipStreamSynchronize(h->pipe_i);
    if (h->pipe_x) (void)hipStreamSynchronize(h->pipe_x);
    (void)hipStreamSynchronize(h->stream);
    return rc;
  }
  HIPCHK(hipMemcpyAsync(h->h_iscal, h->iscal.p, (size_t)nslots * IS_COUNT * sizeof(int), hipMemcpyDeviceToHost, h->stream));
  HIPCHK(hipStreamSynchronize(h->stream));
  for (int qi = 0; qi < h->B; qi++)
    h->last_total_iters += h->h_iscal[(size_t)(qi / BT) * IS_COUNT * BT + IS_ITER * BT + qi % BT];
  h->solved_once = true;
  if (h->st.polish && (rc = polish_impl(h, a))) return rc;
  if (!h->st.polish) { h->pol_status.clear(); h->pol_count = h->pol_accepted = 0; }
  return MI_OSQP_OK;
}


extern "C" {

void mi_osqp_default_settings(mi_osqp_settings *s) {
  if (!s) return;
  s->rho = 0.1; s->sigma = 1e-6; s->scaling = 10; s->adaptive_rho = 1; s->adaptive_rho_interval = 0;
  s->adaptive_rho_tolerance = 5.0; s->max_iter = 4000; s->eps_abs = 1e-3; s->eps_rel = 1e-3;
  s->eps_prim_inf = 1e-4; s->eps_dual_inf = 1e-4; s->alpha = 1.6; s->scaled_termination = 0;
  s->check_termination = 25; s->warm_start = 1; s->verbose = 0;
  s->polish = 0; s->polish_refine_iter = 3; s->delta = 1e-6;
}

const char *mi_osqp_exit_code_name(int64_t c) {
  static const char *names[] = {"kOptimal", "kPrimalInfeasible", "kDualInfeasible", "kOptimalInaccurate",
                                "kPrimalInfeasibleInaccurate", "kDualInfeasibleInaccurate", "kMaxIterations",
                                "kInterrupted", "kTimeLimitReached", "kNonConvex", "kUnknown"};
  return (c >= 0 && c <= 10) ? names[c] : "kUnknown";
}
const char *mi_osqp_error_name(int64_t e) {
  static const char *names[] = {"ok", "invalid data", "invalid settings", "sparsity pattern changed",
                                "non-convex problem / KKT inertia", "device error", "null argument", "allocation / size"};
  return (e >= 0 && e <= 7) ? names[e] : "unknown";
}
const char *mi_osqp_version(void) { return "mi-osqp 0.2 (gfx950)"; }
const char *mi_osqp_last_error(void) { return g_last_error.c_str(); }

static int64_t exit_code_of(int status) {
  switch (status) {
    case 1: return MI_OSQP_EXIT_OPTIMAL;
    case 2: return MI_OSQP_EXIT_OPTIMAL_INACCURATE;
    case -3: return MI_OSQP_EXIT_PRIMAL_INFEASIBLE;
    case 3: return MI_OSQP_EXIT_PRIMAL_INFEASIBLE_INACCURATE;
    case -4: return MI_OSQP_EXIT_DUAL_INFEASIBLE;
    case 4: return MI_OSQP_EXIT_DUAL_INFEASIBLE_INACCURATE;
    case -2: return MI_OSQP_EXIT_MAX_ITERATIONS;
    case -5: return MI_OSQP_EXIT_INTERRUPTED;
    case -6: return MI_OSQP_EXIT_TIME_LIMIT_REACHED;
    case -7: return MI_OSQP_EXIT_NON_CONVEX;
    default: return MI_OSQP_EXIT_UNKNOWN;
  }
}

int mi_osqp_batch_setup(mi_osqp_batch **out, int64_t B, int64_t n, int64_t m, const int64_t *Pp, const int64_t *Pi,
                        const double *Pv, const double *q, const int64_t *Ap, const int64_t *Ai, const double *Av,
                        const double *l, const double *u, const mi_osqp_settings *settings, int64_t device) {
  CallTimer timer_("batch_setup");
  if (!out) return MI_OSQP_ERR_NULL;
  *out = nullptr;
  if (n <= 0 || m < 0) return MI_OSQP_ERR_INVALID_DATA;
  mi_osqp_batch *h = new (std::nothrow) mi_osqp_batch();
  if (!h) return MI_OSQP_ERR_ALLOC;
  h->st = to_settings(settings);
  int rc = batch_setup_impl(h, B, n, m, Pp, Pi, Pv, q, Ap, Ai, Av, l, u, device);
  if (rc) { delete h; return rc; }
  *out = h;
  return MI_OSQP_OK;
}

int mi_osqp_prefetch_analysis(int64_t B, int64_t n, int64_t m, const int64_t *Pp, const int64_t *Pi, const int64_t *Ap, const int64_t *Ai, int64_t device) {
  CallTimer timer_("prefetch_analysis");
  if (B <= 0 || n <= 0 || m < 0 || !Pp || !Ap || (Pp[n] > 0 && !Pi) || (Ap[n] > 0 && !Ai)) return MI_OSQP_ERR_INVALID_DATA;
  mi_osqp_batch tmp;
  tmp.tune = tuning_from_env();
  int BT = 1, max_extra = -1;
  std::shared_ptr<const Analysis> an;
  return shape_and_analysis(&tmp, B, n, m, Pp, Pi, Ap, Ai, device, BT, max_extra, an);
// ... 110 lines not shown
  if (!h || !act) return MI_OSQP_ERR_NULL;
  const size_t cnt = (size_t)h->B * (*h->anp).m;
  if (!h->pol_act.p) { memset(act, 0, cnt); return MI_OSQP_OK; }
  DevGuard guard(h->device);
  if (h->cont.on) HIPCHK(hipStreamSynchronize(h->stream));
  if (cnt) HIPCHK(hipMemcpy(act, h->pol_act.p, cnt, hipMemcpyDeviceToHost));
  return MI_OSQP_OK;
}

static AdjointArgs adjoint_args(mi_osqp_batch *h, const double *d_dx, const double *d_dy, double *d_dq, double *d_dP, double *d_dA,
                                double *d_dl, double *d_du) {
  const Analysis &an = (*h->anp);
  AdjointArgs ga{};
  ga.gx = d_dx; ga.gy = d_dy; ga.dq = d_dq; ga.dP = d_dP; ga.dA = d_dA; ga.dl = d_dl; ga.du = d_du;
  ga.prow = h->rz_prow.p; ga.pcol = h->rz_pcol.p; ga.arow = h->rz_arow.p; ga.acol = h->rz_acol.p;
  ga.nnzP = (int)an.Pp[an.n]; ga.nnzA = (int)an.Ap[an.n];
  return ga;
}
int mi_osqp_batch_adjoint_device(mi_osqp_batch *h, const double *d_dx, const double *d_dy, double *d_dq, double *d_dP, double *d_dA,
                                 double *d_dl, double *d_du, int32_t *d_status, void *stream) {
  CallTimer timer_("batch_adjoint_device");
  if (!h) return MI_OSQP_ERR_NULL;
  if (!d_dx) { g_last_error = "adjoint: dx is null (dL/dx is required; only dy may be null)"; return MI_OSQP_ERR_NULL; }
  for (const double *o : {(const double *)d_dq, (const double *)d_dP, (const double *)d_dA, (const double *)d_dl, (const double *)d_du})
    if (o && (o == d_dx || o == d_dy)) { g_last_error = "adjoint: an output aliases dx or dy"; return MI_OSQP_ERR_INVALID_DATA; }
  DevGuard guard(h->device);
  { const int rc_ = cont_leave(h); if (rc_) return rc_; }
  return adjoint_impl(h, adjoint_args(h, d_dx, d_dy, d_dq, d_dP, d_dA, d_dl, d_du), d_status, (hipStream_t)stream);
}
int mi_osqp_batch_adjoint(mi_osqp_batch *h, const double *dx, const double *dy, double *dq, double *dP, double *dA, double *dl,
                          double *du, int32_t *status) {
  CallTimer timer_("batch_adjoint");
  if (!h) return MI_OSQP_ERR_NULL;
  if (!dx) { g_last_error = "adjoint: dx is null (dL/dx is required; only dy may be null)"; return MI_OSQP_ERR_NULL; }
  DevGuard guard(h->device);
  { const int rc_ = cont_leave(h); if (rc_) return rc_; }
  const Analysis &an = (*h->anp);
  const size_t B = (size_t)h->B, n = (size_t)an.n, m = (size_t)an.m, nnzP = (size_t)an.Pp[an.n], nnzA = (size_t)an.Ap[an.n];
  const size_t len[7] = {B * n, dy ? B * m : 0, dq ? B * n : 0, dP ? B * nnzP : 0, dA ? B * nnzA : 0, dl ? B * m : 0, du ? B * m : 0};
  size_t off[8] = {0};
  for (int k = 0; k < 7; k++) off[k + 1] = off[k] + len[k];
  DevBuf<double> buf;
  DevBuf<int> stat;
  int rc;
  if ((rc = buf.alloc(off[7])) || (rc = stat.alloc(B))) return rc;
  auto at = [&](int k) -> double * { return len[k] ? buf.p + off[k] : nullptr; };
  HIPCHK(hipMemcpy(at(0), dx, len[0] * sizeof(double), hipMemcpyHostToDevice));
  if (len[1]) HIPCHK(hipMemcpy(at(1), dy, len[1] * sizeof(double), hipMemcpyHostToDevice));
  if ((rc = adjoint_impl(h, adjoint_args(h, at(0), at(1), at(2), at(3), at(4), at(5), at(6)), stat.p, nullptr))) return rc;
  double *out[7] = {nullptr, nullptr, dq, dP, dA, dl, du};
  for (int k = 2; k < 7; k++) if (len[k]) HIPCHK(hipMemcpy(out[k], at(k), len[k] * sizeof(double), hipMemcpyDeviceToHost));
  if (status) HIPCHK(hipMemcpy(status, stat.p, B * sizeof(int32_t), hipMemcpyDeviceToHost));
  return MI_OSQP_OK;
}

int mi_osqp_batch_get_scaling(mi_osqp_batch *h, double *D, double *E, double *c) {
  if (!h || !D || !E || !c) return MI_OSQP_ERR_NULL;
  DevGuard guard(h->device);
  { const int rc_ = cont_leave(h); if (rc_) return rc_; }
  const int n = (*h->anp).n, m = (*h->anp).m, B = h->B, BT = h->BT;
  int rc;
  if ((rc = ensure_stage(h, (size_t)B * std::max({n, m, 1}) + 1, 0))) return rc;
  auto down = [&](const double *src, int len, double *dst) -> int {
    if (!len) return 0;
    HIPCHK(launch_deinterleave(src, h->stage.p, B, len, BT, h->stream));
    HIPCHK(hipMemcpyAsync(dst, h->stage.p, (size_t)B * len * sizeof(double), hipMemcpyDeviceToHost, h->stream));
    HIPCHK(hipStreamSynchronize(h->stream));
    return 0;
  };
  if ((rc = down(h->Dsc.p, n, D)) || (rc = down(h->Esc.p, m, E))) return rc;
  const size_t dcnt = (size_t)h->ntiles * DS_COUNT * BT;
  HIPCHK(hipMemcpy(h->h_dscal, h->dscal.p, dcnt * sizeof(double), hipMemcpyDeviceToHost));
  for (int q = 0; q < B; q++) c[q] = h->h_dscal[(size_t)(q / BT) * DS_COUNT * BT + DS_C * BT + q % BT];
  return MI_OSQP_OK;
}

int mi_osqp_batch_get_stats(mi_osqp_batch *h, mi_osqp_stats *st) {
  if (!h || !st) return MI_OSQP_ERR_NULL;
  *st = h->stats;
  st->pipelined_refactors = h->pipelined_refactors;
  st->refactor_lanes = h->refactor_lanes;
  st->iterate_launches_deep_ring = h->rf_launches[RF_FORM_DEEP_RING];
  st->iterate_launches_long_head = h->rf_launches[RF_FORM_LONG_HEAD];
  return MI_OSQP_OK;
}

int mi_osqp_batch_get_ordering(mi_osqp_batch *h, int64_t *kkt_perm) {
  if (!h || !kkt_perm) return MI_OSQP_ERR_NULL;
  const Analysis &an = (*h->anp);
  for (int k = 0; k < an.N; k++) kkt_perm[k] = an.perm[(size_t)k];
  return MI_OSQP_OK;
}

int mi_osqp_batch_last_solve_stats(mi_osqp_batch *h, int64_t *total_iters, int64_t *kernel_launches, double *device_seconds,
                                   double *refactor_seconds, int64_t *refactor_count, double *compact_seconds) {
  if (!h) return MI_OSQP_ERR_NULL;
  if (compact_seconds) *compact_seconds = 0.0;
  if (total_iters) *total_iters = h->last_total_iters;
  if (kernel_launches) *kernel_launches = h->last_launches;
  if (device_seconds) *device_seconds = h->last_device_s;
  if (refactor_seconds) *refactor_seconds = h->last_refactor_s;
  if (refactor_count) *refactor_count = h->last_refactors;
  return MI_OSQP_OK;
}

int mi_osqp_batch_kernel_time(mi_osqp_batch *h, double *avg_ms, int64_t *launches) {
  if (!h) return MI_OSQP_ERR_NULL;
  if (avg_ms) *avg_ms = h->kernel_launches ? h->kernel_ms_sum / (double)h->kernel_launches : 0.0;
  if (launches) *launches = h->kernel_launches;
  h->kernel_ms_sum = 0.0; h->kernel_launches = 0;
  return MI_OSQP_OK;
}

int mi_osqp_batch_refactor_time(mi_osqp_batch *h, double *factor_ms, double *dense_ms, int64_t *launches, int64_t *qps) {
  if (!h) return MI_OSQP_ERR_NULL;
  if (factor_ms) *factor_ms = h->factor_ms_sum;
  if (dense_ms) *dense_ms = h->dense_ms_sum;
  if (launches) *launches = h->refactor_launches;
  if (qps) *qps = h->refactor_qps;
  h->factor_ms_sum = h->dense_ms_sum = 0.0; h->refactor_launches = h->refactor_qps = 0;
  h->peak_qps = 0; h->peak_factor_ms = h->peak_tail_ms = 0.0;
  return MI_OSQP_OK;
}

int mi_osqp_batch_refactor_peak(mi_osqp_batch *h, int64_t *qps, double *factor_ms, double *tail_ms) {
  if (!h) return MI_OSQP_ERR_NULL;
  if (qps) *qps = h->peak_qps;
  if (factor_ms) *factor_ms = h->peak_factor_ms;
  if (tail_ms) *tail_ms = h->peak_tail_ms;
  return MI_OSQP_OK;
}

int mi_osqp_batch_reset(mi_osqp_batch *h) {
  CallTimer timer_("batch_reset");
  if (!h) return MI_OSQP_ERR_NULL;
  DevGuard guard(h->device);
  { const int rc_ = cont_leave(h); if (rc_) return rc_; }
  return restore_snapshot(h);
}
}
static int restore_snapshot(mi_osqp_batch *h) {
  h->clear_rho_updates = true;
  auto cp = [&](DevBuf<double> &dst, DevBuf<double> &src) -> int {
    if (src.n) HIPCHK(hipMemcpyAsync(dst.p, src.p, src.n * sizeof(double), hipMemcpyDeviceToDevice, h->stream));
    return 0;
  };
  int rc;
  const size_t nflags = (size_t)h->ntiles * h->BT;
  HIPCHK(hipMemsetD32Async((hipDeviceptr_t)h->use_work.p, 0, nflags, h->stream));
  if ((rc = cp(h->dinv, h->dinv0)) || (rc = cp(h->rho_vec, h->rho_vec0)) || (rc = cp(h->rho_inv, h->rho_inv0)) || (rc = cp(h->dscal, h->dscal0))) return rc;
  if ((rc = reset_solve_state(h, true))) return rc;
  HIPCHK(hipStreamSynchronize(h->stream));
  h->host_rho_stale = true;
  return MI_OSQP_OK;
}
extern "C" {

int mi_osqp_batch_warm_start_x(mi_osqp_batch *h, const double *x) {
  CallTimer timer_("batch_warm_start_x");
  if (!h || !x) return MI_OSQP_ERR_NULL;
  DevGuard guard(h->device);
  { const int rc_ = cont_leave(h); if (rc_) return rc_; }
  h->st.warm_start = 1;
  size_t cnt = (size_t)h->B * (*h->anp).n;
  int rc;
  if ((rc = ensure_stage(h, cnt, 0)) || (rc = ensure_pin(h, cnt))) return rc;
// ... 1539 lines not shown
                  const double *u, const mi_osqp_settings *settings) {
  if (!out) return MI_OSQP_ERR_NULL;
  *out = nullptr;
  mi_osqp_batch *b = nullptr;
  int rc = mi_osqp_batch_setup(&b, 1, n, m, Pp, Pi, Pv, q, Ap, Ai, Av, l, u, settings, -1);
  if (rc) return rc;
  mi_osqp_solver *s = new (std::nothrow) mi_osqp_solver();
  if (!s) { delete b; return MI_OSQP_ERR_ALLOC; }
  s->b = b; *out = s;
  return MI_OSQP_OK;
}
void mi_osqp_free(mi_osqp_solver *h) { if (h) { delete h->b; delete h; } }
int mi_osqp_update_A_bounds(mi_osqp_solver *h, const int64_t *Ap, const int64_t *Ai, const double *Av, const double *l, const double *u) {
  return h ? mi_osqp_batch_update_A_bounds(h->b, Ap, Ai, Av, l, u) : MI_OSQP_ERR_NULL;
}
int mi_osqp_update_A(mi_osqp_solver *h, const int64_t *Ap, const int64_t *Ai, const double *Av) {
  return h ? mi_osqp_batch_update_A(h->b, Ap, Ai, Av) : MI_OSQP_ERR_NULL;
}
int mi_osqp_update_bounds(mi_osqp_solver *h, const double *l, const double *u) {
  return h ? mi_osqp_batch_update_bounds(h->b, l, u) : MI_OSQP_ERR_NULL;
}
int mi_osqp_warm_start_x(mi_osqp_solver *h, const double *x) { return h ? mi_osqp_batch_warm_start_x(h->b, x) : MI_OSQP_ERR_NULL; }
int mi_osqp_update_q(mi_osqp_solver *h, const double *q) { return h ? mi_osqp_batch_update_q(h->b, q) : MI_OSQP_ERR_NULL; }
int mi_osqp_update_P(mi_osqp_solver *h, const int64_t *Pp, const int64_t *Pi, const double *Pv) {
  return h ? mi_osqp_batch_update_P(h->b, Pp, Pi, Pv) : MI_OSQP_ERR_NULL;
}
int mi_osqp_update_P_A(mi_osqp_solver *h, const int64_t *Pp, const int64_t *Pi, const double *Pv, const int64_t *Ap, const int64_t *Ai,
                       const double *Av) {
  return h ? mi_osqp_batch_update_P_A(h->b, Pp, Pi, Pv, Ap, Ai, Av) : MI_OSQP_ERR_NULL;
}
int mi_osqp_warm_start_y(mi_osqp_solver *h, const double *y) { return h ? mi_osqp_batch_warm_start_y(h->b, y) : MI_OSQP_ERR_NULL; }
int mi_osqp_solve(mi_osqp_solver *h, mi_osqp_info *info) {
  if (!h) return MI_OSQP_ERR_NULL;
  int rc = mi_osqp_batch_solve(h->b);
  if (rc) return rc;
  if (info) return mi_osqp_batch_get_info(h->b, info);
  return MI_OSQP_OK;
}
int mi_osqp_get_primal(mi_osqp_solver *h, double *x) { return h ? mi_osqp_batch_get_primal(h->b, x) : MI_OSQP_ERR_NULL; }
int mi_osqp_get_dual(mi_osqp_solver *h, double *y) { return h ? mi_osqp_batch_get_dual(h->b, y) : MI_OSQP_ERR_NULL; }
int mi_osqp_get_prim_inf_cert(mi_osqp_solver *h, double *dy_out) { return h ? mi_osqp_batch_get_prim_inf_cert(h->b, dy_out) : MI_OSQP_ERR_NULL; }
int mi_osqp_get_dual_inf_cert(mi_osqp_solver *h, double *dx_out) { return h ? mi_osqp_batch_get_dual_inf_cert(h->b, dx_out) : MI_OSQP_ERR_NULL; }
int mi_osqp_adjoint(mi_osqp_solver *h, const double *dx, const double *dy, double *dq, double *dP, double *dA, double *dl, double *du,
                    int32_t *status) {
  return h ? mi_osqp_batch_adjoint(h->b, dx, dy, dq, dP, dA, dl, du, status) : MI_OSQP_ERR_NULL;
}
int mi_osqp_debug_refactor_chunks(int64_t n_flagged, const int64_t *flagged, int64_t n_active, const int64_t *active, int64_t tile,
                                  int64_t chunk_qps, int64_t max_chunks, int64_t *n_chunks, int64_t *work_begin, int64_t *tiles,
                                  int64_t *tile_begin) {
  if (!n_chunks || !work_begin || !tiles || !tile_begin || (n_flagged > 0 && !flagged) || (n_active > 0 && !active)) return MI_OSQP_ERR_NULL;
  if (n_flagged < 0 || n_active < 0 || tile < 1 || chunk_qps < 1 || max_chunks < 1) return MI_OSQP_ERR_INVALID_DATA;
  const std::vector<int> f(flagged, flagged + n_flagged), a(active, active + n_active);
  const RefactorChunks ch = refactor_chunks(f, a, (int)tile, (int)chunk_qps, (int)max_chunks);
  *n_chunks = ch.n_chunks;
  std::copy(ch.work_begin.begin(), ch.work_begin.end(), work_begin);
  std::copy(ch.tiles.begin(), ch.tiles.end(), tiles);
  std::copy(ch.tile_begin.begin(), ch.tile_begin.end(), tile_begin);
  return MI_OSQP_OK;
}
int mi_osqp_debug_refactor_lanes(int64_t n_flagged, const int64_t *flagged, int64_t n_active, const int64_t *active, int64_t tile,
                                 int64_t chunk_qps, int64_t max_chunks, int64_t kbt, int64_t lanes, int64_t chunk0_first,
                                 int64_t scratch_slots, int64_t *n_lanes, int64_t *lane_of, int64_t *order, int64_t *order_begin,
                                 int64_t *scratch_begin, int64_t *n_waits, int64_t *wait_chunk, int64_t *wait_for) {
  if (!n_lanes || !lane_of || !order || !order_begin || !scratch_begin || !n_waits || !wait_chunk || !wait_for ||
      (n_flagged > 0 && !flagged) || (n_active > 0 && !active)) return MI_OSQP_ERR_NULL;
  if (n_flagged < 0 || n_active < 0 || tile < 1 || chunk_qps < 1 || max_chunks < 1 || kbt < 1 || lanes < 1 || lanes > 3 || scratch_slots < 0)
    return MI_OSQP_ERR_INVALID_DATA;
  const std::vector<int> f(flagged, flagged + n_flagged), a(active, active + n_active);
  const RefactorChunks ch = refactor_chunks(f, a, (int)tile, (int)chunk_qps, (int)max_chunks);
  const RefactorLanes rl = refactor_lanes(ch, f, (int)tile, (int)kbt, (int)lanes, chunk0_first != 0, (int)std::min<int64_t>(scratch_slots, INT32_MAX));
  *n_lanes = rl.n_lanes;
  std::copy(rl.lane_of.begin(), rl.lane_of.end(), lane_of);
  order_begin[0] = 0;
  for (int l = 0; l < rl.n_lanes; l++) {
    std::copy(rl.order[l].begin(), rl.order[l].end(), order + order_begin[l]);
    order_begin[l + 1] = order_begin[l] + (int64_t)rl.order[l].size();
  }
  std::copy(rl.scratch_begin.begin(), rl.scratch_begin.begin() + ch.n_chunks, scratch_begin);
  *n_waits = (int64_t)rl.wait_chunk.size();
  std::copy(rl.wait_chunk.begin(), rl.wait_chunk.end(), wait_chunk);
  std::copy(rl.wait_for.begin(), rl.wait_for.end(), wait_for);
  return MI_OSQP_OK;
}
int mi_osqp_debug_iterate_form(int64_t tiles, int64_t has_head, int64_t forced_form, int64_t long_min, int64_t *form) {
  if (!form) return MI_OSQP_ERR_NULL;
  if (tiles < 0 || tiles > INT32_MAX || forced_form < 0 || forced_form > 2 || long_min < -1 || long_min > INT32_MAX)
    return MI_OSQP_ERR_INVALID_DATA;
  Tuning t;
  t.rf_form = (int)forced_form; t.rf_long_min = (int)long_min;
  *form = iterate_form((int)tiles, has_head != 0, t);
  return MI_OSQP_OK;
}
int mi_osqp_get_stats(mi_osqp_solver *h, mi_osqp_stats *st) { return h ? mi_osqp_batch_get_stats(h->b, st) : MI_OSQP_ERR_NULL; }
int mi_osqp_get_settings(mi_osqp_solver *h, mi_osqp_settings *out) { return h ? mi_osqp_batch_get_settings(h->b, out) : MI_OSQP_ERR_NULL; }
int mi_osqp_update_settings(mi_osqp_solver *h, const mi_osqp_settings *s) { return h ? mi_osqp_batch_update_settings(h->b, s) : MI_OSQP_ERR_NULL; }


}

struct ShardWorker {
  std::thread th;
  std::mutex mu;
  std::condition_variable cv;
  std::function<int()> job;
  bool has_job = false, busy = false, quit = false;
  int rc = 0;
  std::string err;
  void start() {
    th = std::thread([this] {
      std::unique_lock<std::mutex> lk(mu);
      for (;;) {
        cv.wait(lk, [this] { return has_job || quit; });
        if (quit) return;
        std::function<int()> f = std::move(job);
        has_job = false;
        lk.unlock();
        const int r = f();
        const std::string e = r ? g_last_error : std::string();
        lk.lock();
        rc = r; err = e; busy = false;
        cv.notify_all();
      }
    });
  }
  void post(std::function<int()> f) {
    std::unique_lock<std::mutex> lk(mu);
    cv.wait(lk, [this] { return !busy; });
    job = std::move(f); has_job = true; busy = true; rc = 0; err.clear();
    cv.notify_all();
  }
  int wait(std::string &e) {
    std::unique_lock<std::mutex> lk(mu);
    cv.wait(lk, [this] { return !busy; });
    e = err;
    return rc;
  }
  ~ShardWorker() {
    { std::lock_guard<std::mutex> lk(mu); quit = true; }
    cv.notify_all();
    if (th.joinable()) th.join();
  }
};

struct mi_osqp_multi {
  int64_t B = 0, n = 0, m = 0;
  std::vector<int64_t> dev, begin;
  std::vector<mi_osqp_batch *> shard;
  std::vector<std::unique_ptr<ShardWorker>> worker;
  bool async_pending = false;
  ~mi_osqp_multi() { worker.clear(); for (mi_osqp_batch *b : shard) delete b; }
  size_t count() const { return shard.size(); }
};

static int multi_join(mi_osqp_multi *h) {
  int rc = MI_OSQP_OK;
  for (size_t k = 0; k < h->worker.size(); k++) {
    std::string e;
    const int r = h->worker[k]->wait(e);
    if (r && !rc) { rc = r; g_last_error = "shard " + std::to_string(k) + ": " + e; }
  }
  h->async_pending = false;
  return rc;
}
template <class F>
static int multi_fan_out(mi_osqp_multi *h, F &&fn) {
  const size_t ns = h->count();
// ... 237 lines not shown
```

Before: 40920.

## Run a slowest-residual tile group ahead through refactor pipeline while others iterate

Adds a run-ahead mode that picks the active tiles with the largest scaled primal plus dual residuals at a rho-update point. That group is sent through the pipelined refactor path while the remaining tiles keep iterating over an indirect tile list; its leftovers are finished in a later phase. The aim is to keep the GPU busy during refactorisation and shorten the tail of slow QPs. In exchange it adds residual readback, host sorting, extra worklist and fail-mark kernels, and more complex control flow and bookkeeping. It is on by default.

```diff
diff --git a/include/mi_osqp.h b/include/mi_osqp.h
--- a/include/mi_osqp.h
+++ b/include/mi_osqp.h
@@ -83,6 +83,7 @@
   int64_t dense_tail_tasks, dense_tail_waves_used, dense_tail_wave_tasks_max;
   int64_t refactor_lanes;
   int64_t iterate_launches_deep_ring, iterate_launches_long_head;
+  int64_t runahead_regions, runahead_tiles, runahead_left, runahead_missed;
 } mi_osqp_stats;
 
 typedef struct mi_osqp_solver mi_osqp_solver;
@@ -294,6 +295,9 @@
                                  int64_t scratch_slots, int64_t *n_lanes, int64_t *lane_of, int64_t *order, int64_t *order_begin,
                                  int64_t *scratch_begin, int64_t *n_waits, int64_t *wait_chunk, int64_t *wait_for);
 
+int mi_osqp_debug_runahead_group(int64_t n_active, const int64_t *tiles, const double *pri_res, const double *dua_res, int64_t size,
+                                 int64_t min_active, int64_t *n_group, int64_t *group);
+
 int mi_osqp_debug_iterate_form(int64_t tiles, int64_t has_head, int64_t forced_form, int64_t long_min, int64_t *form);
 
 int mi_osqp_debug_trace_kkt_solve(mi_osqp_batch *h, int32_t which, const double *d_rhs, double *d_sol,
diff --git a/osqp-solver_amd/__init__.py b/osqp-solver_amd/__init__.py
--- a/osqp-solver_amd/__init__.py
+++ b/osqp-solver_amd/__init__.py
@@ -50,7 +50,9 @@
                 ("resident_factor_steps", C.c_int64), ("lds_bytes_factor", C.c_int64),
                 ("dense_tail_tasks", C.c_int64), ("dense_tail_waves_used", C.c_int64), ("dense_tail_wave_tasks_max", C.c_int64),
                 ("refactor_lanes", C.c_int64),
-                ("iterate_launches_deep_ring", C.c_int64), ("iterate_launches_long_head", C.c_int64)]
+                ("iterate_launches_deep_ring", C.c_int64), ("iterate_launches_long_head", C.c_int64),
+                ("runahead_regions", C.c_int64), ("runahead_tiles", C.c_int64), ("runahead_left", C.c_int64),
+                ("runahead_missed", C.c_int64)]
 
     def as_dict(self):
         return {k: getattr(self, k) for k, _ in self._fields_}
@@ -190,6 +192,7 @@
                                                    C.POINTER(Settings), C.c_int64, dp, dp, dp, C.POINTER(Stats)]
         L.mi_osqp_debug_refactor_chunks.argtypes = [C.c_int64, ip, C.c_int64, ip, C.c_int64, C.c_int64, C.c_int64, ip, ip, ip, ip]
         L.mi_osqp_debug_refactor_lanes.argtypes = [C.c_int64, ip, C.c_int64, ip] + [C.c_int64] * 7 + [ip] * 8
+        L.mi_osqp_debug_runahead_group.argtypes = [C.c_int64, ip, dp, dp, C.c_int64, C.c_int64, ip, ip]
         L.mi_osqp_debug_iterate_form.argtypes = [C.c_int64] * 4 + [ip]
         L.mi_osqp_prefetch_analysis.argtypes = [C.c_int64, C.c_int64, C.c_int64, ip, ip, ip, ip, C.c_int64]
         L.mi_osqp_debug_host_block_factor.argtypes = [C.c_int64, C.c_int64, ip, ip, dp, ip, ip, dp, dp, dp,
@@ -854,6 +857,16 @@
                 waits=list(zip(wc[:nw.value].tolist(), wf[:nw.value].tolist())))
 
 
+def debug_runahead_group(tiles, pri_res, dua_res, size, min_active):
+    t, p, d = _i64(tiles), _f64(pri_res), _f64(dua_res)
+    if not (len(t) == len(p) == len(d)):
+        raise ValueError("tiles, pri_res and dua_res differ in length")
+    ng = C.c_int64()
+    out = np.zeros(max(1, len(t)), dtype=np.int64)
+    _chk(lib().mi_osqp_debug_runahead_group(len(t), _ip(t), _dp(p), _dp(d), size, min_active, C.byref(ng), _ip(out)), "debug_runahead_group")
+    return out[:ng.value].tolist()
+
+
 def debug_iterate_form(tiles, has_head=True, forced_form=0, long_min=-1):
     form = C.c_int64()
     _chk(lib().mi_osqp_debug_iterate_form(tiles, int(bool(has_head)), forced_form, long_min, C.byref(form)), "debug_iterate_form")
diff --git a/osqp-solver_amd/csrc/device_types.h b/osqp-solver_amd/csrc/device_types.h
--- a/osqp-solver_amd/csrc/device_types.h
+++ b/osqp-solver_amd/csrc/device_types.h
@@ -62,6 +62,7 @@
   const unsigned char *rflag;
   const int *sel;
   const int *tiles;
+  double *res;
 };
 
 struct FactorArgs {
@@ -188,6 +189,7 @@
 hipError_t launch_fresh_slots(const KernelArgs &a, const int *slots, int nslots, int BT, double rho0, hipStream_t st);
 hipError_t launch_set_rho_slots(const KernelArgs &a, const int *slots, const double *rho, double rho_all, int nslots, int BT, hipStream_t st);
 hipError_t launch_worklist(const int *iscal, int *work, int nslots, int BT, hipStream_t st);
+hipError_t launch_worklist_of(const int *iscal, const int *slots, int *work, int nlist, int BT, hipStream_t st);
 hipError_t launch_resume_flagged(const KernelArgs &a, int nslots, int BT, hipStream_t st);
 hipError_t launch_copy_slot_streams(double *dst, const double *src, const int *slots, int nslots, size_t per, hipStream_t st);
 hipError_t launch_keep_rows(double *dst, const double *src, const int *ids, int n_ids, int len, hipStream_t st);
@@ -216,7 +218,7 @@
 hipError_t launch_gomp_relinearise(const GompArgs &g, hipStream_t st);
 hipError_t launch_gather_status(const int *iscal, int32_t *status, int32_t *iters, int B, int BT, hipStream_t st);
 hipError_t launch_fail_slots(const KernelArgs &a, const int *slots, int nfail, int BT, int iter, hipStream_t st);
-hipError_t launch_fail_flagged(const KernelArgs &a, const int *slots, int nslots, int BT, int iter, hipStream_t st);
+hipError_t launch_fail_flagged(const KernelArgs &a, const int *slots, int nslots, int BT, int iter, hipStream_t st, int *mark = nullptr);
 hipError_t launch_bounds(const double *gl, const double *gu, double *l, double *u, const double *Esc,
                          const double *rho_vec, const double *dscal, int *changed, int B, int m, int BT,
                          int scaling, hipStream_t st);
diff --git a/osqp-solver_amd/csrc/host_core.cpp b/osqp-solver_amd/csrc/host_core.cpp
--- a/osqp-solver_amd/csrc/host_core.cpp
+++ b/osqp-solver_amd/csrc/host_core.cpp
@@ -6,6 +6,7 @@
 #include <cstdio>
 #include <cstdlib>
 #include <cstring>
+#include <limits>
 #include <numeric>
 #include <set>
 #include <chrono>
@@ -949,6 +950,10 @@
   if (const char *e = getenv("MI_OSQP_REFACTOR_CHUNK_QPS")) t.pipeline_chunk_qps = std::max(0, atoi(e));
   if (const char *e = getenv("MI_OSQP_REFACTOR_LANES")) t.refactor_lanes = std::max(1, std::min(3, atoi(e)));
   if (const char *e = getenv("MI_OSQP_REFACTOR_CHUNK0")) t.lanes_chunk0 = atoi(e) != 0;
+  if (const char *e = getenv("MI_OSQP_RUNAHEAD")) t.runahead = atoi(e) != 0;
+  if (const char *e = getenv("MI_OSQP_RUNAHEAD_TILES")) t.runahead_tiles = std::max(0, atoi(e));
+  if (const char *e = getenv("MI_OSQP_RUNAHEAD_MIN")) t.runahead_min = std::max(0, atoi(e));
+  if (const char *e = getenv("MI_OSQP_RUNAHEAD_END")) t.runahead_end = std::max(0, atoi(e));
   if (const char *e = getenv("MI_OSQP_RF_FORM")) { const int v = atoi(e); if (v == kIterDeepRing || v == kIterLongHead) t.rf_form = v; }
   if (const char *e = getenv("MI_OSQP_RF_LONG_MIN")) t.rf_long_min = std::max(0, atoi(e));
   AnalysisTuning &a = t.analysis;
@@ -1024,6 +1029,30 @@
     for (int d = 1; d < c; d++) if (need[d]) { rl.wait_chunk.push_back(c); rl.wait_for.push_back(d); }
   }
   return rl;
+}
+
+std::vector<int> runahead_group(const std::vector<int> &tiles, const std::vector<double> &pri, const std::vector<double> &dua, int size, int min_active) {
+  const size_t na = tiles.size();
+  if (!na || size <= 0 || na < (size_t)std::max(0, min_active) || pri.size() != na || dua.size() != na) return {};
+  const double inf = std::numeric_limits<double>::infinity();
+  auto scaled = [&](const std::vector<double> &r) {
+    std::vector<double> v(na);
+    for (size_t i = 0; i < na; i++) v[i] = std::isnan(r[i]) ? inf : r[i];
+    std::vector<double> s = v;
+    std::nth_element(s.begin(), s.begin() + na / 2, s.end());
+    const double med = s[na / 2];
+    for (size_t i = 0; i < na; i++) v[i] = v[i] == inf ? inf : med == inf ? 0.0 : med > 0.0 ? v[i] / med : v[i] > 0.0 ? inf : 0.0;
+    return v;
+  };
+  const std::vector<double> sp = scaled(pri), sd = scaled(dua);
+  std::vector<std::pair<double, int>> order(na);
+  for (size_t i = 0; i < na; i++) order[i] = {sp[i] + sd[i], tiles[i]};
+  std::sort(order.begin(), order.end(), [](const std::pair<double, int> &x, const std::pair<double, int> &y) {
+    return x.first > y.first || (x.first == y.first && x.second < y.second);
+  });
+  std::vector<int> group(std::min(na, (size_t)size));
+  for (size_t i = 0; i < group.size(); i++) group[i] = order[i].second;
+  return group;
 }
 
 int iterate_form(int tiles, bool has_head, const Tuning &t) {
diff --git a/osqp-solver_amd/csrc/host_core.hpp b/osqp-solver_amd/csrc/host_core.hpp
--- a/osqp-solver_amd/csrc/host_core.hpp
+++ b/osqp-solver_amd/csrc/host_core.hpp
@@ -35,6 +35,7 @@
     return dense_tail == o.dense_tail && ordering == o.ordering && nd_leaf == o.nd_leaf && relax == o.relax && serial == o.serial;
   }
 };
+constexpr bool kRunaheadDefault = true;
 struct Tuning {
   int tile = 0;
   int threads = 0;
@@ -55,6 +56,10 @@
   int pipeline_chunk_qps = 0;
   int refactor_lanes = 0;
   int lanes_chunk0 = -1;
+  bool runahead = kRunaheadDefault;
+  int runahead_tiles = 0;
+  int runahead_min = 0;
+  int runahead_end = 0;
   int rf_form = 0;
   int rf_long_min = -1;
   AnalysisTuning analysis;
@@ -81,6 +86,8 @@
   std::vector<int> wait_chunk, wait_for;
 };
 RefactorLanes refactor_lanes(const RefactorChunks &ch, const std::vector<int> &flagged, int bt, int kbt, int lanes, bool chunk0_first, int scratch_slots);
+
+std::vector<int> runahead_group(const std::vector<int> &tiles, const std::vector<double> &pri, const std::vector<double> &dua, int size, int min_active);
 
 struct Schedule {
   int n_phases = 0, nw = 0, bt = 1;
diff --git a/osqp-solver_amd/csrc/kernels.hip b/osqp-solver_amd/csrc/kernels.hip
--- a/osqp-solver_amd/csrc/kernels.hip
+++ b/osqp-solver_amd/csrc/kernels.hip
@@ -987,7 +987,7 @@
   bool dfm = false;
   if constexpr (GX && BT == 1 && WIDE) dfm = a.df != 0 && a.mw_groups > 1;
   const Mw mw{a.mw_bar, dfm ? (unsigned)a.mw_groups : 1u};
-  const int tile = dfm ? 0 : blockIdx.x;
+  const int tile = dfm ? 0 : (a.tiles ? a.tiles[blockIdx.x] : (int)blockIdx.x);
   const int ltid = threadIdx.x, lwave = __builtin_amdgcn_readfirstlane(ltid >> 6), lnw = blockDim.x >> 6;
   const int tid = dfm ? blockIdx.x * blockDim.x + threadIdx.x : threadIdx.x, nthr = dfm ? blockDim.x * mw.G : blockDim.x;
   const int lane = tid & 63, wave = __builtin_amdgcn_readfirstlane(tid >> 6), nw = nthr >> 6;
@@ -1195,6 +1195,7 @@
     p.iscal[IS_RHO_UPDATES * BT + b] = rho_updates;
     if (!was_done) { p.iscal[IS_NEED_REFACTOR * BT + b] = need_refactor; p.iscal[IS_CUR * BT + b] = iter; }
     p.dscal[DS_RHO * BT + b] = rho;
+    if (a.res && !done && qp >= 0) { a.res[2 * (size_t)qp] = pri_res; a.res[2 * (size_t)qp + 1] = dua_res; }
   }
   int ev = (just_done ? 1 : 0) | (need_refactor ? 2 : 0);
   if constexpr (BT > 1) ev = (__syncthreads_or(ev & 1) ? 1 : 0) | (__syncthreads_or(ev & 2) ? 2 : 0);
@@ -2798,18 +2799,18 @@
     ds[DS_OBJ * BT + b] = nanv; ds[DS_PRI_RES * BT + b] = nanv; ds[DS_DUA_RES * BT + b] = nanv;
   }
 }
-__global__ void fail_flagged_kernel(KernelArgs a, const int *__restrict__ slots, int BT, int iter) {
+__global__ void fail_flagged_kernel(KernelArgs a, const int *__restrict__ slots, int BT, int iter, int *mark) {
   const int slot = slots[blockIdx.x];
   if (slot < 0) return;
   int *flag = a.iscal + ((size_t)slot / BT) * IS_COUNT * BT + IS_NEED_REFACTOR * BT + (size_t)slot % BT;
   if (*flag >= 0) return;
   fail_one_slot(a, slot, BT, iter, threadIdx.x, blockDim.x);
   __syncthreads();
-  if (threadIdx.x == 0) *flag = 0;
-}
-hipError_t launch_fail_flagged(const KernelArgs &a, const int *slots, int nslots, int BT, int iter, hipStream_t st) {
+  if (threadIdx.x == 0) { *flag = 0; if (mark) mark[slot] = 1; }
+}
+hipError_t launch_fail_flagged(const KernelArgs &a, const int *slots, int nslots, int BT, int iter, hipStream_t st, int *mark) {
   if (nslots <= 0) return hipSuccess;
-  hipLaunchKernelGGL(fail_flagged_kernel, dim3(nslots), dim3(256), 0, st, a, slots, BT, iter);
+  hipLaunchKernelGGL(fail_flagged_kernel, dim3(nslots), dim3(256), 0, st, a, slots, BT, iter, mark);
   return hipGetLastError();
 }
 __global__ void start_slots_kernel(KernelArgs a, const int *__restrict__ slots, const int *__restrict__ clear, int BT, int cold) {
@@ -2885,6 +2886,29 @@
 }
 hipError_t launch_worklist(const int *iscal, int *work, int nslots, int BT, hipStream_t st) {
   hipLaunchKernelGGL(worklist_kernel, dim3(1), dim3(1024), 0, st, iscal, work, nslots, BT);
+  return hipGetLastError();
+}
+__global__ __launch_bounds__(1024) void worklist_of_kernel(const int *__restrict__ iscal, const int *__restrict__ slots, int *work, int nlist, int BT) {
+  __shared__ int s_flag[1024];
+  int cnt = 0;
+  for (int base = 0; base < nlist; base += 1024) {
+    const int j = base + (int)threadIdx.x;
+    int f = 0;
+    if (j < nlist) {
+      const int s = slots[j];
+      f = s >= 0 && iscal[(size_t)(s / BT) * IS_COUNT * BT + IS_NEED_REFACTOR * BT + s % BT] == 1;
+    }
+    s_flag[threadIdx.x] = f;
+    __syncthreads();
+    if (threadIdx.x == 0)
+      for (int k = 0; k < 1024 && base + k < nlist; k++) if (s_flag[k]) work[cnt++] = slots[base + k];
+    __syncthreads();
+  }
+  if (threadIdx.x == 0) for (int k = cnt; k < nlist; k++) work[k] = -1;
+}
+hipError_t launch_worklist_of(const int *iscal, const int *slots, int *work, int nlist, int BT, hipStream_t st) {
+  if (nlist <= 0) return hipSuccess;
+  hipLaunchKernelGGL(worklist_of_kernel, dim3(1), dim3(1024), 0, st, iscal, slots, work, nlist, BT);
   return hipGetLastError();
 }
 __global__ void resume_flagged_kernel(KernelArgs a, int BT) {
diff --git a/osqp-solver_amd/csrc/solver.hip b/osqp-solver_amd/csrc/solver.hip
--- a/osqp-solver_amd/csrc/solver.hip
+++ b/osqp-solver_amd/csrc/solver.hip
@@ -308,6 +308,11 @@
   DevBuf<int> tile_list;
   int64_t pipelined_refactors = 0;
   int64_t refactor_lanes = 0;
+  DevBuf<int> ra_list;
+  DevBuf<double> ra_res;
+  double *h_res = nullptr; int *h_mark = nullptr;
+  size_t h_res_cap = 0, h_mark_cap = 0;
+  int64_t ra_regions = 0, ra_tiles = 0, ra_left = 0, ra_missed = 0;
   double factor_ms_sum = 0.0, dense_ms_sum = 0.0;
   int64_t refactor_launches = 0, refactor_qps = 0, peak_qps = 0;
   double peak_factor_ms = 0.0, peak_tail_ms = 0.0;
@@ -365,6 +370,7 @@
     if (evp1) (void)hipEventDestroy(evp1);
     hostpool::give(cont.h_done, cont.h_done_cap); hostpool::give(cont.h_pstat, cont.h_pstat_cap);
     hostpool::give(h_iscal, h_iscal_cap); hostpool::give(h_dscal, h_dscal_cap); hostpool::give(pin, pin_cap); hostpool::give(h_npos, h_npos_cap);
+    hostpool::give(h_res, h_res_cap); hostpool::give(h_mark, h_mark_cap);
     if (pipe_r) (void)hipStreamSynchronize(pipe_r);
     if (pipe_i) (void)hipStreamSynchronize(pipe_i);
     if (pipe_x) (void)hipStreamSynchronize(pipe_x);
@@ -1277,7 +1283,31 @@
   return h->tune.refactor_pipeline && n_ref > longer_than && h->mw_groups <= 0 && !h->global_xs && !(*h->anp).wide && !(*h->anp).df;
 }
 
-static int pipelined_refactor_iterate(mi_osqp_batch *h, const KernelArgs &a, const std::vector<int> &work, const std::vector<int> &active, PipeRegion *pr) {
+struct RunAhead {
+  bool open = false;
+  bool used = false;
+  int chk_threads = 0;
+  std::vector<int> points;
+  std::vector<int> group, rest, work;
+  std::vector<int> ru0;
+};
+constexpr int kRunaheadQuarters = 2;
+static bool runahead_applies(const mi_osqp_batch *h) {
+  const int lanes = h->tune.refactor_lanes > 0 ? h->tune.refactor_lanes : kDefaultLanes;
+  return h->tune.runahead && h->tune.refactor_pipeline && h->BT == 1 && lanes <= 2 && h->st.adaptive_rho && h->st.adaptive_rho_interval > 0 &&
+         h->mw_groups <= 0 && !h->global_xs && !(*h->anp).wide && !(*h->anp).df;
+}
+static int ensure_runahead_buffers(mi_osqp_batch *h) {
+  int rc;
+  if (!h->ra_list.p && (rc = h->ra_list.alloc((size_t)5 * h->ntiles))) return rc;
+  if (!h->ra_res.p && (rc = h->ra_res.alloc((size_t)2 * h->ntiles))) return rc;
+  if (!h->h_res) HIPCHK(hostpool::alloc((void **)&h->h_res, (size_t)2 * h->ntiles * sizeof(double), &h->h_res_cap));
+  if (!h->h_mark) HIPCHK(hostpool::alloc((void **)&h->h_mark, (size_t)h->ntiles * sizeof(int), &h->h_mark_cap));
+  return 0;
+}
+
+static int pipelined_refactor_iterate(mi_osqp_batch *h, const KernelArgs &a, const std::vector<int> &work, const std::vector<int> &active, PipeRegion *pr,
+                                      const RunAhead *ra = nullptr) {
   using streampool::kPipeChunks; using streampool::kPipeEvents; using streampool::kPipeLanes;
   const double t_begin = now_s();
   const int BT = h->BT, nq = (int)work.size();
@@ -1298,6 +1328,7 @@
                                           h->ntiles * BT + 4);
   const int L = rl.n_lanes;
   if (L > 2 && !h->pipe_x) HIPCHK(hipStreamCreateWithFlags(&h->pipe_x, hipStreamNonBlocking));
+  if (ra && (L > 2 || BT != 1)) { g_last_error = "run-ahead beside three chunk lanes / tiles of several QPs"; return MI_OSQP_ERR_INVALID_SETTINGS; }
   std::vector<int> &wl = pr->wl;
   std::vector<int> wl_begin(1, 0);
   wl.clear();
@@ -1311,6 +1342,15 @@
   if (h->tile_list.n < ch.tiles.size() && (rc = h->tile_list.alloc((size_t)h->ntiles))) return rc;
   HIPCHK(hipMemcpyAsync(h->work.p, wl.data(), wl.size() * sizeof(int), hipMemcpyHostToDevice, h->stream));
   HIPCHK(hipMemcpyAsync(h->tile_list.p, pr->tiles.data(), pr->tiles.size() * sizeof(int), hipMemcpyHostToDevice, h->stream));
+  const int ntl = h->ntiles, G = ra ? (int)ra->group.size() : 0, gw = ra ? (int)ra->work.size() : 0;
+  int *d_rest = h->ra_list.p, *d_group = d_rest + ntl, *d_gwork = d_rest + 2 * (size_t)ntl, *d_dwork = d_rest + 3 * (size_t)ntl, *d_mark = d_rest + 4 * (size_t)ntl;
+  if (ra) {
+    if (!h->ra_list.p || G <= 0 || G + (int)ra->rest.size() != ntl || gw > G || nq + G > ntl + 4) { g_last_error = "run-ahead: inconsistent lists"; return MI_OSQP_ERR_INVALID_SETTINGS; }
+    if (!ra->rest.empty()) HIPCHK(hipMemcpyAsync(d_rest, ra->rest.data(), ra->rest.size() * sizeof(int), hipMemcpyHostToDevice, h->stream));
+    HIPCHK(hipMemcpyAsync(d_group, ra->group.data(), (size_t)G * sizeof(int), hipMemcpyHostToDevice, h->stream));
+    if (gw) HIPCHK(hipMemcpyAsync(d_gwork, ra->work.data(), (size_t)gw * sizeof(int), hipMemcpyHostToDevice, h->stream));
+    HIPCHK(hipMemsetAsync(d_mark, 0, (size_t)ntl * sizeof(int), h->stream));
+  }
   pr->host_s = now_s() - t_begin;
   HIPCHK(hipEventRecord(ev_fork, h->stream));
   FactorArgs fa = make_factor_args(h, 0);
@@ -1340,6 +1380,39 @@
     HIPCHK(launch_iterate(ai, BT, nt, h->threads, h->lds_iter + h->lds_factor, st));
     return 0;
   };
+  hipStream_t sx = h->stream;
+  KernelArgs ac = a;
+  ac.tiles = d_group; ac.res = nullptr; ac.info_at_end = 1;
+  FactorArgs fg = make_factor_args(h, 0);
+  fg.wg_base = nq;
+  auto chain_refactor = [&](const int *list, int n, int iter) -> int {
+    if (n <= 0) return 0;
+    fg.work = list;
+    HIPCHK(launch_factor(fg, 1, n, h->tune.factor_threads, sx));
+    if (tail) {
+      TailArgs da = make_tail_args(h, 1, list);
+      da.wg_base = nq;
+      HIPCHK(launch_tail(da, n, h->dt_lds_asm, h->dt_lds, sx));
+    }
+    HIPCHK(launch_fail_flagged(a, list, n, BT, iter, sx, d_mark));
+    return 0;
+  };
+  auto chain_segment = [&](size_t k) -> int {
+    ac.iter_begin = k ? ra->points[k - 1] : a.iter_begin; ac.iter_end = ra->points[k];
+    ac.rf_form = iterate_form(G, h->rf_off != 0, h->tune);
+    h->rf_launches[ac.rf_form]++;
+    HIPCHK(launch_iterate(ac, BT, G, h->threads, h->lds_iter + h->lds_factor, sx));
+    HIPCHK(launch_check(ac, BT, G, ra->chk_threads, h->lds, sx));
+    const int e = ra->points[k];
+    if (k + 1 < ra->points.size() && e % (int)h->st.adaptive_rho_interval == 0) {
+      HIPCHK(launch_worklist_of(h->iscal.p, d_group, d_dwork, G, BT, sx));
+      return chain_refactor(d_dwork, G, e);
+    }
+    return 0;
+  };
+  if (ra) {
+    if ((rc = chain_refactor(d_gwork, gw, a.iter_begin)) || (rc = chain_segment(0))) return rc;
+  }
   pr->lane_last.assign(L, 0);
   if (L == 1) {
     HIPCHK(hipStreamWaitEvent(h->pipe_r, ev_fork, 0));
@@ -1352,7 +1425,6 @@
       if ((rc = enqueue_iterate(c, h->pipe_i))) return rc;
     }
     HIPCHK(hipEventRecord(ev_lane(0), h->pipe_i));
-    HIPCHK(hipStreamWaitEvent(h->stream, ev_lane(0), 0));
   } else {
     hipStream_t lane[kPipeLanes] = {h->pipe_r, h->pipe_i, h->pipe_x};
     for (int l = 0; l < L; l++) HIPCHK(hipStreamWaitEvent(lane[l], ev_fork, 0));
@@ -1367,8 +1439,10 @@
       if ((rc = enqueue_iterate(c, lane[l]))) return rc;
     }
     if (!chunk0_first && (rc = enqueue_iterate(0, lane[rl.lane_of[0]]))) return rc;
-    for (int l = 0; l < L; l++) { HIPCHK(hipEventRecord(ev_lane(l), lane[l])); HIPCHK(hipStreamWaitEvent(h->stream, ev_lane(l), 0)); }
-  }
+    for (int l = 0; l < L; l++) HIPCHK(hipEventRecord(ev_lane(l), lane[l]));
+  }
+  if (ra) for (size_t k = 1; k < ra->points.size(); k++) if ((rc = chain_segment(k))) return rc;
+  for (int l = 0; l < L; l++) HIPCHK(hipStreamWaitEvent(h->stream, ev_lane(l), 0));
   HIPCHK(hipEventRecord(ev_join, h->stream));
   HIPCHK(launch_fail_flagged(a, h->work.p, (int)wl.size(), BT, a.iter_begin, h->stream));
   pr->open = true; pr->iter = a.iter_begin; pr->n_chunks = ch.n_chunks; pr->n_lanes = L; pr->tail = tail;
@@ -1432,13 +1506,29 @@
       seg_end = std::min<int64_t>(seg_end, (iter / S.adaptive_rho_interval + 1) * S.adaptive_rho_interval);
     return seg_end;
   };
+  const int ra_min = h->tune.runahead_min > 0 ? h->tune.runahead_min : h->n_cus;
+  if (runahead_applies(h) && ntl > 1 && ntl >= ra_min) {
+    if ((rc = ensure_runahead_buffers(h))) return rc;
+    a.res = h->ra_res.p;
+  }
+  auto is_rho_point = [&](int iter) { return S.adaptive_rho && S.adaptive_rho_interval > 0 && iter % S.adaptive_rho_interval == 0; };
   auto loop = [&]() -> int {
     int iter = 0;
     bool iterated = false;
     PipeRegion region;
-    while (true) {
-      const int seg_end = segment_end(iter);
-      a.iter_begin = iter; a.iter_end = seg_end; a.info_at_end = 1;
+    RunAhead ra;
+    std::vector<char> held;
+    std::vector<int> left;
+    const int *d_tiles = nullptr;
+    int n_launch = ntl, res_iter = -1;
+    bool leftovers_phase = false;
+    auto check_threads = [&]() {
+      int chk_threads = h->mw_groups > 0 ? h->mw_threads : h->threads;
+      if (h->mw_groups <= 0 && h->threads == 1024 && ntl > 2 * h->n_cus) chk_threads = 512;
+      return chk_threads;
+    };
+    auto device_turn = [&](int seg_end) -> int {
+      a.iter_begin = iter; a.iter_end = seg_end; a.info_at_end = 1; a.tiles = d_tiles;
       {
         std::unique_lock<std::mutex> spin_lock(spin_mutex(h->device), std::defer_lock);
         if (h->mw_groups > 0) spin_lock.lock();
@@ -1447,15 +1537,16 @@
           if (h->mw_groups > 0) HIPCHK(hipMemsetAsync(h->mw_bar.p, 0, 4 * sizeof(uint32_t), h->stream));
           a.rf_form = iterate_form(iterating, h->rf_off != 0, h->tune);
           h->rf_launches[a.rf_form]++;
-          HIPCHK(launch_iterate(a, BT, ntl, h->mw_groups > 0 ? h->mw_threads : h->threads, h->lds_iter + h->lds_factor, h->stream));
+          HIPCHK(launch_iterate(a, BT, n_launch, h->mw_groups > 0 ? h->mw_threads : h->threads, h->lds_iter + h->lds_factor, h->stream));
           HIPCHK(hipEventRecord(h->ev1, h->stream));
         }
-        {
-          int chk_threads = h->mw_groups > 0 ? h->mw_threads : h->threads;
-          if (h->mw_groups <= 0 && h->threads == 1024 && ntl > 2 * h->n_cus) chk_threads = 512;
-          HIPCHK(launch_check(a, BT, ntl, chk_threads, h->lds, h->stream));
+        HIPCHK(launch_check(a, BT, n_launch, check_threads(), h->lds, h->stream));
+        HIPCHK(hipMemcpyAsync(h->h_iscal, h->iscal.p, (size_t)ntl * IS_COUNT * BT * sizeof(int), hipMemcpyDeviceToHost, h->stream));
+        if (a.res && !ra.used && is_rho_point(seg_end) && seg_end < S.max_iter) {
+          HIPCHK(hipMemcpyAsync(h->h_res, h->ra_res.p, (size_t)2 * ntl * sizeof(double), hipMemcpyDeviceToHost, h->stream));
+          res_iter = seg_end;
         }
-        HIPCHK(hipMemcpyAsync(h->h_iscal, h->iscal.p, (size_t)ntl * IS_COUNT * BT * sizeof(int), hipMemcpyDeviceToHost, h->stream));
+        if (ra.open) HIPCHK(hipMemcpyAsync(h->h_mark, h->ra_list.p + 4 * (size_t)ntl, (size_t)ntl * sizeof(int), hipMemcpyDeviceToHost, h->stream));
         HIPCHK(hipStreamSynchronize(h->stream));
       }
       if ((rc = mw_barrier_ok(h))) {
@@ -1470,15 +1561,38 @@
         h->last_device_s += ms * 1e-3; h->kernel_ms_sum += ms; h->kernel_launches++; h->last_launches++;
       } else if ((rc = pipelined_region_finish(h, &region))) return rc;
       iterated = false;
-      iter = seg_end;
+      if (ra.open) {
+        ra.open = false;
+        int64_t inner = 0, n_left = 0;
+        for (size_t i = 0; i < ra.group.size(); i++) {
+          const int t = ra.group[i];
+          const int *f = h->h_iscal + (size_t)t * IS_COUNT;
+          const bool flagged = f[IS_NEED_REFACTOR] == 1;
+          inner += f[IS_RHO_UPDATES] - ra.ru0[i] - (flagged ? 1 : 0);
+          if (h->h_mark[t]) h->failed[(size_t)t] = 1;
+          n_left += !f[IS_DONE];
+          if (!f[IS_DONE] || flagged) left.push_back(t);
+        }
+        std::sort(left.begin(), left.end());
+        h->last_refactors += inner; h->refactor_qps += (int64_t)ra.work.size() + inner;
+        h->ra_left += n_left;
+        if (left.empty()) { d_tiles = nullptr; n_launch = ntl; }
+        else { held.assign((size_t)nslots, 0); for (int t : left) held[(size_t)t] = 1; }
+      }
+      return 0;
+    };
+    auto host_turn = [&](bool *go_on) -> int {
+      *go_on = false;
       std::vector<int> active, work;
       for (int s = 0; s < h->B; s++) {
+        if (!held.empty() && held[(size_t)s]) continue;
         const int *t = h->h_iscal + (size_t)(s / BT) * IS_COUNT * BT;
         if (!t[IS_DONE * BT + s % BT]) active.push_back(s);
         if (t[IS_NEED_REFACTOR * BT + s % BT]) work.push_back(s);
       }
+      if (ra.used && !leftovers_phase && ra.points.size() && iter == segment_end(ra.points[0])) h->ra_missed += (int64_t)active.size();
       const int n_ref = (int)work.size();
-      if (active.empty() && !n_ref) break;
+      if (active.empty() && !n_ref) return 0;
       if (n_ref) {
         double tr = now_s();
         std::vector<int> bad;
@@ -1486,7 +1600,33 @@
         if (!active.empty() && pipeline_applies(h, n_ref)) {
           KernelArgs nx = a;
           nx.iter_begin = iter; nx.iter_end = segment_end(iter); nx.info_at_end = 1;
-          if ((rc2 = pipelined_refactor_iterate(h, nx, work, active, &region))) return rc2;
+          std::vector<int> work_m, active_m;
+          if (a.res && !ra.used && res_iter == iter) {
+            std::vector<double> pri(active.size()), dua(active.size());
+            for (size_t i = 0; i < active.size(); i++) { pri[i] = h->h_res[2 * (size_t)active[i]]; dua[i] = h->h_res[2 * (size_t)active[i] + 1]; }
+            const int size = h->tune.runahead_tiles > 0 ? h->tune.runahead_tiles : std::max(1, h->n_cus * kRunaheadQuarters / 4);
+            std::vector<int> group = runahead_group(active, pri, dua, size, ra_min);
+            if (!group.empty() && group.size() < active.size()) {
+              std::vector<char> in((size_t)nslots, 0);
+              for (int t : group) in[(size_t)t] = 1;
+              for (int s : work) (in[(size_t)s] ? ra.work : work_m).push_back(s);
+              for (int s : active) if (!in[(size_t)s]) active_m.push_back(s);
+              if (pipeline_applies(h, (int)work_m.size())) {
+                for (int t = 0; t < ntl; t++) if (!in[(size_t)t]) ra.rest.push_back(t);
+                for (int t : group) ra.ru0.push_back(h->h_iscal[(size_t)t * IS_COUNT + IS_RHO_UPDATES]);
+                const int interval = (int)S.adaptive_rho_interval;
+                const int end = (int)std::min<int64_t>(S.max_iter, (int64_t)(iter / interval + 2) * interval);
+                for (int it = iter; it < end && (h->tune.runahead_end <= 0 || (int)ra.points.size() < h->tune.runahead_end);) ra.points.push_back(it = segment_end(it));
+                ra.group = std::move(group); ra.chk_threads = check_threads();
+                ra.used = ra.open = true;
+              } else ra.work.clear();
+            }
+          }
+          if (ra.open) {
+            if ((rc2 = pipelined_refactor_iterate(h, nx, work_m, active_m, &region, &ra))) return rc2;
+            d_tiles = h->ra_list.p; n_launch = (int)ra.rest.size();
+            h->ra_regions++; h->ra_tiles += (int64_t)ra.group.size();
+          } else if ((rc2 = pipelined_refactor_iterate(h, nx, work, active, &region))) return rc2;
           iterated = true;
           tr = now_s();
         } else if ((rc2 = device_refactor_slots(h, std::move(work), &bad))) return rc2;
@@ -1500,13 +1640,34 @@
           active.erase(std::remove_if(active.begin(), active.end(), [&](int q) { return isbad[q] != 0; }), active.end());
         }
       }
-      if (active.empty()) break;
+      if (active.empty()) return 0;
       iterating = 0;
       for (size_t i = 0; i < active.size(); i++) iterating += !i || active[i] / BT != active[i - 1] / BT;
+      *go_on = true;
+      return 0;
+    };
+    while (true) {
+      const int seg_end = segment_end(iter);
+      if ((rc = device_turn(seg_end))) return rc;
+      iter = seg_end;
+      bool go_on = false;
+      if ((rc = host_turn(&go_on))) return rc;
+      if (go_on) continue;
+      if (leftovers_phase || left.empty()) break;
+      leftovers_phase = true;
+      held.assign((size_t)nslots, 1);
+      for (int t : left) held[(size_t)t] = 0;
+      HIPCHK(hipMemcpyAsync(h->ra_list.p, left.data(), left.size() * sizeof(int), hipMemcpyHostToDevice, h->stream));
+      d_tiles = h->ra_list.p; n_launch = (int)left.size();
+      a.tiles = d_tiles;
+      iter = ra.points.back();
+      if ((rc = host_turn(&go_on))) return rc;
+      if (!go_on) break;
     }
     return MI_OSQP_OK;
   };
   rc = loop();
+  a.tiles = nullptr; a.res = nullptr;
   if (rc) {
     if (h->pipe_r) (void)hipStreamSynchronize(h->pipe_r);
     if (h->pipe_i) (void)hipStreamSynchronize(h->pipe_i);
@@ -1783,6 +1944,8 @@
   st->refactor_lanes = h->refactor_lanes;
   st->iterate_launches_deep_ring = h->rf_launches[RF_FORM_DEEP_RING];
   st->iterate_launches_long_head = h->rf_launches[RF_FORM_LONG_HEAD];
+  st->runahead_regions = h->ra_regions; st->runahead_tiles = h->ra_tiles;
+  st->runahead_left = h->ra_left; st->runahead_missed = h->ra_missed;
   return MI_OSQP_OK;
 }
 
@@ -3488,6 +3651,26 @@
   std::copy(rl.wait_for.begin(), rl.wait_for.end(), wait_for);
   return MI_OSQP_OK;
 }
+int mi_osqp_debug_runahead_group(int64_t n_active, const int64_t *tiles, const double *pri_res, const double *dua_res, int64_t size,
+                                 int64_t min_active, int64_t *n_group, int64_t *group) {
+  if (!n_group || !group || (n_active > 0 && (!tiles || !pri_res || !dua_res))) return MI_OSQP_ERR_NULL;
+  if (n_active < 0 || n_active > INT32_MAX || size < 0 || size > INT32_MAX || min_active < 0 || min_active > INT32_MAX) return MI_OSQP_ERR_INVALID_DATA;
+  std::vector<int> t((size_t)n_active);
+  for (int64_t i = 0; i < n_active; i++) {
+    if (tiles[i] < 0 || tiles[i] > INT32_MAX || pri_res[i] < 0.0 || dua_res[i] < 0.0) return MI_OSQP_ERR_INVALID_DATA;
+    t[(size_t)i] = (int)tiles[i];
+  }
+  {
+    std::vector<int> sorted = t;
+    std::sort(sorted.begin(), sorted.end());
+    if (std::adjacent_find(sorted.begin(), sorted.end()) != sorted.end()) return MI_OSQP_ERR_INVALID_DATA;
+  }
+  const std::vector<int> g = runahead_group(t, std::vector<double>(pri_res, pri_res + n_active), std::vector<double>(dua_res, dua_res + n_active),
+                                            (int)size, (int)min_active);
+  *n_group = (int64_t)g.size();
+  std::copy(g.begin(), g.end(), group);
+  return MI_OSQP_OK;
+}
 int mi_osqp_debug_iterate_form(int64_t tiles, int64_t has_head, int64_t forced_form, int64_t long_min, int64_t *form) {
   if (!form) return MI_OSQP_ERR_NULL;
   if (tiles < 0 || tiles > INT32_MAX || forced_form < 0 || forced_form > 2 || long_min < -1 || long_min > INT32_MAX)
```

Measured after the change: 42880, median of 6. 4.8% higher.
